# lyclyc52/Instance_NeRF

Hardware: AMD Instinct MI355X
Metric: Msamples/sec (train+infer) 3D-FRONT 800x800 at 1/2/4/8 MI355X; PSNR parity (higher is better)
Workload: dtype f32; 1 GPU; render 800x800 synthetic 3D-FRONT-like room, hash-grid NeRF L=16 F=2 T=6119864 sigma+rgb (BASELINE configs[1]), one view per step per GPU; parallelism=views sharded over 1 GPU(s), no data-path collective

## Files before the change

include/inr.h:

```cpp
#ifndef INR_H
#define INR_H

#include <stdint.h>

#ifdef __cplusplus
extern "C" {
#endif

#define INR_ABI_VERSION 12
#define INR_MAX_LEVELS 16

enum {
  INR_OK = 0,
  INR_EINVAL = -1,
  INR_ELAUNCH = -2,
  INR_ENODEV = -3
};

typedef void* inr_stream_t;

enum {
  INR_NUMERICS_TABLE_F16 = 1,
  INR_NUMERICS_MLP_F16 = 2
};

typedef struct inr_grid_desc {
  int32_t num_levels;
  int32_t level_dim;
  uint32_t offsets[INR_MAX_LEVELS + 1];
  float scales[INR_MAX_LEVELS];
  uint32_t resolutions[INR_MAX_LEVELS];
  uint32_t hashed[INR_MAX_LEVELS];
} inr_grid_desc;

int inr_abi_version(void);
const char* inr_last_error(void);
int inr_device_info(int32_t device, int64_t* props);
int inr_set_overlap_placement(int32_t on);
int inr_set_march_mode(int32_t mode);

int inr_get_rays(const float* poses, int64_t B, float fx, float fy, float cx, float cy, int32_t W,
                 const int64_t* inds , int64_t n, float* rays_o, float* rays_d, inr_stream_t s);

int inr_sample_training_batch(const float* pose , float fx, float fy, float cx, float cy, int32_t H, int32_t W,
                              const float* image , int32_t channels, const int32_t* mask ,
                              int32_t num_instances, int64_t seed, int64_t step, int64_t n, int64_t* inds ,
                              float* rays_o, float* rays_d, float* rgb , int64_t* labels ,
                              inr_stream_t s);

int inr_near_far_from_aabb(const float* rays_o, const float* rays_d, const float* aabb ,
                           int64_t N, float min_near, float* nears, float* fars, inr_stream_t s);
int inr_near_far_from_aabb_skip(const float* rays_o, const float* rays_d, const float* aabb , int64_t N,
                                float min_near, const int64_t* labels, int64_t ignore_index, float* nears, float* fars,
                                inr_stream_t s);

int inr_morton3D(const int32_t* coords , int64_t N, int32_t* indices, inr_stream_t s);
int inr_morton3D_invert(const int32_t* indices, int64_t N, int32_t* coords , inr_stream_t s);
int inr_packbits(const float* grid, int64_t n_bytes, float thresh, uint8_t* bitfield, inr_stream_t s);

int inr_mark_untrained_grid(const float* poses, int32_t B, float fx, float fy, float cx, float cy, int32_t H,
                            int32_t cascade, float bound, float* grid , inr_stream_t s);
int inr_occ_cell_positions(const int32_t* morton_idx, const float* noise, int64_t n, int32_t H, float cascade_bound,
                           float* xyz , inr_stream_t s);
int inr_occ_update(float* grid , const float* sigma , const int32_t* morton_idx ,
                   int64_t n_cells, int64_t m, float decay, float density_scale, float* tmp, double* mean_sum,
                   inr_stream_t s);
int inr_packbits_mean(const float* grid, int64_t n_cells , const double* mean_sum, float density_thresh,
                      uint8_t* bitfield, float* mean_out , const int32_t* counters ,
                      int32_t n_counters, int32_t counter_stride , double* stats_out ,
                      inr_stream_t s);
int64_t inr_occ_sample_workspace_bytes(int64_t n_cells);
int inr_occ_sample_cells(const float* grid , int64_t n_cells, const float* u ,
                         int64_t n, int32_t* morton_idx , void* workspace, inr_stream_t s);

int inr_march_write_fills_unowned_rows(int64_t N, int32_t sample_cap, int32_t max_steps);
int64_t inr_march_workspace_bytes(int64_t N, int32_t sample_cap);
int inr_march_rays_train_count(const float* rays_o, const float* rays_d, const uint8_t* bitfield,
                               float bound, float dt_gamma, int32_t max_steps, int64_t N,
                               int32_t cascade, int32_t H, const float* nears, const float* fars,
                               const float* noises , int32_t* rays ,
                               int32_t* counter , void* workspace, int32_t sample_cap, inr_stream_t s);
int inr_march_rays_train_write(const float* rays_o, const float* rays_d, const uint8_t* bitfield,
                               float bound, float dt_gamma, int32_t max_steps, int64_t N,
                               int32_t cascade, int32_t H, int64_t M, const float* nears,
                               const float* fars, const float* noises ,
                               const int32_t* rays , float* xyzs ,
                               float* dirs , float* deltas , const void* workspace,
                               int32_t sample_cap, inr_stream_t s);

int inr_march_rays_patch_write(const float* rays_o, const float* rays_d, const uint8_t* bitfield,
                               float bound, float dt_gamma, int32_t max_steps, int64_t N,
                               int32_t cascade, int32_t H, int64_t M, const float* nears,
                               const float* fars, const float* noises ,
                               const int32_t* rays ,
                               float* xyzs, float* dirs , float* deltas,
                               const void* workspace, int32_t sample_cap, int32_t* ray_ids ,
                               int32_t normalise , inr_stream_t s);
int inr_composite_rays_patch_forward(const float* sigmas, const float* rgbs, const float* deltas,
                                     const int32_t* rays, int64_t N, int64_t M, float T_thresh,
                                     const float* extra , int32_t K,
                                     float* weights_sum, float* depth, float* image,
                                     float* extra_out , float* weights ,
                                     uint64_t* skippable ,
                                     inr_stream_t s);
int inr_project_masks_patch(const float* xyzs, const float* weights, const int32_t* rays, int64_t N, int64_t M,
                            const uint32_t* mask_words, int32_t W, int32_t L, int32_t H, const float* bbox ,
                            int32_t k_total, int32_t k_base, int32_t k_count, float* out, inr_stream_t s);

int inr_march_rays(int64_t n_alive, int32_t n_step, const int32_t* rays_alive, const float* rays_t,
                   const float* rays_o, const float* rays_d, float bound, float dt_gamma,
                   int32_t max_steps, int32_t cascade, int32_t H, const uint8_t* bitfield,
                   const float* nears, const float* fars, float* xyzs, float* dirs, float* deltas,
                   inr_stream_t s);
int inr_composite_rays(int64_t n_alive, int32_t n_step, int32_t* rays_alive, float* rays_t,
                       const float* sigmas, const float* rgbs, const float* deltas,
                       float* weights_sum, float* depth, float* image, float T_thresh,
                       const float* extra , float* extra_acc ,
                       int32_t K, inr_stream_t s);
int inr_compact_alive(const int32_t* rays_alive, int64_t n_alive, int32_t* out, int32_t* n_out,
                      inr_stream_t s);

int inr_composite_rays_train_forward(const float* sigmas, const float* rgbs, const float* deltas,
                                     const int32_t* rays, int64_t N, int64_t M, float T_thresh,
                                     const float* extra , int32_t K,
                                     float* weights_sum, float* depth, float* image,
                                     float* extra_out , float* weights ,
                                     int32_t* sample_ray , inr_stream_t s);
int inr_composite_rays_extra_forward(const float* weights , const float* extra , const int32_t* rays,
                                     int64_t N, int64_t M, int32_t K, float* extra_out ,
                                     const int64_t* labels , int32_t n_classes, int64_t ignore_index,
                                     float* grad_pix, void* workspace, float* loss_out, inr_stream_t s);
int inr_composite_rays_train_backward(const float* grad_weights_sum, const float* grad_image,
                                      const float* grad_extra_out , const float* sigmas,
                                      const float* rgbs, const float* extra, const float* deltas,
                                      const int32_t* rays, const float* weights_sum,
                                      const float* image, const float* weights ,
                                      int64_t N, int64_t M, float T_thresh, int32_t K,
                                      float* grad_sigmas, float* grad_rgbs ,
                                      float* grad_extra , const int32_t* total_dev ,
                                      inr_stream_t s);

int inr_grid_encode_forward(const float* x , const float* embeddings ,
                            const inr_grid_desc* desc , int64_t M, float bound,
                            float* out , inr_stream_t s);
int inr_grid_encode_backward(const float* x, const float* grad_out ,
                             const inr_grid_desc* desc , int64_t M, float bound,
                             float* grad_embeddings , inr_stream_t s);

int inr_grid_encode_backward_ordered(const float* x, const float* grad_out, const int32_t* order,
                                     const inr_grid_desc* desc , int64_t M, float bound,
                                     float* grad_embeddings , inr_stream_t s);
int inr_grid_encode_backward_input(const float* x, const float* grad_out , const float* embeddings,
                                   const inr_grid_desc* desc , int64_t M, float bound, float* grad_x,
                                   inr_stream_t s);
int inr_grid_encode_backward_levels(const float* x, const float* grad_out, const int32_t* order,
                                    const inr_grid_desc* desc, int64_t M, float bound, float* grad_embeddings,
                                    int32_t level_lo, int32_t level_hi, inr_stream_t s);

#define INR_GRID_FX_STATE_FLOATS 4192
int inr_grid_encode_backward_levels_fx(const float* x, const float* grad_out, const int32_t* order,
                                       const inr_grid_desc* desc, int64_t M, float bound, float* grad_embeddings,
                                       int32_t level_lo, int32_t level_hi, float* fx_state ,
                                       inr_stream_t s);
int inr_grid_grad_finish_fx(float* grad_embeddings, const inr_grid_desc* desc , int32_t level_lo,
                            int32_t level_hi, float* fx_state, inr_stream_t s);
int inr_grid_fx_update(float* fx_state, int32_t num_levels, float headroom, int32_t sum_bits , inr_stream_t s);
int inr_grid_encode_backward_levels_fx64(const float* x, const float* grad_out, const int32_t* order,
                                         const inr_grid_desc* desc, int64_t M, float bound, float* grad_embeddings,
                                         int64_t* acc64 , int32_t level_lo, int32_t level_hi, float* fx_state,
                                         inr_stream_t s);
int inr_grid_grad_finish_fx64(int64_t* acc64, float* grad_embeddings, const inr_grid_desc* desc , int32_t level_lo,
                              int32_t level_hi, float* fx_state, inr_stream_t s);

int inr_sh_encode_forward(const float* d , int64_t M, int32_t degree, float* out, inr_stream_t s);
int inr_sh_encode_backward(const float* grad_out, const float* d, int64_t M, int32_t degree,
                           float* grad_d, inr_stream_t s);
int inr_sh_table_q(const float* d , int64_t N, float* out , inr_stream_t s);

int64_t inr_nerf_packed_floats(void);
int inr_nerf_pack_weights(const float* sigma_w0, const float* sigma_w1, const float* color_w0,
                          const float* color_w1, const float* color_w2, float* packed , int32_t numerics);
int64_t inr_instance_packed_floats(int32_t K);
int inr_instance_pack_weights(const float* w0, const float* w1, const float* w2, int32_t K,
                              float* packed , int32_t numerics);
int inr_nerf_forward(const float* x, const float* d, int64_t M, const int32_t* n_samples_dev,
                     float bound, const void* embeddings, const inr_grid_desc* desc ,
                     const float* packed , float density_scale, float* sigma, float* rgb,
                     float* geo_feat, int32_t numerics, inr_stream_t s);
int inr_nerf_forward_table(const float* x01, const int32_t* ray_ids, const float* sh_table_q, int64_t M,
                           float bound, const void* embeddings, const inr_grid_desc* desc ,
                           const float* packed , float density_scale, float* sigma, float* rgb,
                           int32_t numerics, inr_stream_t s);
int64_t inr_nerf_forward_table_sliced_workspace_bytes(int64_t M);
int inr_nerf_forward_table_sliced(const float* x01, const int32_t* ray_ids, const float* sh_table_q, int64_t M,
                                  float bound, const float* embeddings, const inr_grid_desc* desc ,
                                  const float* packed , float density_scale, float* sigma, float* rgb,
                                  float* fine_ws, inr_stream_t s);
int64_t inr_nerf_bwd_packed_floats(void);
int inr_nerf_pack_weights_device(const float* sigma_w0, const float* sigma_w1, const float* color_w0,
                                 const float* color_w1, const float* color_w2, float* packed_fwd,
                                 float* packed_bwd, inr_stream_t s);
int inr_nerf_forward_train(const float* x, const float* d, int64_t M, float bound, const float* embeddings,
                           const inr_grid_desc* desc , const float* packed_fwd, float* sigma, float* rgb,
                           float* enc, float* h1, float* so, float* cin, float* c1, float* c2, inr_stream_t s);
int inr_nerf_backward(const float* grad_sigma, const float* grad_rgb, const float* rgb, const float* so,
                      const float* h1, const float* c1, const float* c2, int64_t M, float density_scale,
                      const float* packed_bwd, float* grad_o, float* grad_zc2, float* grad_zc1, float* grad_so,
                      float* grad_zh1, float* grad_enc, inr_stream_t s);
int inr_nerf_forward_enc(const float* x, const float* d, int64_t M, float bound, const float* embeddings,
                         const inr_grid_desc* desc , const float* packed_fwd, float* sigma, float* rgb,
                         float* enc, inr_stream_t s);
int inr_nerf_head_backward(const float* enc, const float* d, const float* grad_sigma, const float* grad_rgb, int64_t M,
                           float density_scale, const float* packed_fwd, const float* packed_bwd, float* grad_enc,
                           void* workspace, float* grad_ws0, float* grad_ws1, float* grad_wc0, float* grad_wc1,
                           float* grad_wc2, float* zero_buf , int64_t zero_floats, inr_stream_t s);
int64_t inr_instance_bwd_packed_floats(void);
int inr_instance_pack_weights_device(const float* w0 , const float* w1 ,
                                     const float* w2 , int32_t K, float* packed_fwd, float* packed_bwd,
                                     inr_stream_t s);
int inr_instance_forward_train(const float* x, int64_t M, float bound, const float* embeddings,
                               const inr_grid_desc* desc , const float* packed_fwd, int32_t K,
                               float* logits, float* enc, float* h1, float* h2, inr_stream_t s);
int inr_instance_backward(const float* grad_logits, int32_t K, const float* h1, const float* h2, int64_t M,
                          const float* packed_bwd, float* grad_z2, float* grad_z1, float* grad_enc,
                          inr_stream_t s);
int inr_instance_forward_enc(const float* x, int64_t M, const int32_t* n_samples_dev, float bound,
                             const float* embeddings, const inr_grid_desc* desc , const float* packed_fwd,
                             int32_t K, float* logits, float* enc, inr_stream_t s);
int64_t inr_instance_head_workspace_bytes(void);
int inr_instance_head_backward(const float* enc, const float* weights, const int32_t* sample_ray,
                               const float* grad_pix, int32_t K, int64_t N, int64_t M, const int32_t* n_samples_dev,
                               const float* scale_a , const float* scale_b ,
                               const float* packed_fwd, const float* packed_bwd, float* grad_enc, void* workspace,
                               float* grad_w0, float* grad_w1, float* grad_w2, float* zero_buf ,
                               int64_t zero_floats, inr_stream_t s);
int inr_nerf_forward_dirs(const float* x, int64_t M, float bound, const float* embeddings, const inr_grid_desc* desc ,
                          const float* packed , const float* sh_dirs, int32_t n_dirs, float* out, inr_stream_t s);
int inr_nerf_forward_lattice(const float* ax_w, const float* ax_l, const float* ax_h, int32_t W, int32_t L, int32_t H,
                             float bound, const float* embeddings, const inr_grid_desc* desc ,
                             const float* packed , const float* sh_dirs, int32_t n_dirs, float logit_min,
                             float* out, inr_stream_t s);
int inr_instance_forward(const float* x, int64_t M, const int32_t* n_samples_dev, float bound,
                         const float* embeddings, const inr_grid_desc* desc ,
                         const float* packed , int32_t K, float* logits ,
                         inr_stream_t s);
int inr_instance_lattice(const float* ax_w, const float* ax_l, const float* ax_h, int32_t W, int32_t L, int32_t H,
                         float bound, const float* nerf_embeddings, const inr_grid_desc* nerf_desc ,
                         const float* nerf_packed , float density_scale, float sigma_thresh,
                         const float* inst_embeddings, const inr_grid_desc* inst_desc ,
                         const float* inst_packed , int32_t K, uint8_t* labels, float* confidence,
// ... 88 lines not shown
```

instance_nerf_amd/_lib.py:

```python
import ctypes
import os
from ctypes import POINTER, Structure, c_char_p, c_float, c_int32, c_int64, c_uint32, c_void_p

import torch

_HERE = os.path.dirname(os.path.abspath(__file__))
LIB_PATH = os.environ.get("INR_LIB_PATH") or os.path.join(_HERE, "csrc", "libinr_hip.so")
MAX_LEVELS = 16
GRID_FX_STATE_FLOATS = 4192
NUMERICS_TABLE_F16, NUMERICS_MLP_F16 = 1, 2


class GridDesc(Structure):
    _fields_ = [("num_levels", c_int32), ("level_dim", c_int32),
                ("offsets", c_uint32 * (MAX_LEVELS + 1)), ("scales", c_float * MAX_LEVELS),
                ("resolutions", c_uint32 * MAX_LEVELS), ("hashed", c_uint32 * MAX_LEVELS)]


P = c_void_p
_SIGS = {
    "inr_abi_version": (c_int32, []),
    "inr_last_error": (c_char_p, []),
    "inr_set_overlap_placement": (c_int32, [c_int32]),
    "inr_set_march_mode": (c_int32, [c_int32]),
    "inr_device_info": (c_int32, [c_int32, POINTER(c_int64)]),
    "inr_get_rays": (c_int32, [P, c_int64, c_float, c_float, c_float, c_float, c_int32, P, c_int64, P, P, P]),
    "inr_sample_training_batch": (c_int32, [P, c_float, c_float, c_float, c_float, c_int32, c_int32, P, c_int32, P, c_int32,
                                            c_int64, c_int64, c_int64, P, P, P, P, P, P]),
    "inr_near_far_from_aabb": (c_int32, [P, P, P, c_int64, c_float, P, P, P]),
    "inr_near_far_from_aabb_skip": (c_int32, [P, P, P, c_int64, c_float, P, c_int64, P, P, P]),
    "inr_morton3D": (c_int32, [P, c_int64, P, P]),
    "inr_morton3D_invert": (c_int32, [P, c_int64, P, P]),
    "inr_packbits": (c_int32, [P, c_int64, c_float, P, P]),
    "inr_mark_untrained_grid": (c_int32, [P, c_int32, c_float, c_float, c_float, c_float, c_int32, c_int32, c_float, P, P]),
    "inr_occ_cell_positions": (c_int32, [P, P, c_int64, c_int32, c_float, P, P]),
    "inr_occ_update": (c_int32, [P, P, P, c_int64, c_int64, c_float, c_float, P, P, P]),
    "inr_packbits_mean": (c_int32, [P, c_int64, P, c_float, P, P, P, c_int32, c_int32, P, P]),
    "inr_occ_sample_workspace_bytes": (c_int64, [c_int64]),
    "inr_occ_sample_cells": (c_int32, [P, c_int64, P, c_int64, P, P, P]),
    "inr_march_write_fills_unowned_rows": (c_int32, [c_int64, c_int32, c_int32]),
    "inr_march_workspace_bytes": (c_int64, [c_int64, c_int32]),
    "inr_march_rays_train_count": (c_int32, [P, P, P, c_float, c_float, c_int32, c_int64, c_int32, c_int32,
                                             P, P, P, P, P, P, c_int32, P]),
    "inr_march_rays_train_write": (c_int32, [P, P, P, c_float, c_float, c_int32, c_int64, c_int32, c_int32,
                                             c_int64, P, P, P, P, P, P, P, P, c_int32, P]),
    "inr_march_rays_patch_write": (c_int32, [P, P, P, c_float, c_float, c_int32, c_int64, c_int32, c_int32,
                                             c_int64, P, P, P, P, P, P, P, P, c_int32, P, c_int32, P]),
    "inr_nerf_bwd_packed_floats": (c_int64, []),
    "inr_nerf_pack_weights_device": (c_int32, [P, P, P, P, P, P, P, P]),
    "inr_nerf_forward_train": (c_int32, [P, P, c_int64, c_float, P, POINTER(GridDesc), P, P, P, P, P, P, P, P, P, P]),
    "inr_nerf_backward": (c_int32, [P, P, P, P, P, P, P, c_int64, c_float, P, P, P, P, P, P, P, P]),
    "inr_instance_bwd_packed_floats": (c_int64, []),
    "inr_instance_pack_weights_device": (c_int32, [P, P, P, c_int32, P, P, P]),
    "inr_instance_forward_train": (c_int32, [P, c_int64, c_float, P, POINTER(GridDesc), P, c_int32, P, P, P, P, P]),
    "inr_instance_backward": (c_int32, [P, c_int32, P, P, c_int64, P, P, P, P, P]),
    "inr_nerf_forward_enc": (c_int32, [P, P, c_int64, c_float, P, POINTER(GridDesc), P, P, P, P, P]),
    "inr_nerf_head_backward": (c_int32, [P, P, P, P, c_int64, c_float, P, P, P, P, P, P, P, P, P, P, c_int64, P]),
    "inr_instance_forward_enc": (c_int32, [P, c_int64, P, c_float, P, POINTER(GridDesc), P, c_int32, P, P, P]),
    "inr_instance_head_workspace_bytes": (c_int64, []),
    "inr_instance_head_backward": (c_int32, [P, P, P, P, c_int32, c_int64, c_int64, P, P, P, P, P, P, P, P, P, P, P, c_int64, P]),
    "inr_adam_step_multi": (c_int32, [c_int32, P, P, P, P, P, P, c_float, c_float, c_float, c_int32, c_float, P]),
    "inr_adam_ema_step_multi": (c_int32, [c_int32, P, P, P, P, P, P, c_float, c_float, c_float, c_int32, c_float, P,
                                          c_float, P]),
    "inr_adam_set_hyper": (c_int32, [P, c_int32, c_float, c_float, c_float, c_int32, P, P]),
    "inr_adam_step_multi_dev": (c_int32, [c_int32, P, P, P, P, P, P, c_float, c_float, c_float, P]),
    "inr_copy_multi": (c_int32, [c_int32, P, P, P, P]),
    "inr_adam_set_hyper_ema": (c_int32, [P, c_int32, c_float, c_float, c_float, c_int32, c_float, P, P]),
    "inr_adam_ema_step_multi_dev": (c_int32, [c_int32, P, P, P, P, P, P, c_float, c_float, c_float, P, P]),
    "inr_cross_entropy": (c_int32, [P, P, c_int64, c_int32, c_int64, P, P, P, P]),
    "inr_finish_rays": (c_int32, [P, P, P, P, P, P, c_float, c_float, c_float, c_int64, P, P, P]),
    "inr_finish_rays_mse": (c_int32, [P, P, P, P, P, c_float, c_float, c_float, P, P, c_int64, P, P, P, P, P]),
    "inr_sh_table_q": (c_int32, [P, c_int64, P, P]),
    "inr_nerf_forward_table": (c_int32, [P, P, P, c_int64, c_float, P, POINTER(GridDesc), P, c_float, P, P, c_int32, P]),
    "inr_nerf_forward_table_sliced_workspace_bytes": (c_int64, [c_int64]),
    "inr_nerf_forward_table_sliced": (c_int32, [P, P, P, c_int64, c_float, P, POINTER(GridDesc), P, c_float, P, P, P, P]),
    "inr_composite_rays_patch_forward": (c_int32, [P, P, P, P, c_int64, c_int64, c_float, P, c_int32, P, P, P, P, P, P, P]),
    "inr_project_masks_patch": (c_int32, [P, P, P, c_int64, c_int64, P, c_int32, c_int32, c_int32, P, c_int32, c_int32, c_int32,
                                          P, P]),
    "inr_march_rays": (c_int32, [c_int64, c_int32, P, P, P, P, c_float, c_float, c_int32, c_int32, c_int32,
                                 P, P, P, P, P, P, P]),
    "inr_composite_rays": (c_int32, [c_int64, c_int32, P, P, P, P, P, P, P, P, c_float, P, P, c_int32, P]),
    "inr_compact_alive": (c_int32, [P, c_int64, P, P, P]),
    "inr_composite_rays_extra_forward": (c_int32, [P, P, P, c_int64, c_int64, c_int32, P, P, c_int32, c_int64, P, P, P, P]),
    "inr_composite_rays_train_forward": (c_int32, [P, P, P, P, c_int64, c_int64, c_float, P, c_int32, P, P, P, P, P, P, P]),
    "inr_composite_rays_train_backward": (c_int32, [P, P, P, P, P, P, P, P, P, P, P, c_int64, c_int64, c_float, c_int32,
                                                    P, P, P, P, P]),
    "inr_grid_encode_forward": (c_int32, [P, P, POINTER(GridDesc), c_int64, c_float, P, P]),
    "inr_grid_encode_backward": (c_int32, [P, P, POINTER(GridDesc), c_int64, c_float, P, P]),
    "inr_grid_encode_backward_ordered": (c_int32, [P, P, P, POINTER(GridDesc), c_int64, c_float, P, P]),
    "inr_grid_encode_backward_input": (c_int32, [P, P, P, POINTER(GridDesc), c_int64, c_float, P, P]),
    "inr_grid_encode_backward_levels": (c_int32, [P, P, P, POINTER(GridDesc), c_int64, c_float, P, c_int32, c_int32, P]),
    "inr_grid_encode_backward_levels_fx": (c_int32, [P, P, P, POINTER(GridDesc), c_int64, c_float, P, c_int32, c_int32, P, P]),
    "inr_grid_grad_finish_fx": (c_int32, [P, POINTER(GridDesc), c_int32, c_int32, P, P]),
    "inr_grid_fx_update": (c_int32, [P, c_int32, c_float, c_int32, P]),
    "inr_grid_encode_backward_levels_fx64": (c_int32, [P, P, P, POINTER(GridDesc), c_int64, c_float, P, P, c_int32, c_int32, P, P]),
    "inr_grid_grad_finish_fx64": (c_int32, [P, P, POINTER(GridDesc), c_int32, c_int32, P, P]),
    "inr_sh_encode_forward": (c_int32, [P, c_int64, c_int32, P, P]),
    "inr_sh_encode_backward": (c_int32, [P, P, c_int64, c_int32, P, P]),
    "inr_nerf_packed_floats": (c_int64, []),
    "inr_nerf_pack_weights": (c_int32, [P, P, P, P, P, P, c_int32]),
    "inr_instance_packed_floats": (c_int64, [c_int32]),
    "inr_instance_pack_weights": (c_int32, [P, P, P, c_int32, P, c_int32]),
    "inr_nerf_forward": (c_int32, [P, P, c_int64, P, c_float, P, POINTER(GridDesc), P, c_float, P, P, P, c_int32, P]),
    "inr_nerf_forward_dirs": (c_int32, [P, c_int64, c_float, P, POINTER(GridDesc), P, P, c_int32, P, P]),
    "inr_nerf_forward_lattice": (c_int32, [P, P, P, c_int32, c_int32, c_int32, c_float, P, POINTER(GridDesc), P, P, c_int32,
                                           c_float, P, P]),
    "inr_instance_forward": (c_int32, [P, c_int64, P, c_float, P, POINTER(GridDesc), P, c_int32, P, P]),
    "inr_instance_lattice": (c_int32, [P, P, P, c_int32, c_int32, c_int32, c_float, P, POINTER(GridDesc), P, c_float,
                                       c_float, P, POINTER(GridDesc), P, c_int32, P, P, P, P]),
    "inr_instance_volume_stats": (c_int32, [P, P, c_int32, c_int32, c_int32, c_int32, P, c_int64, P, P, P, P]),
    "inr_mesh_workspace_bytes": (c_int64, [c_int32, c_int32, c_int32, c_int32]),
    "inr_mesh_count": (c_int32, [P, c_int32, c_float, c_float, P, c_int32, c_int32, c_int32, c_int32, c_int32, P, c_int64, P, P]),
    "inr_mesh_emit": (c_int32, [P, c_int32, c_float, c_float, P, c_int32, P, P, P, P, c_int32, c_int32, c_int32, c_float,
                                c_float, c_float, c_int32, P, c_int64, c_int32, c_int32, P, P, P, P, P]),
    "inr_roi_align_3d_set_mode": (c_int32, [c_int32]),
    "inr_roi_align_3d_forward": (c_int32, [P, P, P, c_int32, c_int32, c_int32, c_int32, c_int32, c_int64, c_int32,
                                           c_int32, c_int32, c_float, P, P]),
    "inr_roi_align_3d_backward": (c_int32, [P, P, P, c_int32, c_int32, c_int32, c_int32, c_int32, c_int64, c_int32,
                                            c_int32, c_int32, c_float, P, P]),
    "inr_roi_align_3d_backward_workspace_bytes": (c_int64, [c_int32, c_int32, c_int32, c_int32, c_int32, c_int64, c_int32,
                                                            c_int32, c_int32]),
    "inr_roi_align_3d_backward_prefers_workspace": (c_int32, [c_int32, c_int32, c_int32, c_int32, c_int32, c_int64, c_int32,
                                                              c_int32, c_int32, c_int64]),
    "inr_roi_align_3d_backward_ws": (c_int32, [P, P, P, c_int32, c_int32, c_int32, c_int32, c_int32, c_int64, c_int32,
                                               c_int32, c_int32, c_float, P, P, c_int64, P]),
    "inr_nerf_render": (c_int32, [P, P, P, P, c_int64, c_int64, c_float, P, POINTER(GridDesc), P, c_float, c_float,
                                  P, P, P, P, P, c_int32, c_int32, P]),
    "inr_instance_render": (c_int32, [P, P, P, c_int64, c_int64, c_float, P, POINTER(GridDesc), P, c_int32, P, c_int32, P,
                                      c_int32, P]),
    "inr_linear_wgrad_workspace_bytes": (c_int64, []),
    "inr_linear_wgrad": (c_int32, [P, P, c_int64, c_int32, c_int32, P, P, P]),
    "inr_adam_step": (c_int32, [P, P, P, P, c_int64, c_float, c_float, c_float, c_float, c_int32, c_float, P]),
}
EXPORTS = tuple(_SIGS)

ABI_VERSION = 12
INSTANCE_STATS_WORKSPACE_BYTES = 512 * 64 * 8 * 4
_lib = None


def load():
    global _lib
    if _lib is not None:
        return _lib
    if not os.path.exists(LIB_PATH):
        raise RuntimeError(
            f"{LIB_PATH} is missing: build it with `python -m instance_nerf_amd.build` "
            "(or __graft_entry__.build()).  There is no CPU fallback.")
    lib = ctypes.CDLL(LIB_PATH)
    version = getattr(lib, "inr_abi_version", None)
    if version is not None:
        version.restype, version.argtypes = c_int32, []
    found = version() if version is not None else None
    if found != ABI_VERSION:
        raise RuntimeError(f"{LIB_PATH} ABI version {found} != {ABI_VERSION} (include/inr.h "
                           "INR_ABI_VERSION): rebuild with `python -m instance_nerf_amd.build --force`")
    for name, (res, args) in _SIGS.items():
        fn = getattr(lib, name)
        fn.restype = res
        fn.argtypes = args
    _lib = lib
    return lib


def check(rc, what=""):
    if rc != 0:
        msg = load().inr_last_error()
        raise RuntimeError(f"libinr_hip {what} failed (code {rc}): {msg.decode() if msg else ''}")


_raw_stream = getattr(torch._C, "_cuda_getCurrentRawStream", None)
_cur_device = getattr(torch._C, "_cuda_getDevice", None)


def stream_ptr():
    if _raw_stream is not None and _cur_device is not None:
        return c_void_p(_raw_stream(_cur_device()))
    return c_void_p(torch.cuda.current_stream().cuda_stream)


def ptr(t, dtype=None, name="tensor", allow_none=False):
    if t is None:
        if allow_none:
            return None
        raise RuntimeError(f"{name} must not be None")
    if not t.is_cuda:
        raise RuntimeError(f"{name} must be a GPU tensor (the HIP path has no CPU fallback)")
    if not t.is_contiguous():
        raise RuntimeError(f"{name} must be contiguous")
    if dtype is not None and t.dtype != dtype:
        raise RuntimeError(f"{name} must be {dtype}, got {t.dtype}")
    return c_void_p(t.data_ptr())


def host_ptr(t, dtype, name="tensor"):
    if t.is_cuda or not t.is_contiguous() or t.dtype != dtype:
        raise RuntimeError(f"{name} must be a contiguous CPU {dtype} tensor")
    return c_void_p(t.data_ptr())


def make_grid_desc(table):
    d = GridDesc()
    L = int(table["num_levels"])
    d.num_levels = L
    d.level_dim = int(table["level_dim"])
    for i in range(L + 1):
        d.offsets[i] = int(table["offsets"][i])
    for i in range(L):
        d.scales[i] = float(table["scales"][i])
        d.resolutions[i] = int(table["resolutions"][i])
        d.hashed[i] = int(table["hashed"][i])
    return d
```

instance_nerf_amd/csrc/raymarch.hip:

```cpp
#include "common.h"

namespace inr {

static thread_local char g_err[512] = "";
int g_field_lds_min = 0;
int g_march_lds_pad = 0;
void set_error(const char* fmt, ...) {
  va_list ap;
  va_start(ap, fmt);
  vsnprintf(g_err, sizeof(g_err), fmt, ap);
  va_end(ap);
}

constexpr int kRayBlock = 256;
constexpr float kSqrt3x2 = 3.4641016151377544f;

__global__ void __launch_bounds__(kRayBlock) k_near_far(const float* __restrict__ rays_o,
                                                        const float* __restrict__ rays_d,
                                                        const float* __restrict__ aabb, int64_t N,
                                                        float min_near, float* __restrict__ nears,
                                                        float* __restrict__ fars,
                                                        const int64_t* __restrict__ labels, int64_t ignore) {
  const int64_t n = (int64_t)blockIdx.x * blockDim.x + threadIdx.x;
  if (n >= N) return;
  float near = -INFINITY, far = INFINITY;
  bool miss = labels != nullptr && labels[n] == ignore;
#pragma unroll
  for (int a = 0; a < 3; ++a) {
    const float o = rays_o[n * 3 + a];
    const float rd = 1.0f / rays_d[n * 3 + a];
    const float t0 = (aabb[a] - o) * rd;
    const float t1 = (aabb[a + 3] - o) * rd;
    const float lo = t0 > t1 ? t1 : t0;
    const float hi = t0 > t1 ? t0 : t1;
    if (a > 0) miss = miss || (near > hi) || (lo > far);
    near = lo > near ? lo : near;
    far = hi < far ? hi : far;
  }
  if (near < min_near) near = min_near;
  nears[n] = miss ? 3.402823466e+38f : near;
  fars[n] = miss ? 3.402823466e+38f : far;
}

__global__ void __launch_bounds__(kRayBlock) k_get_rays(const float* __restrict__ poses, int64_t B, float fx, float fy,
                                                        float cx, float cy, int W, const int64_t* __restrict__ inds,
                                                        int64_t n, float* __restrict__ rays_o,
                                                        float* __restrict__ rays_d) {
  const int64_t idx = (int64_t)blockIdx.x * blockDim.x + threadIdx.x;
  if (idx >= B * n) return;
  const int64_t b = idx / n, k = idx - b * n;
  const int64_t pix = inds ? inds[k] : k;
  const float i = (float)(pix % W) + 0.5f, j = (float)(pix / W) + 0.5f;
  const float xs = (i - cx) / fx, ys = (j - cy) / fy;
  const float nrm = sqrtf(xs * xs + ys * ys + 1.0f * 1.0f);
  const float dx = xs / nrm, dy = ys / nrm, dz = 1.0f / nrm;
  const float* P = poses + b * 16;
#pragma unroll
  for (int r = 0; r < 3; ++r) {
    rays_d[idx * 3 + r] = dx * P[r * 4 + 0] + dy * P[r * 4 + 1] + dz * P[r * 4 + 2];
    rays_o[idx * 3 + r] = P[r * 4 + 3];
  }
}

__device__ __forceinline__ uint64_t mix64(uint64_t z) {
  z = (z ^ (z >> 30)) * 0xBF58476D1CE4E5B9ull;
  z = (z ^ (z >> 27)) * 0x94D049BB133111EBull;
  return z ^ (z >> 31);
}
__global__ void __launch_bounds__(kRayBlock) k_sample_batch(const float* __restrict__ pose, float fx, float fy, float cx,
                                                            float cy, int H, int W, const float* __restrict__ image,
                                                            int C, const int32_t* __restrict__ mask, int num_instances,
                                                            uint64_t seed, uint64_t step, int64_t n,
                                                            int64_t* __restrict__ inds, float* __restrict__ rays_o,
                                                            float* __restrict__ rays_d, float* __restrict__ rgb,
                                                            int64_t* __restrict__ labels) {
  const int64_t k = (int64_t)blockIdx.x * blockDim.x + threadIdx.x;
  if (k >= n) return;
  const uint64_t h = mix64(seed + 0x9E3779B97F4A7C15ull * ((step << 32) + (uint64_t)k));
  const uint64_t pix = ((h >> 32) * (uint64_t)((int64_t)H * W)) >> 32;
  inds[k] = (int64_t)pix;
  const float i = (float)(pix % (uint64_t)W) + 0.5f, j = (float)(pix / (uint64_t)W) + 0.5f;
  const float xs = (i - cx) / fx, ys = (j - cy) / fy;
  const float nrm = sqrtf(xs * xs + ys * ys + 1.0f * 1.0f);
  const float dx = xs / nrm, dy = ys / nrm, dz = 1.0f / nrm;
#pragma unroll
  for (int r = 0; r < 3; ++r) {
    rays_d[k * 3 + r] = dx * pose[r * 4 + 0] + dy * pose[r * 4 + 1] + dz * pose[r * 4 + 2];
    rays_o[k * 3 + r] = pose[r * 4 + 3];
  }
  if (image) {
    for (int c = 0; c < C; ++c) rgb[k * C + c] = image[pix * C + c];
  }
  if (mask) {
    const int32_t l = mask[pix];
    labels[k] = l >= num_instances ? -1 : (int64_t)l;
  }
}

__global__ void k_morton3D(const int32_t* __restrict__ coords, int64_t N, int32_t* __restrict__ out) {
  const int64_t n = (int64_t)blockIdx.x * blockDim.x + threadIdx.x;
  if (n >= N) return;
  out[n] = (int32_t)morton3((uint32_t)coords[n * 3], (uint32_t)coords[n * 3 + 1], (uint32_t)coords[n * 3 + 2]);
}
__global__ void k_morton3D_invert(const int32_t* __restrict__ idx, int64_t N, int32_t* __restrict__ coords) {
  const int64_t n = (int64_t)blockIdx.x * blockDim.x + threadIdx.x;
  if (n >= N) return;
  const uint32_t m = (uint32_t)idx[n];
  coords[n * 3 + 0] = (int32_t)compact_bits10(m);
  coords[n * 3 + 1] = (int32_t)compact_bits10(m >> 1);
  coords[n * 3 + 2] = (int32_t)compact_bits10(m >> 2);
}
__global__ void k_packbits(const float* __restrict__ grid, int64_t n_bytes, float thresh,
                           uint8_t* __restrict__ bits) {
  const int64_t n = (int64_t)blockIdx.x * blockDim.x + threadIdx.x;
  if (n >= n_bytes) return;
  const float4 a = reinterpret_cast<const float4*>(grid)[n * 2];
  const float4 b = reinterpret_cast<const float4*>(grid)[n * 2 + 1];
  uint32_t v = (a.x > thresh) | ((a.y > thresh) << 1) | ((a.z > thresh) << 2) | ((a.w > thresh) << 3) |
               ((b.x > thresh) << 4) | ((b.y > thresh) << 5) | ((b.z > thresh) << 6) | ((b.w > thresh) << 7);
  bits[n] = (uint8_t)v;
}

__global__ void k_occ_positions(const int32_t* __restrict__ morton, const float* __restrict__ noise, int64_t n, float Hm1,
                                float ext, float half, float* __restrict__ xyz) {
  const int64_t i = (int64_t)blockIdx.x * blockDim.x + threadIdx.x;
  if (i >= n) return;
  const uint32_t m = morton ? (uint32_t)morton[i] : (uint32_t)i;
  const uint32_t c[3] = {compact_bits10(m), compact_bits10(m >> 1), compact_bits10(m >> 2)};
#pragma unroll
  for (int a = 0; a < 3; ++a) {
    float v = (2.0f * (float)c[a] / Hm1 - 1.0f) * ext;
    if (noise) v = v + (noise[i * 3 + a] * 2.0f - 1.0f) * half;
    xyz[i * 3 + a] = v;
  }
}
__global__ void __launch_bounds__(256) k_mark_untrained(const float* __restrict__ poses, int B, float kx, float ky, int H,
                                                        int C, float bound, float* __restrict__ grid) {
  const int64_t i = (int64_t)blockIdx.x * blockDim.x + threadIdx.x;
  const int64_t H3 = (int64_t)H * H * H;
  if (i >= (int64_t)C * H3) return;
  const int cas = (int)(i / H3);
  const uint32_t m = (uint32_t)(i - (int64_t)cas * H3);
  const float bnd = fminf(ldexpf(1.0f, cas), bound), half = bnd / (float)H, ext = bnd - half;
  const float wx = (2.0f * (float)compact_bits10(m) / (float)(H - 1) - 1.0f) * ext;
  const float wy = (2.0f * (float)compact_bits10(m >> 1) / (float)(H - 1) - 1.0f) * ext;
  const float wz = (2.0f * (float)compact_bits10(m >> 2) / (float)(H - 1) - 1.0f) * ext;
  bool seen = false;
  for (int b = 0; b < B && !seen; ++b) {
    const float* P = poses + (int64_t)b * 16;
    const float dx = wx - P[3], dy = wy - P[7], dz = wz - P[11];
    const float cx = dx * P[0] + dy * P[4] + dz * P[8];
    const float cy = dx * P[1] + dy * P[5] + dz * P[9];
    const float cz = dx * P[2] + dy * P[6] + dz * P[10];
    seen = cz > 0.0f && fabsf(cx) < kx * cz + half * 2.0f && fabsf(cy) < ky * cz + half * 2.0f;
  }
  if (!seen) grid[i] = -1.0f;
}

__global__ void k_occ_scatter(const float* __restrict__ sigma, const int32_t* __restrict__ morton, int64_t m,
                              float density_scale, float* __restrict__ tmp) {
  const int64_t i = (int64_t)blockIdx.x * blockDim.x + threadIdx.x;
  if (i < m) tmp[morton[i]] = sigma[i] * density_scale;
}
__global__ void __launch_bounds__(256) k_occ_update(float* __restrict__ grid, const float* __restrict__ tmp, int64_t n,
                                                    float decay, float scale, double* __restrict__ mean_sum) {
  __shared__ double red[4];
  double acc = 0.0;
  auto cell = [&](float g, float t, bool& changed) {
    t *= scale;
    if (g >= 0.0f && t >= 0.0f) { g = fmaxf(g * decay, t); changed = true; }
    acc += (double)fmaxf(g, 0.0f);
    return g;
  };
  const int64_t n4 = (((uintptr_t)grid | (uintptr_t)tmp) & 15) == 0 ? n / 4 : 0;
  for (int64_t i = (int64_t)blockIdx.x * blockDim.x + threadIdx.x; i < n4; i += (int64_t)gridDim.x * blockDim.x) {
    float4 g = reinterpret_cast<float4*>(grid)[i];
    const float4 t = reinterpret_cast<const float4*>(tmp)[i];
    bool changed = false;
    g.x = cell(g.x, t.x, changed); g.y = cell(g.y, t.y, changed); g.z = cell(g.z, t.z, changed); g.w = cell(g.w, t.w, changed);
    if (changed) reinterpret_cast<float4*>(grid)[i] = g;
  }
  for (int64_t i = n4 * 4 + (int64_t)blockIdx.x * blockDim.x + threadIdx.x; i < n; i += (int64_t)gridDim.x * blockDim.x) {
    bool changed = false;
    const float g = cell(grid[i], tmp[i], changed);
    if (changed) grid[i] = g;
  }
#pragma unroll
  for (int d = 32; d >= 1; d >>= 1) acc += __shfl_xor(acc, d, 64);
  if ((threadIdx.x & 63) == 0) red[threadIdx.x >> 6] = acc;
  __syncthreads();
  if (threadIdx.x == 0) atomicAdd(mean_sum, red[0] + red[1] + red[2] + red[3]);
}
__global__ void k_packbits_mean(const float* __restrict__ grid, int64_t n_bytes, const double* __restrict__ mean_sum,
                                double inv_cells, float density_thresh, uint8_t* __restrict__ bits,
                                float* __restrict__ mean_out, const int32_t* __restrict__ counters, int n_counters,
                                int counter_stride, double* __restrict__ stats_out) {
  const int64_t n = (int64_t)blockIdx.x * blockDim.x + threadIdx.x;
  const float mean = (float)(*mean_sum * inv_cells);
  if (n == 0 && mean_out) *mean_out = mean;
  if (n == 0 && stats_out) {
    int64_t total = 0;
    for (int k = 0; k < n_counters; ++k) total += counters[(int64_t)k * counter_stride];
    stats_out[0] = (double)mean;
    stats_out[1] = (double)total;
  }
  if (n >= n_bytes) return;
  const float thresh = fminf(mean, density_thresh);
  const float4 a = reinterpret_cast<const float4*>(grid)[n * 2];
  const float4 b = reinterpret_cast<const float4*>(grid)[n * 2 + 1];
  uint32_t v = (a.x > thresh) | ((a.y > thresh) << 1) | ((a.z > thresh) << 2) | ((a.w > thresh) << 3) |
               ((b.x > thresh) << 4) | ((b.y > thresh) << 5) | ((b.z > thresh) << 6) | ((b.w > thresh) << 7);
  bits[n] = (uint8_t)v;
}

struct MarchParams {
  const uint8_t* bits;
  float bound, dt_gamma, dt_min, dt_max, rH;
  int C, H, H3;
};

struct Ray {
  float ox, oy, oz, dx, dy, dz, rdx, rdy, rdz, sx, sy, sz;
};

__device__ __forceinline__ Ray load_ray(const float* __restrict__ o, const float* __restrict__ d, int64_t n) {
  Ray r;
  r.ox = o[n * 3]; r.oy = o[n * 3 + 1]; r.oz = o[n * 3 + 2];
  r.dx = d[n * 3]; r.dy = d[n * 3 + 1]; r.dz = d[n * 3 + 2];
  r.rdx = 1.0f / r.dx; r.rdy = 1.0f / r.dy; r.rdz = 1.0f / r.dz;
  r.sx = copysignf(1.0f, r.dx); r.sy = copysignf(1.0f, r.dy); r.sz = copysignf(1.0f, r.dz);
  return r;
}

__device__ __forceinline__ float step_dt(const MarchParams& P, float t) {
  return clampf(t * P.dt_gamma, P.dt_min, P.dt_max);
}
template <bool kConst>
struct StepRule {
  float c;
  __device__ __forceinline__ explicit StepRule(const MarchParams& P) : c(step_dt(P, 0.0f)) {}
  __device__ __forceinline__ float operator()(const MarchParams& P, float t) const {
    if constexpr (kConst) return c;
    else return step_dt(P, t);
  }
};

struct MortonCalc {
  __device__ __forceinline__ uint32_t operator()(uint32_t x, uint32_t y, uint32_t z) const { return morton3(x, y, z); }
};
struct MortonLut {
  const uint32_t* lut;
  __device__ __forceinline__ uint32_t operator()(uint32_t x, uint32_t y, uint32_t z) const {
    return lut[x] | (lut[y] << 1) | (lut[z] << 2);
  }
};

template <bool kSingle = false, bool kConstDt = false, class Emit, class Advance, class Morton = MortonCalc>
__device__ __forceinline__ int march_ray(const MarchParams& P, const Ray& r, float t, float far,
                                         int max_emit, Emit&& emit, Advance&& advance, Morton morton = Morton()) {
  int n = 0;
  float last_t = t;
  const StepRule<kConstDt> step(P);
  const float mb1 = fminf(ldexpf(1.0f, 0), P.bound), rmb1 = 1.0f / mb1;
  while (t < far && n < max_emit) {
    const float px = clampf(r.ox + t * r.dx, -P.bound, P.bound);
    const float py = clampf(r.oy + t * r.dy, -P.bound, P.bound);
    const float pz = clampf(r.oz + t * r.dz, -P.bound, P.bound);
    const float dt = step(P, t);
    int level = 0;
    float mb = mb1, rmb = rmb1;
    if constexpr (!kSingle) {
      int e0, e1;
      (void)frexpf(fmaxf(fabsf(px), fmaxf(fabsf(py), fabsf(pz))), &e0);
      (void)frexpf(dt * (float)P.H * 0.5f, &e1);
      level = max(clampi(e0, 0, P.C - 1), clampi(e1, 0, P.C - 1));
      mb = fminf(ldexpf(1.0f, level), P.bound);
      rmb = 1.0f / mb;
    }
    const int nx = clampi((int)(((px * rmb + 1.0f) * 0.5f) * (float)P.H), 0, P.H - 1);
    const int ny = clampi((int)(((py * rmb + 1.0f) * 0.5f) * (float)P.H), 0, P.H - 1);
    const int nz = clampi((int)(((pz * rmb + 1.0f) * 0.5f) * (float)P.H), 0, P.H - 1);
    const uint32_t idx = (uint32_t)level * (uint32_t)P.H3 + morton((uint32_t)nx, (uint32_t)ny, (uint32_t)nz);
    const bool occ = (P.bits[idx >> 3] >> (idx & 7)) & 1;
    if (occ) {
      const float tn = t + dt;
      emit(px, py, pz, dt, tn - last_t, t);
      t = tn;
      advance();
      last_t = tn;
      ++n;
    } else {
      const float ax = ((float)nx + 0.5f) + 0.5f * r.sx;
      const float ay = ((float)ny + 0.5f) + 0.5f * r.sy;
      const float az = ((float)nz + 0.5f) + 0.5f * r.sz;
      const float cx = (((ax * P.rH) * 2.0f - 1.0f) * mb - px) * r.rdx;
      const float cy = (((ay * P.rH) * 2.0f - 1.0f) * mb - py) * r.rdy;
      const float cz = (((az * P.rH) * 2.0f - 1.0f) * mb - pz) * r.rdz;
      const float tt = t + fmaxf(0.0f, fminf(cx, fminf(cy, cz)));
      do {
        t = t + step(P, t);
        advance();
      } while (t < tt);
    }
  }
  return n;
}
template <class Emit>
__device__ __forceinline__ int march_ray(const MarchParams& P, const Ray& r, float t, float far,
                                         int max_emit, Emit&& emit) {
  return P.dt_gamma == 0.0f ? march_ray<false, true>(P, r, t, far, max_emit, emit, [] {})
                            : march_ray<false, false>(P, r, t, far, max_emit, emit, [] {});
}
template <class Emit, class Advance, class Morton>
__device__ __forceinline__ int march_ray_any(const MarchParams& P, const Ray& r, float t, float far,
                                             int max_emit, Emit&& emit, Advance&& advance, Morton morton) {
  if (P.dt_gamma == 0.0f)
    return P.C == 1 ? march_ray<true, true>(P, r, t, far, max_emit, emit, advance, morton)
                    : march_ray<false, true>(P, r, t, far, max_emit, emit, advance, morton);
  return P.C == 1 ? march_ray<true, false>(P, r, t, far, max_emit, emit, advance, morton)
                  : march_ray<false, false>(P, r, t, far, max_emit, emit, advance, morton);
}

__device__ __forceinline__ float start_t(const MarchParams& P, float near, float noise) {
  return near + step_dt(P, near) * noise;
}

__global__ void __launch_bounds__(kRayBlock) k_march_count(MarchParams P, const float* __restrict__ rays_o,
                                                           const float* __restrict__ rays_d, int64_t N,
                                                           int max_steps, const float* __restrict__ nears,
                                                           const float* __restrict__ fars,
                                                           const float* __restrict__ noises,
                                                           int32_t* __restrict__ counts,
                                                           int32_t* __restrict__ block_sums,
                                                           uint32_t* __restrict__ mask, int cap_words) {
  __shared__ int32_t wsum[kRayBlock / 64];
  __shared__ uint32_t lut[1024];
  for (int i = threadIdx.x; i < P.H; i += kRayBlock) lut[i] = expand_bits10((uint32_t)i);
  __syncthreads();
  const MortonLut morton{lut};
  const int64_t n = (int64_t)blockIdx.x * blockDim.x + threadIdx.x;
  int cnt = 0;
  if (n < N) {
    const Ray r = load_ray(rays_o, rays_d, n);
    const float t0 = start_t(P, nears[n], noises ? noises[n] : 0.0f);
    if (cap_words > 0) {
      uint32_t word = 0;
      int widx = 0, cand = 0;
      bool ok = true;
      cnt = march_ray_any(P, r, t0, fars[n], max_steps,
                      [&](float, float, float, float, float, float) {
                        const int w = cand >> 5;
                        if (w < cap_words) {
                          while (widx < w) {
                            mask[(int64_t)widx * N + n] = word;
                            word = 0;
                            ++widx;
                          }
                          word |= 1u << (cand & 31);
                        } else {
                          ok = false;
                        }
                      },
                      [&] { ++cand; }, morton);
      if (widx < cap_words) mask[(int64_t)widx * N + n] = word;
      mask[(int64_t)cap_words * N + n] = ok ? 1u : 0u;
    } else {
      cnt = march_ray_any(P, r, t0, fars[n], max_steps, [](float, float, float, float, float, float) {}, [] {}, morton);
    }
    counts[n] = cnt;
  }
  const int incl = wave_inclusive_scan(cnt);
  if ((threadIdx.x & 63) == 63) wsum[threadIdx.x >> 6] = incl;
  __syncthreads();
  if (threadIdx.x == 0) {
    int s = 0;
#pragma unroll
    for (int w = 0; w < kRayBlock / 64; ++w) s += wsum[w];
    block_sums[blockIdx.x] = s;
  }
}

__global__ void __launch_bounds__(1024) k_scan_block_sums(int32_t* __restrict__ block_sums, int n_blocks,
                                                          int64_t N, int32_t* __restrict__ counter) {
  __shared__ int32_t wsum[16];
  __shared__ int32_t carry_s;
  if (threadIdx.x == 0) carry_s = 0;
  __syncthreads();
  for (int base = 0; base < n_blocks; base += 1024) {
    const int i = base + threadIdx.x;
    const int v = i < n_blocks ? block_sums[i] : 0;
    const int incl = wave_inclusive_scan(v);
    if ((threadIdx.x & 63) == 63) wsum[threadIdx.x >> 6] = incl;
    __syncthreads();
    int wave_off = 0;
    for (int w = 0; w < (int)(threadIdx.x >> 6); ++w) wave_off += wsum[w];
    const int carry = carry_s;
    if (i < n_blocks) block_sums[i] = carry + wave_off + incl - v;
    __syncthreads();
    if (threadIdx.x == 1023) carry_s = carry + wave_off + incl;
    __syncthreads();
  }
  if (threadIdx.x == 0) {
    counter[0] = carry_s;
    counter[1] = (int32_t)N;
  }
}

__global__ void __launch_bounds__(kRayBlock) k_finalize_offsets(const int32_t* __restrict__ counts,
                                                                const int32_t* __restrict__ block_prefix,
                                                                int64_t N, int32_t* __restrict__ rays) {
  __shared__ int32_t wsum[kRayBlock / 64];
  const int64_t n = (int64_t)blockIdx.x * blockDim.x + threadIdx.x;
  const int cnt = n < N ? counts[n] : 0;
  const int incl = wave_inclusive_scan(cnt);
  if ((threadIdx.x & 63) == 63) wsum[threadIdx.x >> 6] = incl;
  __syncthreads();
  int off = block_prefix[blockIdx.x] + incl - cnt;
  for (int w = 0; w < (int)(threadIdx.x >> 6); ++w) off += wsum[w];
  if (n < N) {
    rays[n * 3 + 0] = (int32_t)n;
    rays[n * 3 + 1] = off;
    rays[n * 3 + 2] = cnt;
  }
}

template <bool kConstDt, class Emit>
__device__ __forceinline__ void replay_ray_t(const MarchParams& P, const Ray& r, const uint32_t* __restrict__ mask, int64_t N,
                                             int64_t n, float t, int cnt, Emit&& emit) {
  const StepRule<kConstDt> step(P);
  float last_t = t;
  int emitted = 0;
  for (int w = 0; emitted < cnt; ++w) {
    const uint32_t bits = mask[(int64_t)w * N + n];
    for (int b0 = 0; b0 < 32; b0 += 8) {
      const uint32_t sub = (bits >> b0) & 0xFFu;
      if (__ballot(sub != 0u) == 0ull) {
#pragma unroll
        for (int j = 0; j < 8; ++j) t = t + step(P, t);
        continue;
      }
#pragma unroll
      for (int j = 0; j < 8; ++j) {
        const float dt = step(P, t);
        const float tn = t + dt;
        if (sub & (1u << j)) {
          const float px = clampf(r.ox + t * r.dx, -P.bound, P.bound);
          const float py = clampf(r.oy + t * r.dy, -P.bound, P.bound);
          const float pz = clampf(r.oz + t * r.dz, -P.bound, P.bound);
          emit(px, py, pz, dt, tn - last_t, t);
          last_t = tn;
          ++emitted;
        }
        t = tn;
      }
    }
  }
}
template <class Emit>
__device__ __forceinline__ void replay_ray(const MarchParams& P, const Ray& r, const uint32_t* __restrict__ mask, int64_t N,
                                           int64_t n, float t, int cnt, Emit&& emit) {
  if (P.dt_gamma == 0.0f) replay_ray_t<true>(P, r, mask, N, n, t, cnt, emit);
  else replay_ray_t<false>(P, r, mask, N, n, t, cnt, emit);
}

__global__ void __launch_bounds__(kRayBlock) k_march_write(MarchParams P, const float* __restrict__ rays_o,
                                                           const float* __restrict__ rays_d, int64_t N,
                                                           int64_t M, const float* __restrict__ nears,
                                                           const float* __restrict__ fars,
                                                           const float* __restrict__ noises,
                                                           const int32_t* __restrict__ rays,
                                                           float* __restrict__ xyzs, float* __restrict__ dirs,
                                                           float* __restrict__ deltas,
                                                           const uint32_t* __restrict__ mask, int cap_words) {
  const int64_t n = (int64_t)blockIdx.x * blockDim.x + threadIdx.x;
  if (n >= N) return;
  const int off = rays[n * 3 + 1];
  const int cnt = rays[n * 3 + 2];
  if (cnt == 0 || (int64_t)off + cnt > M) return;
  const Ray r = load_ray(rays_o, rays_d, n);
  int64_t i = off;
  auto emit = [&](float px, float py, float pz, float dt, float delta, float) {
    xyzs[i * 3 + 0] = px; xyzs[i * 3 + 1] = py; xyzs[i * 3 + 2] = pz;
    dirs[i * 3 + 0] = r.dx; dirs[i * 3 + 1] = r.dy; dirs[i * 3 + 2] = r.dz;
    deltas[i * 2 + 0] = dt; deltas[i * 2 + 1] = delta;
    ++i;
  };
  const float t0 = start_t(P, nears[n], noises ? noises[n] : 0.0f);
  if (cap_words > 0 && mask[(int64_t)cap_words * N + n]) {
    replay_ray(P, r, mask, N, n, t0, cnt, emit);
  } else {
    march_ray(P, r, t0, fars[n], cnt, emit);
  }
}

template <bool kSingle = false, class Emit>
__device__ __forceinline__ int march_ray_coop(const MarchParams& P, const Ray& r, float t, float far, int max_emit,
                                              Emit&& emit) {
  const float mb1 = fminf(ldexpf(1.0f, 0), P.bound), rmb1 = 1.0f / mb1;
  const int lane = threadIdx.x & 63;
  const uint64_t lt_mask = (1ull << lane) - 1ull;
  int n = 0;
  float last_t = t;
  while (t < far && n < max_emit) {
    float c = t;
    if (P.dt_gamma == 0.0f) {
      const float dt0 = step_dt(P, t);
      asm volatile(
          ".rept 63\n"
          "s_nop 1\n"
          "v_add_f32_dpp %0, %0, %1 wave_shr:1 row_mask:0xf bank_mask:0xf\n"
          ".endr\n"
          : "+v"(c)
          : "v"(dt0));
    } else {
      for (int j = 0; j < 63; ++j) c = j < lane ? c + step_dt(P, c) : c;
    }
    const bool in = c < far;
    const float px = clampf(r.ox + c * r.dx, -P.bound, P.bound);
    const float py = clampf(r.oy + c * r.dy, -P.bound, P.bound);
    const float pz = clampf(r.oz + c * r.dz, -P.bound, P.bound);
    const float dt = step_dt(P, c);
    const float tn = c + dt;
    int level = 0;
    float mb = mb1, rmb = rmb1;
    if constexpr (!kSingle) {
      int e0, e1;
      (void)frexpf(fmaxf(fabsf(px), fmaxf(fabsf(py), fabsf(pz))), &e0);
      (void)frexpf(dt * (float)P.H * 0.5f, &e1);
      level = max(clampi(e0, 0, P.C - 1), clampi(e1, 0, P.C - 1));
      mb = fminf(ldexpf(1.0f, level), P.bound);
      rmb = 1.0f / mb;
    }
    const int nx = clampi((int)(((px * rmb + 1.0f) * 0.5f) * (float)P.H), 0, P.H - 1);
    const int ny = clampi((int)(((py * rmb + 1.0f) * 0.5f) * (float)P.H), 0, P.H - 1);
    const int nz = clampi((int)(((pz * rmb + 1.0f) * 0.5f) * (float)P.H), 0, P.H - 1);
    const uint32_t idx = (uint32_t)level * (uint32_t)P.H3 + morton3((uint32_t)nx, (uint32_t)ny, (uint32_t)nz);
    const bool occ = (P.bits[idx >> 3] >> (idx & 7)) & 1;
    const float ax = ((float)nx + 0.5f) + 0.5f * r.sx;
    const float ay = ((float)ny + 0.5f) + 0.5f * r.sy;
    const float az = ((float)nz + 0.5f) + 0.5f * r.sz;
    const float cx = (((ax * P.rH) * 2.0f - 1.0f) * mb - px) * r.rdx;
    const float cy = (((ay * P.rH) * 2.0f - 1.0f) * mb - py) * r.rdy;
    const float cz = (((az * P.rH) * 2.0f - 1.0f) * mb - pz) * r.rdz;
    const float tt = c + fmaxf(0.0f, fminf(cx, fminf(cy, cz)));
    int lo = lane + 1, hi = 64;
    bool settled_all = false;
    if (P.dt_gamma == 0.0f) {
      const int i0 = lane + (int)fminf((tt - c) * (1.0f / dt), 64.0f);
      const float ca = __shfl(c, clampi(i0 - 1, 0, 63), 64);
      const float cb = __shfl(c, min(i0, 63), 64);
      const float cc = __shfl(c, min(i0 + 1, 63), 64);
      const bool lt_a = i0 - 1 <= lane || ca < tt;
      const bool ge_b = i0 >= 64 || !(cb < tt);
      const bool ge_c = i0 + 1 >= 64 || !(cc < tt);
      const bool take_b = i0 > lane && ge_b;
      const bool settled = take_b ? lt_a : ge_c;
      lo = take_b ? min(i0, 64) : i0 + 1;
      settled_all = __ballot(in && !occ && !settled) == 0;
    }
    if (!settled_all) {
      lo = lane + 1;
#pragma unroll
      for (int it = 0; it < 7; ++it) {
        const int mid = (lo + hi) >> 1;
        const float cm = __shfl(c, min(mid, 63), 64);
        const bool below = mid < 64 && cm < tt;
        if (lo < hi) {
          if (below) lo = mid + 1; else hi = mid;
        }
      }
    }
    const int next = lo;
    const uint64_t in_mask = __ballot(in);
    const uint64_t miss_mask = __ballot(in && !occ);
    const int n_in = __popcll(in_mask);
// ... 605 lines not shown
    const float e = live ? expf(x - m) : 0.f;
    float ssum = e;
#pragma unroll
    for (int d = 1; d < 64; d <<= 1) ssum += __shfl_xor(ssum, d, 64);
    const float xy = __shfl(x, keep ? (int)y : 0, 64);
    if (lane < K) ce.dpix[(int64_t)rid * K + lane] = (keep && live) ? e / ssum - (lane == (int)y ? 1.f : 0.f) : 0.f;
    if (lane == 0)
      ce.part[rid] = make_float4(keep ? (m + logf(ssum)) - xy : 0.f, keep ? 1.f : 0.f,
                                 (y != ce.ignore_index && !in_range) ? 1.f : 0.f, 0.f);
  }
}

__global__ void __launch_bounds__(1024) k_ce_finalize(const float4* __restrict__ part, int64_t N, float* __restrict__ loss_out) {
  __shared__ float red[3][16];
  float a = 0.f, b = 0.f, c = 0.f;
  for (int64_t i = threadIdx.x; i < N; i += 1024) {
    const float4 p = part[i];
    a += p.x; b += p.y; c += p.z;
  }
  a = wave_sum(a); b = wave_sum(b); c = wave_sum(c);
  if ((threadIdx.x & 63) == 0) { red[0][threadIdx.x >> 6] = a; red[1][threadIdx.x >> 6] = b; red[2][threadIdx.x >> 6] = c; }
  __syncthreads();
  if (threadIdx.x == 0) {
    float sa = 0.f, sb = 0.f, sc = 0.f;
    for (int w = 0; w < 16; ++w) { sa += red[0][w]; sb += red[1][w]; sc += red[2][w]; }
    loss_out[0] = sc > 0.f ? NAN : sa / sb;
    loss_out[1] = sb > 0.f ? 1.0f / sb : 0.f;
    loss_out[2] = sb;
    loss_out[3] = sc;
  }
}

__global__ void __launch_bounds__(kRayBlock) k_composite_train_bwd(
    const float* __restrict__ g_ws, const float* __restrict__ g_img, const float* __restrict__ sigmas,
    const float* __restrict__ rgbs, const float* __restrict__ deltas, const int32_t* __restrict__ rays,
    const float* __restrict__ weights_sum, const float* __restrict__ image, int64_t N, int64_t M, float T_thresh,
    float* __restrict__ grad_sigmas, float* __restrict__ grad_rgbs, const int32_t* __restrict__ total_dev) {
  const int64_t n = ((int64_t)blockIdx.x * blockDim.x + threadIdx.x) >> 6;
  const int lane = threadIdx.x & 63;
  if (n >= N) return;
  const int32_t rid = rays[n * 3], off = rays[n * 3 + 1];
  int32_t cnt = rays[n * 3 + 2];
  auto zero_rows = [&](int64_t lo, int64_t hi) {
    for (int64_t i = lo + lane; i < hi; i += 64) {
      grad_sigmas[i] = 0.f; grad_rgbs[i * 3] = 0.f; grad_rgbs[i * 3 + 1] = 0.f; grad_rgbs[i * 3 + 2] = 0.f;
    }
  };
  if (total_dev) {
    const int64_t total = total_dev[0];
    if (total < M) {
      const int64_t per = (M - total + N - 1) / N;
      zero_rows(total + n * per, min(M, total + (n + 1) * per));
    }
  }
  if ((int64_t)off + cnt > M) {
    if (total_dev && cnt > 0 && off < M) zero_rows(off, M);
    cnt = 0;
  }
  const float gr = g_img[rid * 3], gg = g_img[rid * 3 + 1], gb = g_img[rid * 3 + 2];
  const float gw = g_ws ? g_ws[rid] : 0.0f;
  const float rf = image[rid * 3], gf = image[rid * 3 + 1], bf = image[rid * 3 + 2];
  const float wsf = weights_sum[rid];
  float T_carry = 1.0f, cr_carry = 0.f, cg_carry = 0.f, cb_carry = 0.f;
  bool dead = false;
  for (int base = 0; base < cnt; base += 64) {
    const bool act = base + lane < cnt;
    const int64_t i = (int64_t)off + base + lane;
    if (dead) {
      if (act) { grad_sigmas[i] = 0.f; grad_rgbs[i * 3] = 0.f; grad_rgbs[i * 3 + 1] = 0.f; grad_rgbs[i * 3 + 2] = 0.f; }
      continue;
    }
    float alpha = 0.f, d0 = 0.f, cr = 0.f, cg = 0.f, cb = 0.f;
    if (act) {
      d0 = deltas[i * 2];
      alpha = 1.0f - expf(-sigmas[i] * d0);
      cr = rgbs[i * 3]; cg = rgbs[i * 3 + 1]; cb = rgbs[i * 3 + 2];
    }
    const float P = wave_incl_prod(1.0f - alpha, lane);
    float Pprev = __shfl_up(P, 1, 64);
    if (lane == 0) Pprev = 1.0f;
    const float T = T_carry * Pprev, Tn = T_carry * P;
    const bool used = act && (T >= T_thresh || (base + lane) == 0);
    const float w = used ? alpha * T : 0.0f;
    const float ar = cr_carry + wave_incl_sum(w * cr, lane);
    const float ag = cg_carry + wave_incl_sum(w * cg, lane);
    const float ab = cb_carry + wave_incl_sum(w * cb, lane);
    if (act) {
      grad_rgbs[i * 3] = gr * w; grad_rgbs[i * 3 + 1] = gg * w; grad_rgbs[i * 3 + 2] = gb * w;
      grad_sigmas[i] = used ? d0 * (gr * (Tn * cr - (rf - ar)) + gg * (Tn * cg - (gf - ag)) + gb * (Tn * cb - (bf - ab)) +
                                    gw * (1.0f - wsf))
                            : 0.0f;
    }
    T_carry *= __shfl(P, 63, 64);
    cr_carry = __shfl(ar, 63, 64); cg_carry = __shfl(ag, 63, 64); cb_carry = __shfl(ab, 63, 64);
    if (T_carry < T_thresh) dead = true;
  }
}

__global__ void __launch_bounds__(kRayBlock) k_composite_train_extra_bwd(
    const float* __restrict__ g_extra_out, const float* __restrict__ wbuf, const int32_t* __restrict__ rays, int64_t N,
    int64_t M, int K, float* __restrict__ grad_extra) {
  const int64_t n = ((int64_t)blockIdx.x * blockDim.x + threadIdx.x) >> 6;
  const int lane = threadIdx.x & 63;
  if (n >= N) return;
  const int32_t rid = rays[n * 3], off = rays[n * 3 + 1];
  int32_t cnt = rays[n * 3 + 2];
  if ((int64_t)off + cnt > M) cnt = 0;
  if (lane >= K) return;
  const float g = g_extra_out[(int64_t)rid * K + lane];
  for (int s = 0; s < cnt; ++s) grad_extra[((int64_t)off + s) * K + lane] = wbuf[(int64_t)off + s] * g;
}

constexpr int kGroup = 16;

struct GroupCursor {
  int c[kGroup];
  int S;
  int r;
  int k;
  __device__ __forceinline__ void init(int my_count, int my_offset) {
    const int lane = threadIdx.x & 63, g0 = lane & ~(kGroup - 1);
    r = lane & (kGroup - 1);
#pragma unroll
    for (int i = 0; i < kGroup; ++i) c[i] = __shfl(my_count, g0 + i, 64);
    S = __shfl(my_offset, g0, 64);
    k = 0;
  }
  __device__ __forceinline__ int total() const {
    int t = 0;
#pragma unroll
    for (int i = 0; i < kGroup; ++i) t += c[i];
    return t;
  }
  int nact_ = 0, rank_ = 0, k_change_ = 0;
  __device__ __forceinline__ int next() {
    if (k >= k_change_) {
      int nact = 0, rank = 0, nxt = 0x7FFFFFFF;
#pragma unroll
      for (int i = 0; i < kGroup; ++i) {
        const bool gt = c[i] > k;
        nact += gt ? 1 : 0;
        rank += (gt && i < r) ? 1 : 0;
        nxt = gt ? min(nxt, c[i]) : nxt;
      }
      nact_ = nact; rank_ = rank; k_change_ = nxt;
    }
    const int slot = S + rank_;
    S += nact_;
    ++k;
    return slot;
  }
};

__global__ void __launch_bounds__(kRayBlock) k_march_write_patch(MarchParams P, const float* __restrict__ rays_o,
                                                                 const float* __restrict__ rays_d, int64_t N, int64_t M,
                                                                 const float* __restrict__ nears,
                                                                 const float* __restrict__ fars,
                                                                 const float* __restrict__ noises,
                                                                 const int32_t* __restrict__ rays,
                                                                 float* __restrict__ xyzs, float* __restrict__ dirs,
                                                                 float* __restrict__ deltas,
                                                                 const uint32_t* __restrict__ mask, int cap_words,
                                                                 int32_t* __restrict__ ray_ids, int normalise) {
  const int64_t n = (int64_t)blockIdx.x * blockDim.x + threadIdx.x;
  const int off = n < N ? rays[n * 3 + 1] : 0;
  const int cnt = n < N ? rays[n * 3 + 2] : 0;
  GroupCursor cur;
  cur.init(cnt, off);
  if (cnt == 0 || (int64_t)cur.S + cur.total() > M) return;
  const Ray r = load_ray(rays_o, rays_d, n);
  const float rb = 2.0f * P.bound;
  auto emit = [&](float px, float py, float pz, float dt, float delta, float) {
    const int64_t i = cur.next();
    if (normalise) {
      px = (px + P.bound) / rb; py = (py + P.bound) / rb; pz = (pz + P.bound) / rb;
    }
    xyzs[i * 3 + 0] = px; xyzs[i * 3 + 1] = py; xyzs[i * 3 + 2] = pz;
    if (dirs) { dirs[i * 3 + 0] = r.dx; dirs[i * 3 + 1] = r.dy; dirs[i * 3 + 2] = r.dz; }
    if (ray_ids) ray_ids[i] = (int32_t)n;
    deltas[i * 2 + 0] = dt; deltas[i * 2 + 1] = delta;
  };
  const float t0 = start_t(P, nears[n], noises ? noises[n] : 0.0f);
  if (cap_words > 0 && mask[(int64_t)cap_words * N + n]) {
    replay_ray(P, r, mask, N, n, t0, cnt, emit);
  } else {
    march_ray(P, r, t0, fars[n], cnt, emit);
  }
}

__global__ void __launch_bounds__(kRayBlock) k_composite_patch_fwd(const float* __restrict__ sigmas,
                                                                   const float* __restrict__ rgbs,
                                                                   const float* __restrict__ deltas,
                                                                   const int32_t* __restrict__ rays, int64_t N, int64_t M,
                                                                   float T_thresh, float* __restrict__ wbuf,
                                                                   float* __restrict__ weights_sum,
                                                                   float* __restrict__ depth, float* __restrict__ image,
                                                                   unsigned long long* __restrict__ skippable) {
  const int64_t n = (int64_t)blockIdx.x * blockDim.x + threadIdx.x;
  const int lane = threadIdx.x & 63, g0 = lane & ~(kGroup - 1), rr = lane & (kGroup - 1);
  const int32_t rid = n < N ? rays[n * 3] : 0;
  const int off = n < N ? rays[n * 3 + 1] : 0;
  int cnt = n < N ? rays[n * 3 + 2] : 0;
  int S = __shfl(off, g0, 64);
  int gtot = cnt;
#pragma unroll
  for (int d = 1; d < kGroup; d <<= 1) gtot += __shfl_xor(gtot, d, 64);
  if ((int64_t)S + gtot > M) cnt = 0;
  int maxc = cnt;
#pragma unroll
  for (int d = 1; d < 64; d <<= 1) maxc = max(maxc, __shfl_xor(maxc, d, 64));
  float T = 1.0f, r = 0, g = 0, b = 0, ws = 0, t = 0, dsum = 0;
  bool done = false;
  unsigned n_skip = 0;
  constexpr int kAhead = 8;
  for (int k = 0; k < maxc; k += kAhead) {
    unsigned field[kAhead];
    int64_t slot[kAhead];
    bool active[kAhead];
    float2 dl[kAhead];
    float sg[kAhead], cr[kAhead], cg[kAhead], cb[kAhead];
#pragma unroll
    for (int j = 0; j < kAhead; ++j) {
      active[j] = k + j < cnt;
      field[j] = (unsigned)(__ballot(active[j]) >> g0) & 0xFFFFu;
      slot[j] = (int64_t)S + __popc(field[j] & ((1u << rr) - 1u));
      S += __popc(field[j]);
      const int64_t i = (active[j] && !done) ? slot[j] : 0;
      dl[j] = reinterpret_cast<const float2*>(deltas)[i];
      sg[j] = sigmas[i];
      cr[j] = rgbs[i * 3]; cg[j] = rgbs[i * 3 + 1]; cb[j] = rgbs[i * 3 + 2];
    }
#pragma unroll
    for (int j = 0; j < kAhead; ++j) {
      if (skippable) {
        const unsigned live = (unsigned)(__ballot(active[j] && !done) >> g0) & 0xFFFFu;
        if (rr == 0 && field[j] != 0 && live == 0) n_skip += __popc(field[j]);
      }
      if (active[j] && !done) {
        const float alpha = 1.0f - expf(-sg[j] * dl[j].x);
        const float w = alpha * T;
        r += w * cr[j]; g += w * cg[j]; b += w * cb[j];
        t += dl[j].y;
        dsum += w * t;
        ws += w;
        if (wbuf) wbuf[slot[j]] = w;
        T *= 1.0f - alpha;
        if (T < T_thresh) done = true;
      } else if (active[j] && wbuf) {
        wbuf[slot[j]] = 0.0f;
      }
    }
  }
  if (n < N) {
    weights_sum[rid] = ws; depth[rid] = dsum;
    image[rid * 3] = r; image[rid * 3 + 1] = g; image[rid * 3 + 2] = b;
  }
  if (skippable) {
#pragma unroll
    for (int d = 1; d < 64; d <<= 1) n_skip += __shfl_xor(n_skip, d, 64);
    if (lane == 0 && n_skip) atomicAdd(skippable, (unsigned long long)n_skip);
  }
}

__global__ void __launch_bounds__(kRayBlock) k_composite_patch_extra(const float* __restrict__ wbuf,
                                                                     const float* __restrict__ extra,
                                                                     const int32_t* __restrict__ rays, int64_t N,
                                                                     int64_t M, int K, float* __restrict__ extra_out) {
  const int64_t n = ((int64_t)blockIdx.x * blockDim.x + threadIdx.x) >> 6;
  const int lane = threadIdx.x & 63;
  if (n >= N) return;
  const int64_t g0 = n & ~(int64_t)(kGroup - 1);
  const int r = (int)(n - g0);
  int c[kGroup];
  int total = 0;
#pragma unroll
  for (int i = 0; i < kGroup; ++i) {
    c[i] = (g0 + i < N) ? rays[(g0 + i) * 3 + 2] : 0;
    total += c[i];
  }
  const int32_t rid = rays[n * 3];
  int64_t S = rays[g0 * 3 + 1];
  const int cnt = (S + total <= M) ? c[r] : 0;
  float acc = 0.0f;
  for (int k = 0; k < cnt; ++k) {
    int nact = 0, rank = 0;
#pragma unroll
    for (int i = 0; i < kGroup; ++i) {
      const int gt = c[i] > k ? 1 : 0;
      nact += gt;
      rank += (i < r) ? gt : 0;
    }
    const int64_t slot = S + rank;
    S += nact;
    const float w = wbuf[slot];
    if (lane < K && w != 0.0f) acc += w * extra[slot * K + lane];
  }
  if (lane < K) extra_out[(int64_t)rid * K + lane] = acc;
}

struct MaskVolume {
  float lo[3], hi[3], res[3];
  int W, L, H;
};
__global__ void __launch_bounds__(kRayBlock) k_project_masks_patch(const float* __restrict__ xyzs,
                                                                   const float* __restrict__ wbuf,
                                                                   const int32_t* __restrict__ rays, int64_t N, int64_t M,
                                                                   const uint32_t* __restrict__ words, MaskVolume V,
                                                                   int k_total, int k_base, int k_count,
                                                                   float* __restrict__ out) {
  const int64_t n = (int64_t)blockIdx.x * blockDim.x + threadIdx.x;
  const int lane = threadIdx.x & 63, g0 = lane & ~(kGroup - 1), rr = lane & (kGroup - 1);
  const int32_t rid = n < N ? rays[n * 3] : 0;
  const int off = n < N ? rays[n * 3 + 1] : 0;
  int cnt = n < N ? rays[n * 3 + 2] : 0;
  int S = __shfl(off, g0, 64);
  int gtot = cnt;
#pragma unroll
  for (int d = 1; d < kGroup; d <<= 1) gtot += __shfl_xor(gtot, d, 64);
  if ((int64_t)S + gtot > M) cnt = 0;
  int maxc = cnt;
#pragma unroll
  for (int d = 1; d < 64; d <<= 1) maxc = max(maxc, __shfl_xor(maxc, d, 64));
  float acc[32];
#pragma unroll
  for (int i = 0; i < 32; ++i) acc[i] = 0.0f;
  for (int k = 0; k < maxc; ++k) {
    const bool active = k < cnt;
    const unsigned field = (unsigned)(__ballot(active) >> g0) & 0xFFFFu;
    const int64_t slot = (int64_t)S + __popc(field & ((1u << rr) - 1u));
    S += __popc(field);
    const float w = active ? wbuf[slot] : 0.0f;
    if (w != 0.0f) {
      const float x = xyzs[slot * 3], y = xyzs[slot * 3 + 1], z = xyzs[slot * 3 + 2];
      const float fx = floorf(((x - V.lo[0]) / (V.hi[0] - V.lo[0])) * V.res[0]);
      const float fy = floorf(((y - V.lo[1]) / (V.hi[1] - V.lo[1])) * V.res[1]);
      const float fz = floorf(((z - V.lo[2]) / (V.hi[2] - V.lo[2])) * V.res[2]);
      const bool inside = fx >= 0.0f && fx < V.res[0] && fy >= 0.0f && fy < V.res[1] && fz >= 0.0f && fz < V.res[2];
      if (inside) {
        const uint32_t word = words[((int64_t)(int)fx * V.L + (int)fy) * V.H + (int)fz];
// ... 123 lines not shown
  INR_REQUIRE(grid && bitfield, "null pointer");
  INR_REQUIRE(((uintptr_t)grid & 15) == 0, "grid must be 16-byte aligned");
  k_packbits<<<blocks_for(n_bytes, 256), 256, 0, as_stream(s)>>>(grid, n_bytes, thresh, bitfield);
  return check_launch("packbits");
}

int inr_mark_untrained_grid(const float* poses, int32_t B, float fx, float fy, float cx, float cy, int32_t H, int32_t cascade,
                            float bound, float* grid, inr_stream_t s) {
  INR_REQUIRE(B >= 0 && H >= 2 && H <= 1024 && cascade >= 1 && grid, "bad argument");
  INR_REQUIRE(B == 0 || poses, "null poses");
  INR_REQUIRE(fx != 0.0f && fy != 0.0f, "zero focal length");
  const int64_t n = (int64_t)cascade * H * H * H;
  k_mark_untrained<<<blocks_for(n, 256), 256, 0, as_stream(s)>>>(poses, B, cx / fx, cy / fy, H, cascade, bound, grid);
  return check_launch("mark_untrained_grid");
}

int inr_occ_cell_positions(const int32_t* morton_idx, const float* noise, int64_t n, int32_t H, float cascade_bound,
                           float* xyz, inr_stream_t s) {
  INR_REQUIRE(n >= 0 && H >= 2 && H <= 1024, "bad argument");
  if (n == 0) return INR_OK;
  INR_REQUIRE(xyz, "null pointer");
  const float half = cascade_bound / (float)H;
  k_occ_positions<<<blocks_for(n, 256), 256, 0, as_stream(s)>>>(morton_idx, noise, n, (float)(H - 1), cascade_bound - half,
                                                                half, xyz);
  return check_launch("occ_cell_positions");
}

int inr_occ_update(float* grid, const float* sigma, const int32_t* morton_idx, int64_t n_cells, int64_t m, float decay,
                   float density_scale, float* tmp, double* mean_sum, inr_stream_t s) {
  INR_REQUIRE(n_cells > 0 && m >= 0 && grid && mean_sum, "bad argument");
  INR_REQUIRE(m == 0 || sigma, "null sigma");
  hipStream_t st = as_stream(s);
  const unsigned nb = (unsigned)std::min<int64_t>((n_cells + 1023) / 1024, (int64_t)cu_count() * 2);
  if (morton_idx) {
    INR_REQUIRE(tmp, "a listed update needs the scratch grid");
    if (hipMemsetAsync(tmp, 0xBF, (size_t)n_cells * sizeof(float), st) != hipSuccess) {
      set_error("occ_update: memset failed");
      return INR_ELAUNCH;
    }
    if (m) k_occ_scatter<<<blocks_for(m, 256), 256, 0, st>>>(sigma, morton_idx, m, density_scale, tmp);
    k_occ_update<<<nb, 256, 0, st>>>(grid, tmp, n_cells, decay, 1.0f, mean_sum);
  } else {
    INR_REQUIRE(m == n_cells, "a full sweep needs one sigma per cell (Morton order)");
    k_occ_update<<<nb, 256, 0, st>>>(grid, sigma, n_cells, decay, density_scale, mean_sum);
  }
  return check_launch("occ_update");
}

int inr_packbits_mean(const float* grid, int64_t n_cells, const double* mean_sum, float density_thresh, uint8_t* bitfield,
                      float* mean_out, const int32_t* counters, int32_t n_counters, int32_t counter_stride,
                      double* stats_out, inr_stream_t s) {
  INR_REQUIRE(n_cells > 0 && n_cells % 8 == 0 && grid && mean_sum && bitfield, "bad argument");
  INR_REQUIRE(((uintptr_t)grid & 15) == 0, "grid must be 16-byte aligned");
  INR_REQUIRE(n_counters >= 0 && (n_counters == 0 || (counters && stats_out && counter_stride > 0)), "bad counters");
  k_packbits_mean<<<blocks_for(n_cells / 8, 256), 256, 0, as_stream(s)>>>(grid, n_cells / 8, mean_sum, 1.0 / (double)n_cells,
                                                                           density_thresh, bitfield, mean_out, counters,
                                                                           n_counters, counter_stride, stats_out);
  return check_launch("packbits_mean");
}

int64_t inr_occ_sample_workspace_bytes(int64_t n_cells) {
  if (n_cells <= 0) return -1;
  const int64_t n_blocks = (n_cells + kOccBlockCells - 1) / kOccBlockCells;
  return n_blocks * (kOccBlockCells / 64) * (int64_t)sizeof(uint64_t) + (n_blocks + 2 * kOccBuckets) * (int64_t)sizeof(int32_t);
}

int inr_occ_sample_cells(const float* grid, int64_t n_cells, const float* u, int64_t n, int32_t* morton_idx,
                         void* workspace, inr_stream_t s) {
  INR_REQUIRE(grid && u && morton_idx && workspace && n > 0 && n_cells > 0, "bad argument");
  INR_REQUIRE(2 * n < (int64_t)1 << 31 && n_cells < (int64_t)1 << 31, "sizes must fit int32");
  INR_REQUIRE(((uintptr_t)workspace & 7) == 0, "workspace must be 8-byte aligned");
  const int64_t n_blocks = (n_cells + kOccBlockCells - 1) / kOccBlockCells;
  INR_REQUIRE(n_blocks <= kOccMaxBlocks, "grid too large for the block table (H <= 256)");
  hipStream_t st = as_stream(s);
  uint64_t* masks = reinterpret_cast<uint64_t*>(workspace);
  int32_t* block_counts = reinterpret_cast<int32_t*>(masks + n_blocks * (kOccBlockCells / 64));
  int32_t* hist = block_counts + n_blocks;
  k_occ_count<<<(int)n_blocks, kOccBlockCells, 0, st>>>(grid, n_cells, masks, block_counts, hist);
  k_occ_hist<<<(int)std::min<int64_t>(64, blocks_for(2 * n, 1024)), 1024, 0, st>>>(u, n, hist);
  const size_t lds = (size_t)(2 * (kOccBuckets + 1) + n_blocks + 1) * sizeof(int32_t);
  static size_t lds_allowed = 64 * 1024;
  if (lds > lds_allowed) {
    if (hipFuncSetAttribute((const void*)k_occ_pick, hipFuncAttributeMaxDynamicSharedMemorySize, (int)lds) != hipSuccess) {
      set_error("occ_sample_cells: %zu bytes of LDS refused", lds);
      return INR_ELAUNCH;
    }
    lds_allowed = lds;
  }
  k_occ_pick<<<(int)std::min<int64_t>(256, blocks_for(2 * n, 1024)), 1024, lds, st>>>(u + 2 * n, n, hist, masks, block_counts,
                                                                                       (int)n_blocks, n_cells, morton_idx);
  return check_launch("occ_sample_cells");
}

static int g_march_mode = -1;
static bool use_coop(int64_t N, int32_t sample_cap) {
  if (sample_cap > 0) return false;
  if (g_march_mode >= 0) return g_march_mode != 0;
  return N <= 32768;
}
int inr_set_march_mode(int32_t mode) {
  INR_REQUIRE(mode >= -1 && mode <= 1, "mode must be -1 (automatic), 0 (lane per ray) or 1 (wave per ray)");
  g_march_mode = mode;
  return INR_OK;
}

static int64_t ws_ints(int64_t N) {
  const int64_t nb = (N + kRayBlock - 1) / kRayBlock;
  return ((N + nb + 64 + 1) / 2) * 2;
}
static int cap_words_of(int32_t sample_cap) { return sample_cap > 0 ? (sample_cap + 31) / 32 : 0; }
constexpr int kStagePitch = 1024;
constexpr int64_t kStageMaxRays = 8192;
static bool use_stage(int64_t N, int32_t sample_cap, int max_steps) {
  return use_coop(N, sample_cap) && N <= kStageMaxRays && max_steps <= kStagePitch;
}
static int64_t stage_offset_bytes(int64_t N, int32_t sample_cap) {
  const int w = cap_words_of(sample_cap);
  const int64_t b = ws_ints(N) * (int64_t)sizeof(int32_t) + (w ? N * (int64_t)(w + 1) * (int64_t)sizeof(uint32_t) : 0);
  return (b + 15) / 16 * 16;
}
int inr_march_write_fills_unowned_rows(int64_t N, int32_t sample_cap, int32_t max_steps) {
  return use_stage(N, sample_cap, max_steps) ? 1 : 0;
}
int64_t inr_march_workspace_bytes(int64_t N, int32_t sample_cap) {
  const int64_t base = stage_offset_bytes(N, sample_cap);
  return base + (N <= kStageMaxRays && sample_cap == 0 ? N * (int64_t)kStagePitch * 5 * (int64_t)sizeof(float) : 0);
}

static size_t march_lds_pad() { return (size_t)inr::g_march_lds_pad; }

int inr_march_rays_train_count(const float* rays_o, const float* rays_d, const uint8_t* bitfield, float bound,
                               float dt_gamma, int32_t max_steps, int64_t N, int32_t cascade, int32_t H,
                               const float* nears, const float* fars, const float* noises, int32_t* rays,
                               int32_t* counter, void* workspace, int32_t sample_cap, inr_stream_t s) {
  INR_REQUIRE(rays_o && rays_d && bitfield && nears && fars && rays && counter && workspace, "null pointer");
  INR_REQUIRE(N > 0 && N < (1ll << 31), "N out of range");
  INR_REQUIRE(max_steps > 0 && cascade >= 1 && H >= 8 && H <= 1024, "bad grid parameters");
  const MarchParams P = make_params(bitfield, bound, dt_gamma, max_steps, cascade, H);
  const unsigned nb = blocks_for(N, kRayBlock);
  INR_REQUIRE(sample_cap >= 0 && ((uintptr_t)workspace & 7) == 0, "workspace must be 8-byte aligned");
  int32_t* counts = reinterpret_cast<int32_t*>(workspace);
  int32_t* block_sums = counts + N;
  uint32_t* mask = reinterpret_cast<uint32_t*>(counts + ws_ints(N));
  hipStream_t st = as_stream(s);
  if (use_coop(N, sample_cap)) {
    float* stage = use_stage(N, sample_cap, max_steps)
                       ? reinterpret_cast<float*>(reinterpret_cast<char*>(workspace) + stage_offset_bytes(N, sample_cap)) : nullptr;
    k_march_count_coop<<<blocks_for(N, kCoopRaysPerBlock), kCoopRaysPerBlock * 64, 0, st>>>(P, rays_o, rays_d, N, max_steps,
                                                                                          nears, fars, noises, counts, stage,
                                                                                          kStagePitch);
    k_scan_counts<<<1, 1024, 0, st>>>(counts, N, rays, counter);
    return check_launch("march_rays_train_count");
  }
  k_march_count<<<nb, kRayBlock, march_lds_pad(), st>>>(P, rays_o, rays_d, N, max_steps, nears, fars, noises, counts, block_sums,
                                          mask, cap_words_of(sample_cap));
  k_scan_block_sums<<<1, 1024, 0, st>>>(block_sums, (int)nb, N, counter);
  k_finalize_offsets<<<nb, kRayBlock, 0, st>>>(counts, block_sums, N, rays);
  return check_launch("march_rays_train_count");
}

int inr_march_rays_train_write(const float* rays_o, const float* rays_d, const uint8_t* bitfield, float bound,
                               float dt_gamma, int32_t max_steps, int64_t N, int32_t cascade, int32_t H, int64_t M,
                               const float* nears, const float* fars, const float* noises, const int32_t* rays,
                               float* xyzs, float* dirs, float* deltas, const void* workspace, int32_t sample_cap,
                               inr_stream_t s) {
  INR_REQUIRE(rays_o && rays_d && bitfield && nears && fars && rays, "null pointer");
  INR_REQUIRE(N > 0 && M >= 0, "bad sizes");
  if (M == 0) return INR_OK;
  INR_REQUIRE(M == 0 || (xyzs && dirs && deltas), "null output");
  const MarchParams P = make_params(bitfield, bound, dt_gamma, max_steps, cascade, H);
  INR_REQUIRE(sample_cap == 0 || workspace, "sample_cap > 0 needs the workspace of the count pass");
  const uint32_t* mask = sample_cap > 0 ? reinterpret_cast<const uint32_t*>(reinterpret_cast<const int32_t*>(workspace) + ws_ints(N)) : nullptr;
  if (use_stage(N, sample_cap, max_steps)) {
    INR_REQUIRE(workspace, "the staged marcher needs the workspace of the count pass");
    const float* stage = reinterpret_cast<const float*>(reinterpret_cast<const char*>(workspace) + stage_offset_bytes(N, sample_cap));
    k_march_write_staged<<<blocks_for(N, kCoopRaysPerBlock), kCoopRaysPerBlock * 64, 0, as_stream(s)>>>(
        rays_d, N, M, rays, stage, kStagePitch, xyzs, dirs, deltas);
    return check_launch("march_rays_train_write");
  }
  if (use_coop(N, sample_cap)) {
    k_march_write_coop<<<blocks_for(N, kCoopRaysPerBlock), kCoopRaysPerBlock * 64, 0, as_stream(s)>>>(
        P, rays_o, rays_d, N, M, nears, fars, noises, rays, xyzs, dirs, deltas);
    return check_launch("march_rays_train_write");
  }
  k_march_write<<<blocks_for(N, kRayBlock), kRayBlock, 0, as_stream(s)>>>(P, rays_o, rays_d, N, M, nears, fars, noises,
                                                                          rays, xyzs, dirs, deltas, mask, cap_words_of(sample_cap));
  return check_launch("march_rays_train_write");
}

int inr_march_rays_patch_write(const float* rays_o, const float* rays_d, const uint8_t* bitfield, float bound,
                               float dt_gamma, int32_t max_steps, int64_t N, int32_t cascade, int32_t H, int64_t M,
                               const float* nears, const float* fars, const float* noises, const int32_t* rays,
                               float* xyzs, float* dirs, float* deltas, const void* workspace, int32_t sample_cap,
                               int32_t* ray_ids, int32_t normalise, inr_stream_t s) {
  INR_REQUIRE(rays_o && rays_d && bitfield && nears && fars && rays, "null pointer");
  INR_REQUIRE(N > 0 && M >= 0, "bad sizes");
  if (M == 0) return INR_OK;
  INR_REQUIRE(M == 0 || (xyzs && deltas && (dirs || ray_ids)), "null output");
  const MarchParams P = make_params(bitfield, bound, dt_gamma, max_steps, cascade, H);
  INR_REQUIRE(sample_cap == 0 || workspace, "sample_cap > 0 needs the workspace of the count pass");
  const uint32_t* mask = sample_cap > 0 ? reinterpret_cast<const uint32_t*>(reinterpret_cast<const int32_t*>(workspace) + ws_ints(N)) : nullptr;
  k_march_write_patch<<<blocks_for(N, kRayBlock), kRayBlock, march_lds_pad(), as_stream(s)>>>(P, rays_o, rays_d, N, M, nears, fars,
                                                                                noises, rays, xyzs, dirs, deltas, mask,
                                                                                cap_words_of(sample_cap), ray_ids, normalise);
  return check_launch("march_rays_patch_write");
}

int inr_composite_rays_patch_forward(const float* sigmas, const float* rgbs, const float* deltas, const int32_t* rays,
                                     int64_t N, int64_t M, float T_thresh, const float* extra, int32_t K,
                                     float* weights_sum, float* depth, float* image, float* extra_out,
                                     float* weights, uint64_t* skippable, inr_stream_t s) {
  INR_REQUIRE(N >= 0 && M >= 0, "bad sizes");
  if (N == 0) return INR_OK;
  INR_REQUIRE(rays && weights_sum && depth && image, "null pointer");
  INR_REQUIRE(M == 0 || (sigmas && rgbs && deltas), "null sample arrays");
  INR_REQUIRE(!extra || (extra_out && weights && K > 0 && K <= 64), "extra needs extra_out, weights and 0 < K <= 64");
  INR_REQUIRE(((uintptr_t)deltas & 7) == 0, "deltas must be 8-byte aligned");
  hipStream_t st = as_stream(s);
  k_composite_patch_fwd<<<blocks_for(N, kRayBlock), kRayBlock, 0, st>>>(sigmas, rgbs, deltas, rays, N, M, T_thresh,
                                                                        weights, weights_sum, depth, image,
                                                                        reinterpret_cast<unsigned long long*>(skippable));
  if (extra_out && K > 0)
    k_composite_patch_extra<<<blocks_for(N * 64, kRayBlock), kRayBlock, 0, st>>>(weights, extra, rays, N, M, K,
                                                                                 extra_out);
  return check_launch("composite_rays_patch_forward");
}

int inr_project_masks_patch(const float* xyzs, const float* weights, const int32_t* rays, int64_t N, int64_t M,
                            const uint32_t* mask_words, int32_t W, int32_t L, int32_t H, const float* bbox ,
                            int32_t k_total, int32_t k_base, int32_t k_count, float* out, inr_stream_t s) {
  INR_REQUIRE(N >= 0 && M >= 0 && W > 0 && L > 0 && H > 0, "bad sizes");
  INR_REQUIRE(k_total > 0 && k_base >= 0 && k_count > 0 && k_count <= 32 && k_base + k_count <= k_total, "bad mask range");
  if (N == 0) return INR_OK;
  INR_REQUIRE(rays && mask_words && bbox && out, "null pointer");
  INR_REQUIRE(M == 0 || (xyzs && weights), "null sample arrays");
  MaskVolume V;
  for (int a = 0; a < 3; ++a) { V.lo[a] = bbox[a]; V.hi[a] = bbox[3 + a]; }
  V.res[0] = (float)W; V.res[1] = (float)L; V.res[2] = (float)H;
  V.W = W; V.L = L; V.H = H;
  k_project_masks_patch<<<blocks_for(N, kRayBlock), kRayBlock, 0, as_stream(s)>>>(xyzs, weights, rays, N, M, mask_words, V,
                                                                                 k_total, k_base, k_count, out);
  return check_launch("project_masks_patch");
}

int inr_march_rays(int64_t n_alive, int32_t n_step, const int32_t* rays_alive, const float* rays_t,
                   const float* rays_o, const float* rays_d, float bound, float dt_gamma, int32_t max_steps,
                   int32_t cascade, int32_t H, const uint8_t* bitfield, const float* nears, const float* fars,
                   float* xyzs, float* dirs, float* deltas, inr_stream_t s) {
  (void)nears;
  INR_REQUIRE(rays_alive && rays_t && rays_o && rays_d && bitfield && fars && xyzs && dirs && deltas, "null pointer");
  INR_REQUIRE(n_alive >= 0 && n_step > 0, "bad sizes");
  if (n_alive == 0) return INR_OK;
  const MarchParams P = make_params(bitfield, bound, dt_gamma, max_steps, cascade, H);
  k_march_rays<<<blocks_for(n_alive, kRayBlock), kRayBlock, 0, as_stream(s)>>>(P, n_alive, n_step, rays_alive, rays_t,
                                                                               rays_o, rays_d, fars, xyzs, dirs, deltas);
  return check_launch("march_rays");
}

int inr_composite_rays(int64_t n_alive, int32_t n_step, int32_t* rays_alive, float* rays_t, const float* sigmas,
                       const float* rgbs, const float* deltas, float* weights_sum, float* depth, float* image,
                       float T_thresh, const float* extra, float* extra_acc, int32_t K, inr_stream_t s) {
  INR_REQUIRE(rays_alive && rays_t && sigmas && rgbs && deltas && weights_sum && depth && image, "null pointer");
  INR_REQUIRE(!extra || (extra_acc && K > 0), "extra given without extra_acc/K");
  if (n_alive == 0) return INR_OK;
  k_composite_rays<<<blocks_for(n_alive, kRayBlock), kRayBlock, 0, as_stream(s)>>>(
      n_alive, n_step, rays_alive, rays_t, sigmas, rgbs, deltas, weights_sum, depth, image, T_thresh, extra, extra_acc, K);
  return check_launch("composite_rays");
}

int inr_compact_alive(const int32_t* rays_alive, int64_t n_alive, int32_t* out, int32_t* n_out, inr_stream_t s) {
  INR_REQUIRE(rays_alive && out && n_out && n_alive >= 0, "bad argument");
  if (n_alive == 0) {
    (void)hipMemsetAsync(n_out, 0, 2 * sizeof(int32_t), as_stream(s));
    return check_launch("compact_alive");
  }
  const unsigned nb = blocks_for(n_alive, kRayBlock);
  int32_t* counts = out + n_alive;
  int32_t* block_sums = counts + n_alive;
  hipStream_t st = as_stream(s);
  k_alive_flags<<<nb, kRayBlock, 0, st>>>(rays_alive, n_alive, counts, block_sums);
  k_scan_block_sums<<<1, 1024, 0, st>>>(block_sums, (int)nb, n_alive, n_out);
  k_alive_scatter<<<nb, kRayBlock, 0, st>>>(rays_alive, n_alive, block_sums, out);
  return check_launch("compact_alive");
}

int inr_cross_entropy(const float* logits, const int64_t* labels, int64_t N, int32_t K, int64_t ignore_index,
                      float* grad_logits, float* acc, float* loss, inr_stream_t s) {
  INR_REQUIRE(N >= 0 && K > 0 && K <= 64, "K must be in 1..64");
  INR_REQUIRE(acc && loss && ((uintptr_t)acc & 7) == 0, "null or misaligned pointer");
  hipStream_t st = as_stream(s);
  int nb = 0;
  if (N > 0) {
    INR_REQUIRE(logits && labels && grad_logits, "null pointer");
    nb = (int)std::min<int64_t>((N + 3) / 4, kCeBlocks);
    k_ce_rows<<<nb, 256, 0, st>>>(logits, labels, N, K, ignore_index, grad_logits, reinterpret_cast<float2*>(acc));
  }
  const unsigned nb2 = (unsigned)std::max<int64_t>(1, std::min<int64_t>((N * K + 255) / 256, (int64_t)cu_count() * 4));
  k_ce_scale<<<nb2, 256, 0, st>>>(grad_logits, N * K, reinterpret_cast<const float2*>(acc), nb, loss);
  return check_launch("cross_entropy");
}

int inr_finish_rays(const float* image, const float* depth, const float* weights_sum, const float* nears,
                    const float* fars, const float* t0, float bg_r, float bg_g, float bg_b, int64_t N, float* image_out,
                    float* depth_out, inr_stream_t s) {
  INR_REQUIRE(N >= 0, "negative N");
  if (N == 0) return INR_OK;
  INR_REQUIRE(image && depth && weights_sum && nears && fars && image_out && depth_out, "null pointer");
  k_finish_rays<<<blocks_for(N, 256), 256, 0, as_stream(s)>>>(image, depth, weights_sum, nears, fars, t0, bg_r, bg_g, bg_b,
                                                              N, image_out, depth_out);
  return check_launch("finish_rays");
}

int inr_finish_rays_mse(const float* image, const float* depth, const float* weights_sum, const float* nears,
                        const float* fars, float bg_r, float bg_g, float bg_b, const float* bg_rays, const float* target,
                        int64_t N, float* image_out, float* depth_out, float* grad, float* loss, inr_stream_t s) {
  INR_REQUIRE(N > 0 && N <= INR_FINISH_MSE_MAX_RAYS, "N out of range (one workgroup: 0 < N <= INR_FINISH_MSE_MAX_RAYS)");
  INR_REQUIRE(image && depth && weights_sum && nears && fars && target && image_out && depth_out && grad && loss,
              "null pointer");
  k_finish_rays_mse<<<1, kFinishMseThreads, 0, as_stream(s)>>>(image, depth, weights_sum, nears, fars, bg_r, bg_g, bg_b,
                                                               bg_rays, target, N, image_out, depth_out, grad, loss);
  return check_launch("finish_rays_mse");
}

int inr_composite_rays_train_forward(const float* sigmas, const float* rgbs, const float* deltas, const int32_t* rays,
                                     int64_t N, int64_t M, float T_thresh, const float* extra, int32_t K,
                                     float* weights_sum, float* depth, float* image, float* extra_out, float* weights,
                                     int32_t* sample_ray, inr_stream_t s) {
  INR_REQUIRE(rays && weights_sum && depth && image && N >= 0 && M >= 0, "bad argument");
  INR_REQUIRE(!sample_ray || weights, "sample_ray needs weights");
  INR_REQUIRE(!extra || (extra_out && weights && K > 0 && K <= 64), "extra needs extra_out, weights and 0 < K <= 64");
  INR_REQUIRE(!extra_out || M == 0 || (extra && weights), "extra_out needs extra and weights");
  if (N == 0) return INR_OK;
  INR_REQUIRE(M == 0 || (sigmas && rgbs && deltas), "null sample arrays");
  INR_REQUIRE(((uintptr_t)deltas & 7) == 0, "deltas must be 8-byte aligned");
  hipStream_t st = as_stream(s);
  k_composite_train_fwd<<<blocks_for(N * 64, kRayBlock), kRayBlock, 0, st>>>(sigmas, rgbs, deltas, rays, N, M, T_thresh,
                                                                             weights_sum, depth, image, weights, sample_ray);
  if (extra_out && K > 0)
    k_composite_train_extra_fwd<<<blocks_for(N * 64, kRayBlock), kRayBlock, 0, st>>>(weights, extra, rays, N, M, K,
                                                                                     extra_out, CeArgs{});
  return check_launch("composite_rays_train_forward");
}

int inr_composite_rays_extra_forward(const float* weights, const float* extra, const int32_t* rays, int64_t N, int64_t M,
                                     int32_t K, float* extra_out, const int64_t* labels, int32_t n_classes,
                                     int64_t ignore_index, float* grad_pix, void* workspace, float* loss_out,
                                     inr_stream_t s) {
  INR_REQUIRE(rays && extra_out && N >= 0 && M >= 0 && K > 0 && K <= 64, "bad argument");
  INR_REQUIRE(!labels || (grad_pix && workspace && loss_out && n_classes > 0 && n_classes <= K),
              "labels need grad_pix, workspace, loss_out and 0 < n_classes <= K");
  INR_REQUIRE(((uintptr_t)workspace & 15) == 0, "workspace must be 16-byte aligned");
  if (N == 0) return INR_OK;
  INR_REQUIRE(M == 0 || (weights && extra), "null sample arrays");
  hipStream_t st = as_stream(s);
  CeArgs ce{};
  if (labels) ce = CeArgs{labels, n_classes, ignore_index, grad_pix, reinterpret_cast<float4*>(workspace)};
  k_composite_train_extra_fwd<<<blocks_for(N * 64, kRayBlock), kRayBlock, 0, st>>>(weights, extra, rays, N, M, K, extra_out, ce);
  if (labels) k_ce_finalize<<<1, 1024, 0, st>>>(reinterpret_cast<const float4*>(workspace), N, loss_out);
// ... 29 lines not shown
```

instance_nerf_amd/nerf/renderer.py:

```python
import math
import os

import torch
import torch.nn as nn

from .. import _lib, raymarching
from .._lib import check, ptr, stream_ptr


def sample_pdf(bins, weights, n_samples, det=False):
    weights = weights + 1e-5
    pdf = weights / torch.sum(weights, -1, keepdim=True)
    cdf = torch.cat([torch.zeros_like(pdf[..., :1]), torch.cumsum(pdf, -1)], -1)
    if det:
        u = torch.linspace(0.5 / n_samples, 1 - 0.5 / n_samples, steps=n_samples, device=weights.device)
        u = u.expand(list(cdf.shape[:-1]) + [n_samples])
    else:
        u = torch.rand(list(cdf.shape[:-1]) + [n_samples], device=weights.device)
    u = u.contiguous()
    inds = torch.searchsorted(cdf, u, right=True)
    below = torch.max(torch.zeros_like(inds - 1), inds - 1)
    above = torch.min((cdf.shape[-1] - 1) * torch.ones_like(inds), inds)
    cdf_g = torch.stack([torch.gather(cdf, 1, below), torch.gather(cdf, 1, above)], -1)
    bins_g = torch.stack([torch.gather(bins, 1, below), torch.gather(bins, 1, above)], -1)
    denom = cdf_g[..., 1] - cdf_g[..., 0]
    denom = torch.where(denom < 1e-5, torch.ones_like(denom), denom)
    t = (u - cdf_g[..., 0]) / denom
    return bins_g[..., 0] + t * (bins_g[..., 1] - bins_g[..., 0])


class NeRFRenderer(nn.Module):
    min_staged_batch = 1 << 20

    def __init__(self, bound=1, cuda_ray=False, density_scale=1, min_near=0.2, density_thresh=0.01,
                 bg_radius=-1, grid_size=128):
        super().__init__()
        self.bound = bound
        self.cascade = 1 + math.ceil(math.log2(bound))
        self.grid_size = grid_size
        self.density_scale = density_scale
        self.min_near = min_near
        self.density_thresh = density_thresh
        self.bg_radius = bg_radius
        if bg_radius > 0:
            raise NotImplementedError("background sphere model is outside the hot path (SURVEY.md section 2)")
        aabb = torch.tensor([-bound, -bound, -bound, bound, bound, bound], dtype=torch.float32)
        self.register_buffer("aabb_train", aabb)
        self.register_buffer("aabb_infer", aabb.clone())
        self.cuda_ray = cuda_ray
        if cuda_ray:
            self.register_buffer("density_grid", torch.zeros(self.cascade, grid_size ** 3))
            self.register_buffer("density_bitfield", torch.zeros(self.cascade * grid_size ** 3 // 8, dtype=torch.uint8))
            self.mean_density = 0
            self.iter_density = 0
            self.register_buffer("step_counter", torch.zeros(16, 2, dtype=torch.int32))
            self.mean_count = 0
            self.local_step = 0
            self.last_counter = None

    @property
    def mean_density(self):
        pending = self.__dict__.get("_mean_density_dev")
        if pending is not None:
            self.__dict__["_mean_density"] = float(pending[0].item())
            self.__dict__["_mean_density_dev"] = None
        return self.__dict__.get("_mean_density", 0)

    @mean_density.setter
    def mean_density(self, value):
        self.__dict__["_mean_density_dev"] = None
        self.__dict__["_mean_density"] = value

    def forward(self, x, d):
        raise NotImplementedError()

    def density(self, x):
        raise NotImplementedError()

    def color(self, x, d, mask=None, **kwargs):
        raise NotImplementedError()

    def density_sigma(self, x):
        return self.density(x)["sigma"]

    def instance(self, x):
        return None

    def reset_extra_state(self):
        if not self.cuda_ray:
            return
        self.density_grid.zero_()
        self.mean_density = 0
        self.iter_density = 0
        self.step_counter.zero_()
        self.mean_count = 0
        self.local_step = 0

    def run(self, rays_o, rays_d, num_steps=128, upsample_steps=128, bg_color=None, perturb=False, **kwargs):
        prefix = rays_o.shape[:-1]
        rays_o = rays_o.contiguous().view(-1, 3).float()
        rays_d = rays_d.contiguous().view(-1, 3).float()
        N, device = rays_o.shape[0], rays_o.device
        aabb = self.aabb_train if self.training else self.aabb_infer
        nears, fars = raymarching.near_far_from_aabb(rays_o, rays_d, aabb, self.min_near)
        hit = (fars > nears) & (fars < 3.0e38)
        nears = torch.where(hit, nears, torch.zeros_like(nears)).unsqueeze(-1)
        fars = torch.where(hit, fars, torch.ones_like(fars)).unsqueeze(-1)

        z_vals = torch.linspace(0.0, 1.0, num_steps, device=device).unsqueeze(0)
        z_vals = nears + (fars - nears) * z_vals
        sample_dist = (fars - nears) / num_steps
        if perturb:
            z_vals = z_vals + (torch.rand(z_vals.shape, device=device) - 0.5) * sample_dist

        def positions(z):
            x = rays_o.unsqueeze(-2) + rays_d.unsqueeze(-2) * z.unsqueeze(-1)
            return torch.min(torch.max(x, aabb[:3]), aabb[3:])

        def weights_of(z, sigma):
            deltas = torch.cat([z[..., 1:] - z[..., :-1], sample_dist * torch.ones_like(z[..., :1])], dim=-1)
            alphas = 1 - torch.exp(-deltas * self.density_scale * sigma)
            shifted = torch.cat([torch.ones_like(alphas[..., :1]), 1 - alphas + 1e-15], dim=-1)
            return alphas * torch.cumprod(shifted, dim=-1)[..., :-1], deltas

        xyzs = positions(z_vals)
        den = {k: v.view(N, num_steps, -1) for k, v in self.density(xyzs.reshape(-1, 3)).items()}
        if upsample_steps > 0:
            with torch.no_grad():
                weights, deltas = weights_of(z_vals, den["sigma"].squeeze(-1))
                z_mid = z_vals[..., :-1] + 0.5 * deltas[..., :-1]
                new_z = sample_pdf(z_mid, weights[:, 1:-1], upsample_steps, det=not self.training).detach()
                new_xyzs = positions(new_z)
            new_den = {k: v.view(N, upsample_steps, -1) for k, v in self.density(new_xyzs.reshape(-1, 3)).items()}
            z_vals, order = torch.sort(torch.cat([z_vals, new_z], dim=1), dim=1)
            xyzs = torch.gather(torch.cat([xyzs, new_xyzs], dim=1), 1, order.unsqueeze(-1).expand(-1, -1, 3))
            den = {k: torch.gather(torch.cat([den[k], new_den[k]], dim=1), 1,
                                   order.unsqueeze(-1).expand(-1, -1, den[k].shape[-1])) for k in den}
        weights, _ = weights_of(z_vals, den["sigma"].squeeze(-1))
        weights = weights * hit.unsqueeze(-1)
        T = z_vals.shape[1]
        dirs = rays_d.unsqueeze(-2).expand(-1, T, -1)
        mask = (weights > 1e-4).reshape(-1)
        rgbs = self.color(xyzs.reshape(-1, 3), dirs.reshape(-1, 3), mask=mask,
                          geo_feat=den["geo_feat"].reshape(-1, den["geo_feat"].shape[-1])).view(N, T, 3)
        weights_sum = weights.sum(dim=-1)
        depth = torch.sum(weights * ((z_vals - nears) / (fars - nears)).clamp(0, 1), dim=-1)
        image = torch.sum(weights.unsqueeze(-1) * rgbs, dim=-2)
        if bg_color is None:
            bg_color = 1
        image = image + (1 - weights_sum).unsqueeze(-1) * bg_color
        results = {"image": image.view(*prefix, 3), "depth": depth.view(*prefix), "weights_sum": weights_sum.view(*prefix)}
        if getattr(self, "num_instances", 0) > 0:
            logits = self.instance(xyzs.reshape(-1, 3)).view(N, T, -1)
            results["instance"] = torch.sum(weights.detach().unsqueeze(-1) * logits, dim=-2).view(*prefix, -1)
        return results

    def _instance_for_compositing(self, x):
        return self.instance(x)

    def run_cuda(self, rays_o, rays_d, dt_gamma=0, bg_color=None, perturb=False, force_all_rays=False,
                 max_steps=1024, T_thresh=1e-4, infer_mode="auto", noises=None, field_gate=None, ce_labels=None,
                 ce_ignore_index=-1, mse_target=None, marched=None, ce_prune=False, **kwargs):
        prefix = rays_o.shape[:-1]
        rays_o = rays_o.contiguous().view(-1, 3).float()
        rays_d = rays_d.contiguous().view(-1, 3).float()
        N = rays_o.shape[0]
        device = rays_o.device
        aabb = self.aabb_train if self.training else self.aabb_infer
        if marched is not None and not (self.training and marched["n_rays"] == N
                                        and marched.get("grid_state", self.iter_density) == self.iter_density):
            self.drop_ahead(marched)
            marched = None
        if marched is not None:
            marched["consume"]()
            nears, fars = marched["nears"], marched["fars"]
        elif self.training and ce_prune and ce_labels is not None:
            nears, fars = raymarching.near_far_from_aabb(rays_o, rays_d, aabb, self.min_near, skip_labels=ce_labels,
                                                         ignore_index=ce_ignore_index)
        else:
            nears, fars = raymarching.near_far_from_aabb(rays_o, rays_d, aabb, self.min_near)
        if bg_color is None:
            bg_color = 1
        results = {}
        skipped_frac = None
        with_instance = getattr(self, "num_instances", 0) > 0
        if not self.training and infer_mode == "auto":
            infer_mode = "fused_terminate" if self._recent_skippable() > self.terminate_above else "fused"

        fused_inst = with_instance and getattr(self, "_fusable_inst", False) and hasattr(self, "instance_render")
        if (not self.training and infer_mode == "fused_terminate" and getattr(self, "_fusable", False)
                and (fused_inst or not with_instance)):
            counter = torch.zeros(2, dtype=torch.int32, device=device)
            xyzs, _, deltas, rays = raymarching.march_rays_patch(
                rays_o, rays_d, self.bound, self.density_bitfield, self.cascade, self.grid_size, nears, fars,
                dt_gamma, max_steps, noises=noises if perturb else None, counter=counter, table=True)
            if field_gate is not None:
                field_gate.acquire()
            weights_sum, depth, image, wbuf, evaluated = self.nerf_render(xyzs, deltas, rays, rays_d, T_thresh,
                                                                          want_weights=with_instance, normalised=True)
            if field_gate is not None:
                field_gate.release()
            if with_instance:
                if field_gate is not None:
                    field_gate.acquire()
                results["instance"] = self.instance_render(xyzs, rays, wbuf, normalised=True).view(*prefix, -1)
                if field_gate is not None:
                    field_gate.release()
            results["num_samples"] = counter
            results["num_evaluated"] = evaluated
            skipped_frac = (evaluated, int(xyzs.shape[0]), True)
        elif not self.training and infer_mode in ("fused", "fused_terminate"):
            counter = torch.zeros(2, dtype=torch.int32, device=device)
            table = (fused_inst or not with_instance) and getattr(self, "_fusable", False) and hasattr(self, "forward_table")
            early = {}

            def while_waiting():
                early["skippable"] = torch.zeros(1, dtype=torch.int64, device=device)
                if table and hasattr(self, "sh_table"):
                    early["shq"] = self.sh_table(rays_d)
            xyzs, dirs, deltas, rays = raymarching.march_rays_patch(
                rays_o, rays_d, self.bound, self.density_bitfield, self.cascade, self.grid_size, nears, fars,
                dt_gamma, max_steps, noises=noises if perturb else None, counter=counter, table=table,
                while_waiting=while_waiting)
            if field_gate is not None:
                field_gate.acquire()
            sigmas, rgbs = self.forward_table(xyzs, dirs, rays_d, shq=early.get("shq")) if table else self(xyzs, dirs)
            if field_gate is not None:
                field_gate.release()
            if self.density_scale != 1:
                sigmas = self.density_scale * sigmas
            skippable = early["skippable"]
            if fused_inst:
                weights_sum, depth, image, wbuf = raymarching.composite_rays_patch(sigmas, rgbs, deltas, rays, T_thresh,
                                                                                  return_weights=True, skippable=skippable)
                if field_gate is not None:
                    field_gate.acquire()
                results["instance"] = self.instance_render(xyzs, rays, wbuf, normalised=table).view(*prefix, -1)
                if field_gate is not None:
                    field_gate.release()
            else:
                extra = self._instance_for_compositing(xyzs) if with_instance else None
                out = raymarching.composite_rays_patch(sigmas, rgbs, deltas, rays, T_thresh, extra=extra,
                                                       skippable=skippable)
                weights_sum, depth, image = out[0], out[1], out[2]
                if with_instance:
                    results["instance"] = out[3][:, :self.num_instances].reshape(*prefix, -1)
            results["num_samples"] = counter
            if table:
                results["frame_path"] = getattr(self, "last_frame_path", "fused")
            skipped_frac = (skippable, int(xyzs.shape[0]), False)
        elif self.training or infer_mode == "fused_raymajor":
            if marched is not None:
                counter = marched["counter"]
                xyzs, dirs, deltas, rays = marched["xyzs"], marched["dirs"], marched["deltas"], marched["rays"]
            else:
                if self.training:
                    counter = self.step_counter[self.local_step % 16]
                    self.local_step += 1
                    mean_count = self.mean_count
                else:
                    counter = torch.zeros(2, dtype=torch.int32, device=device)
                    mean_count = -1
                    force_all_rays = True
                xyzs, dirs, deltas, rays = raymarching.march_rays_train(
                    rays_o, rays_d, self.bound, self.density_bitfield, self.cascade, self.grid_size, nears, fars,
                    counter, mean_count, perturb, 128, force_all_rays, dt_gamma, max_steps, noises=noises)
            if self.training:
                self.last_counter = counter
            head = with_instance and getattr(self, "instance_head_available", lambda x: False)(xyzs)
            shaded = None
            if (marched is not None and marched.get("shaded") is not None and head and self.shade_ahead_applies()
                    and marched["T_thresh"] == float(T_thresh) and marched["density_scale"] == float(self.density_scale)):
                shaded = marched["shaded"]
            else:
                sigmas, rgbs = self(xyzs, dirs)
                if self.density_scale != 1:
                    sigmas = self.density_scale * sigmas
            if head:
                weights_sum, depth, image, wbuf, sample_ray = shaded if shaded is not None else raymarching.composite_rays_train(
                    sigmas, rgbs, deltas, rays, T_thresh, return_weights=True, total_dev=counter)
                if ce_labels is not None:
                    inst, results["instance_ce"] = self.instance_head_train(
                        xyzs, wbuf, sample_ray, rays, n_dev=counter, ce_labels=ce_labels.reshape(-1),
                        ce_ignore_index=ce_ignore_index)
                else:
                    inst = self.instance_head_train(xyzs, wbuf, sample_ray, rays, n_dev=counter)
                results["instance"] = inst[:, :self.num_instances].reshape(*prefix, -1)
            else:
                extra = self._instance_for_compositing(xyzs) if with_instance else None
                out = raymarching.composite_rays_train(sigmas, rgbs, deltas, rays, T_thresh, extra=extra,
                                                       total_dev=counter)
                weights_sum, depth, image = out[0], out[1], out[2]
                if with_instance:
                    results["instance"] = out[3][:, :self.num_instances].reshape(*prefix, -1)
            results["num_samples"] = counter
        elif infer_mode == "wavefront":
            dtype = torch.float32
            weights_sum = torch.zeros(N, dtype=dtype, device=device)
            depth = torch.zeros(N, dtype=dtype, device=device)
            image = torch.zeros(N, 3, dtype=dtype, device=device)
            K = getattr(self, "num_instances", 0)
            inst = torch.zeros(N, K, dtype=dtype, device=device) if with_instance else None
            n_alive = N
            rays_alive = torch.arange(n_alive, dtype=torch.int32, device=device)
            rays_t = nears.clone()
            step = 0
            evaluated = 0
            while step < max_steps and n_alive > 0:
                n_step = max(min(N // n_alive, 8), 1)
                xyzs, dirs, deltas = raymarching.march_rays(n_alive, n_step, rays_alive, rays_t, rays_o, rays_d,
                                                            self.bound, self.density_bitfield, self.cascade,
                                                            self.grid_size, nears, fars, 128, perturb, dt_gamma,
                                                            max_steps)
                sigmas, rgbs = self(xyzs, dirs)
                sigmas = self.density_scale * sigmas
                extra = self.instance(xyzs) if with_instance else None
                raymarching.composite_rays(n_alive, n_step, rays_alive, rays_t, sigmas, rgbs, deltas, weights_sum,
                                           depth, image, T_thresh, extra=extra, extra_acc=inst)
                evaluated += n_alive * n_step
                rays_alive, n_alive = raymarching.compact_alive(rays_alive, n_alive)
                step += n_step
            if with_instance:
                results["instance"] = inst.view(*prefix, -1)
        else:
            raise ValueError(f"unknown infer_mode {infer_mode!r}")

        if not self.training and skipped_frac is not None:
            self._note_skippable(*skipped_frac)
        t_start = None
        if not self.training and infer_mode in ("fused", "fused_terminate", "fused_raymajor"):
            t_start = nears
            if perturb and noises is not None:
                dt_min = 2 * math.sqrt(3) / max_steps
                dt_max = 2 * math.sqrt(3) * 2 ** (self.cascade - 1) / self.grid_size
                t_start = nears + torch.clamp(nears * dt_gamma, dt_min, dt_max) * noises.to(nears)
        bg3 = self._bg_triplet(bg_color)
        flows = torch.is_grad_enabled() and (image.requires_grad or weights_sum.requires_grad)
        bg_per_ray = torch.is_tensor(bg_color) and bg_color.is_cuda and bg_color.numel() == 3 * N
        if (self.training and mse_target is not None and flows and t_start is None and image.is_cuda
                and 0 < N <= raymarching.FINISH_MSE_MAX_RAYS and (bg3 is not None or bg_per_ray)):
            image, depth, results["image_mse"] = raymarching.finish_rays_mse(
                image, weights_sum, depth, nears, fars, bg3 if bg3 is not None else bg_color, mse_target)
        elif bg3 is not None and not (torch.is_grad_enabled() and (image.requires_grad or weights_sum.requires_grad)):
            lib = _lib.load()
            src_i, src_d = image.detach().contiguous(), depth.detach().contiguous()
            image = torch.empty_like(src_i) if self.training else src_i
            depth = torch.empty_like(src_d) if self.training else src_d
            check(lib.inr_finish_rays(ptr(src_i, torch.float32, "image"), ptr(src_d, torch.float32, "depth"),
                                      ptr(weights_sum.detach().contiguous(), torch.float32, "weights_sum"),
                                      ptr(nears, torch.float32, "nears"), ptr(fars, torch.float32, "fars"),
                                      ptr(t_start, torch.float32, "t0", allow_none=True),
                                      bg3[0], bg3[1], bg3[2], N, ptr(image), ptr(depth), stream_ptr()), "finish_rays")
        else:
            if isinstance(bg_color, (list, tuple)):
                bg_color = image.new_tensor(bg_color)
            image = image + (1 - weights_sum).unsqueeze(-1) * bg_color
            if t_start is not None:
                depth = depth + t_start * weights_sum.detach()
            depth = torch.clamp(depth - nears, min=0) / (fars - nears)
        results["image"] = image.view(*prefix, 3)
        results["depth"] = depth.view(*prefix)
        results["weights_sum"] = weights_sum.view(*prefix)
        return results

    terminate_above = 0.50

    def _note_skippable(self, counter, total, counts_evaluated):
        if not counter.is_cuda:
            v = float(counter.reshape(-1)[0]) / max(total, 1)
            self._skippable_value = 1.0 - v if counts_evaluated else v
            return
        d = self.__dict__
        if "_skippable_free" not in d:
            d["_skippable_free"] = [torch.empty(1, dtype=torch.int64, pin_memory=True) for _ in range(4)]
            d["_skippable_pending"] = []
        self._recent_skippable()
        if not d["_skippable_free"]:
            return
        host = d["_skippable_free"].pop()
        host.copy_(counter.reshape(-1)[:1].view(torch.int64), non_blocking=True)
        ev = torch.cuda.Event()
        ev.record()
        d["_skippable_pending"].append((ev, host, total, counts_evaluated))

# ... 21 lines not shown
            return
        if not torch.is_tensor(poses):
            poses = torch.as_tensor(poses)
        dev = self.density_grid.device
        poses = poses.to(dev).float().contiguous().view(-1, 16)
        fx, fy, cx, cy = [float(v) for v in intrinsic]
        check(_lib.load().inr_mark_untrained_grid(ptr(poses, torch.float32, "poses", allow_none=poses.shape[0] == 0),
                                                  poses.shape[0], fx, fy, cx, cy, self.grid_size, self.cascade,
                                                  float(self.bound), ptr(self.density_grid, torch.float32, "density_grid"),
                                                  stream_ptr()), "mark_untrained_grid")

    def shade_ahead_applies(self):
        if not (getattr(self, "num_instances", 0) > 0 and getattr(self, "_fusable", False)
                and hasattr(self, "_nerf_params") and hasattr(self, "instance_head_train")):
            return False
        if any(p.requires_grad for p in self._nerf_params()):
            return False
        inst = [self.instance_encoder.embeddings] + [l.weight for l in self.instance_net]
        return bool(self._fusable_inst and self.fused_instance_train and self.fused_instance_head
                    and all(p.requires_grad for p in inst))

    @torch.no_grad()
    def march_ahead(self, rays_o, rays_d, dt_gamma=0, perturb=False, max_steps=1024, stream=None, shade=False,
                    T_thresh=1e-4, bufs=None, counter=None, skip_labels=None, ignore_index=-1):
        if not (self.cuda_ray and self.training and self.mean_count > 0 and rays_o.is_cuda):
            return None
        rays_o_in, rays_d_in = rays_o, rays_d
        rays_o = rays_o.contiguous().view(-1, 3).float()
        rays_d = rays_d.contiguous().view(-1, 3).float()
        N = rays_o.shape[0]
        if not _lib.load().inr_march_write_fills_unowned_rows(N, raymarching.SAMPLE_CAP_TRAIN, int(max_steps)):
            return None
        shade = bool(shade) and self.shade_ahead_applies()
        main = torch.cuda.current_stream()
        side = stream if stream is not None else main
        if side is not main:
            side.wait_stream(main)
        M_al = (int(self.mean_count) + 127) // 128 * 128
        if bufs is not None:
            b = bufs
            if b["n_rays"] != N or b["n_samples"] < M_al or (shade and "sigmas" not in b):
                raise RuntimeError("march_ahead(bufs=): buffer set of another batch size")
        else:
            own = getattr(self, "_ahead_bufs", None)
            if (own is None or own[0]["n_rays"] != N or own[0]["n_samples"] != M_al or own[0]["nears"].device != rays_o.device
                    or (shade and "sigmas" not in own[0])):
                own = self._ahead_bufs = [raymarching.march_train_buffers(N, M_al, rays_o.device, shade=shade) for _ in range(2)]
                self._ahead_turn = 0
            b = own[self._ahead_turn]
            self._ahead_turn ^= 1
        slot_taken = counter is None
        slot_index = -1
        if counter is None:
            slot_index = self.local_step % 16
            counter = self.step_counter[slot_index]
            self.local_step += 1
        with torch.cuda.stream(side):
            nears, fars = raymarching.near_far_from_aabb(rays_o, rays_d, self.aabb_train, self.min_near,
                                                         out=(b["nears"], b["fars"]), skip_labels=skip_labels,
                                                         ignore_index=ignore_index)
            xyzs, dirs, deltas, rays = raymarching.march_rays_train(
                rays_o, rays_d, self.bound, self.density_bitfield, self.cascade, self.grid_size, nears, fars,
                counter, self.mean_count, perturb, 128, False, dt_gamma, max_steps, out=b)
            shaded = None
            if shade:
                M = xyzs.shape[0]
                sigmas, rgbs = b["sigmas"][:M], b["rgbs"][:M]
                self._fused_nerf(xyzs, dirs, True, False, out=(sigmas, rgbs))
                if self.density_scale != 1:
                    sigmas.mul_(self.density_scale)
                shaded = raymarching.composite_rays_train_into(sigmas, rgbs, deltas, rays, T_thresh, b)
            done = None
            if side is not main:
                done = torch.cuda.Event()
                done.record(side)
        out = {"n_rays": N, "key": (rays_o.data_ptr(), rays_d.data_ptr(), N), "rays_o": rays_o_in, "rays_d": rays_d_in,
               "nears": nears, "fars": fars, "xyzs": xyzs, "dirs": dirs, "deltas": deltas, "rays": rays, "counter": counter,
               "shaded": shaded, "T_thresh": float(T_thresh), "density_scale": float(self.density_scale),
               "slot_taken": slot_taken, "slot_index": slot_index, "grid_state": self.iter_density,
               "skip_labels": skip_labels}

        def consume():
            cur = torch.cuda.current_stream()
            if done is not None and side is not cur:
                cur.wait_event(done)
        out["consume"] = consume
        return out

    def drop_ahead(self, marched):
        if marched is not None and marched.get("slot_taken") and self.local_step > 0:
            if marched.get("slot_index", -1) == (self.local_step - 1) % 16:
                self.local_step -= 1
            marched["slot_taken"] = False

    @torch.no_grad()
    def update_extra_state(self, decay=0.95, S=128):
        if not self.cuda_ray:
            return
        lib = _lib.load()
        dev = self.density_bitfield.device
        H, C = self.grid_size, self.cascade
        n_cells = H ** 3
        st = stream_ptr()
        total_step = min(16, self.local_step)
        counted = None
        if total_step > 0:
            host = self.__dict__.get("_count_host")
            if host is None:
                host = self.__dict__["_count_host"] = torch.empty(1, dtype=torch.int64).pin_memory()
            host.copy_(self.step_counter[:total_step, 0].sum(0, keepdim=True, dtype=torch.int64), non_blocking=True)
            counted = torch.cuda.Event()
            counted.record()
        mean_sum = torch.zeros(1, dtype=torch.float64, device=dev)
        grid = self.density_grid
        full = self.iter_density < 16
        for cas in range(C):
            bnd = float(min(2 ** cas, self.bound))
            if full:
                idx, m = None, n_cells
            else:
                n = n_cells // 4
                u = torch.rand(4 * n, dtype=torch.float32, device=dev)
                idx = torch.empty(2 * n, dtype=torch.int32, device=dev)
                work = torch.empty(lib.inr_occ_sample_workspace_bytes(n_cells) // 8 + 1, dtype=torch.int64, device=dev)
                check(lib.inr_occ_sample_cells(ptr(grid[cas], torch.float32, "density_grid"), n_cells, ptr(u), n, ptr(idx),
                                               ptr(work), st), "occ_sample_cells")
                m = 2 * n
            xyz = torch.empty(m, 3, dtype=torch.float32, device=dev)
            noise = torch.rand_like(xyz)
            check(lib.inr_occ_cell_positions(ptr(idx, torch.int32, "morton_idx", allow_none=True),
                                             ptr(noise, torch.float32, "noise"), m, H, bnd, ptr(xyz), st),
                  "occ_cell_positions")
            sigma = self.density_sigma(xyz).reshape(-1).detach().float().contiguous()
            tmp = None if full else torch.empty(n_cells, dtype=torch.float32, device=dev)
            check(lib.inr_occ_update(ptr(grid[cas], torch.float32, "density_grid"), ptr(sigma, torch.float32, "sigma"),
                                     ptr(idx, torch.int32, "morton_idx", allow_none=True), n_cells, m, float(decay),
                                     float(self.density_scale), ptr(tmp, allow_none=True), ptr(mean_sum), st),
                  "occ_update")
        stats = torch.empty(2, dtype=torch.float64, device=dev)
        check(lib.inr_packbits_mean(ptr(grid, torch.float32, "density_grid"), C * n_cells, ptr(mean_sum),
                                    float(self.density_thresh), ptr(self.density_bitfield, torch.uint8, "density_bitfield"),
                                    None, ptr(self.step_counter, torch.int32, "step_counter"), max(total_step, 1),
                                    self.step_counter.stride(0), ptr(stats), st), "packbits_mean")
        self.iter_density += 1
        self.__dict__["_mean_density_dev"] = stats
        if counted is not None:
            counted.synchronize()
            self.mean_count = int(float(host[0]) / total_step)
        self.local_step = 0

    def render(self, rays_o, rays_d, staged=False, max_ray_batch=4096, **kwargs):
        _run = self.run_cuda if self.cuda_ray else self.run
        B, N = rays_o.shape[:2]
        if self.cuda_ray:
            max_ray_batch = max(int(max_ray_batch), int(self.min_staged_batch))
        if staged and N > max_ray_batch:
            if not self.training and kwargs.get("infer_mode", "auto") == "auto":
                kwargs = dict(kwargs, infer_mode="fused_terminate" if self._recent_skippable() > self.terminate_above else "fused")
            chunks = {}
            for b in range(B):
                head = 0
                while head < N:
                    tail = min(head + max_ray_batch, N)
                    r = _run(rays_o[b:b + 1, head:tail], rays_d[b:b + 1, head:tail], **kwargs)
                    for k, v in r.items():
                        if torch.is_tensor(v) and v.dim() >= 2 and v.shape[:2] == (1, tail - head):
                            chunks.setdefault((k, b), []).append(v)
                    head += max_ray_batch
            keys = sorted({k for k, _ in chunks})
            n_chunks = (N + max_ray_batch - 1) // max_ray_batch
            keys = [k for k in keys if all(len(chunks.get((k, b), ())) == n_chunks for b in range(B))]
            return {k: torch.cat([torch.cat(chunks[(k, b)], 1) for b in range(B)], 0) for k in keys}
        return _run(rays_o, rays_d, **kwargs)


class FramePipeline:

    def __init__(self, net, device=None):
        self.net = net
        self.streams = [torch.cuda.Stream(device=device), torch.cuda.Stream(device=device)]
        self._turn = 0
        self._field_done = None
        self.open()

    def open(self):
        raymarching.set_overlap_placement(os.environ.get("INR_PIPELINE_PLACEMENT", "1") != "0")

    def acquire(self):
        if self._field_done is not None:
            torch.cuda.current_stream().wait_event(self._field_done)

    def release(self):
        self._field_done = torch.cuda.Event()
        self._field_done.record(torch.cuda.current_stream())

    def next_stream(self):
        st = self.streams[self._turn]
        self._turn ^= 1
        return st

    def render(self, rays_o, rays_d, stream=None, **kwargs):
        if kwargs.pop("staged", False):
            raise RuntimeError("FramePipeline renders a whole view per call (staged=False)")
        if stream is None:
            stream = self.next_stream()
            stream.wait_stream(torch.cuda.current_stream())
            rays_o.record_stream(stream)
            rays_d.record_stream(stream)
        with torch.cuda.stream(stream):
            out = self.net.render(rays_o, rays_d, staged=False, field_gate=self, **kwargs)
        out["stream"] = stream
        return out

    def synchronize(self):
        for st in self.streams:
            st.synchronize()

    def close(self):
        self.synchronize()
        raymarching.set_overlap_placement(False)

    def __enter__(self):
        return self

    def __exit__(self, *exc):
        self.close()
        return False
```

instance_nerf_amd/nerf/utils.py:

```python
import math
import os
import time

import numpy as np
import torch
import torch.distributed as dist

from .. import _lib


_PATCH_INDS = {}


SUPER_TILE = int(os.environ.get("INR_SUPER_TILE", "0"))


def patch_order(H, W, patch, device, super_tile=None):
    st = SUPER_TILE if super_tile is None else super_tile
    key = (H, W, patch, st, str(device))
    if key not in _PATCH_INDS:
        jj, ii = torch.meshgrid(torch.arange(H), torch.arange(W), indexing="ij")
        ii, jj = ii.reshape(-1), jj.reshape(-1)
        npx = (W + patch - 1) // patch
        k = ((jj // patch) * npx + (ii // patch))
        if st:
            nsx = (W + st - 1) // st
            pps = st // patch
            k = ((jj // st) * nsx + (ii // st)) * (pps * pps) + ((jj % st) // patch) * pps + ((ii % st) // patch)
        k = k * (patch * patch) + (jj % patch) * patch + (ii % patch)
        _PATCH_INDS[key] = torch.argsort(k).to(device)
    return _PATCH_INDS[key]


@torch.no_grad()
def get_rays(poses, intrinsics, H, W, N=-1, error_map=None, inds=None, patch=0):
    device = poses.device
    B = poses.shape[0]
    fx, fy, cx, cy = intrinsics
    if inds is None and N > 0 and error_map is not None:
        inds_coarse = torch.multinomial(error_map.to(device), N, replacement=False)
        cx_, cy_ = torch.div(inds_coarse, 128, rounding_mode="floor"), inds_coarse % 128
        sx, sy = H / 128, W / 128
        px = (cx_ * sx + torch.rand(B, N, device=device) * sx).long().clamp(max=H - 1)
        py = (cy_ * sy + torch.rand(B, N, device=device) * sy).long().clamp(max=W - 1)
        per_batch = px * W + py
        parts = [get_rays(poses[b:b + 1], intrinsics, H, W, inds=per_batch[b]) for b in range(B)]
        return {"rays_o": torch.cat([p["rays_o"] for p in parts]), "rays_d": torch.cat([p["rays_d"] for p in parts]),
                "inds": per_batch, "inds_coarse": inds_coarse}
    if inds is None:
        if N > 0:
            inds = torch.randint(0, H * W, size=[N], device=device)
        elif patch:
            inds = patch_order(H, W, patch, device)
        else:
            inds = torch.arange(H * W, device=device)
    inds = inds.contiguous().long()
    n = inds.shape[0]
    if poses.is_cuda:
        lib = _lib.load()
        poses = poses.contiguous().float()
        rays_o = torch.empty(B, n, 3, dtype=torch.float32, device=device)
        rays_d = torch.empty(B, n, 3, dtype=torch.float32, device=device)
        _lib.check(lib.inr_get_rays(_lib.ptr(poses, torch.float32, "poses"), B, float(fx), float(fy), float(cx), float(cy),
                                    int(W), _lib.ptr(inds, torch.int64, "inds", allow_none=n == 0), n,
                                    _lib.ptr(rays_o, allow_none=B * n == 0), _lib.ptr(rays_d, allow_none=B * n == 0),
                                    _lib.stream_ptr()), "get_rays")
        return {"rays_o": rays_o, "rays_d": rays_d, "inds": inds[None].expand(B, -1)}
    i = (inds % W).float() + 0.5
    j = torch.div(inds, W, rounding_mode="floor").float() + 0.5
    xs = (i - cx) / fx
    ys = (j - cy) / fy
    zs = torch.ones_like(xs)
    d = torch.stack([xs, ys, zs], -1)
    d = d / torch.sqrt(d[:, 0] * d[:, 0] + d[:, 1] * d[:, 1] + d[:, 2] * d[:, 2]).unsqueeze(-1)
    R = poses[:, :3, :3].float()
    rays_d = (d[None, :, None, 0] * R[:, None, :, 0] + d[None, :, None, 1] * R[:, None, :, 1]
              + d[None, :, None, 2] * R[:, None, :, 2])
    rays_o = poses[:, None, :3, 3].float().expand_as(rays_d).contiguous()
    return {"rays_o": rays_o, "rays_d": rays_d.contiguous(), "inds": inds[None].expand(B, -1)}


def seed_everything(seed):
    import random
    random.seed(seed)
    os.environ["PYTHONHASHSEED"] = str(seed)
    np.random.seed(seed)
    torch.manual_seed(seed)
    if torch.cuda.is_available():
        torch.cuda.manual_seed(seed)


def linear_to_srgb(x):
    return torch.where(x < 0.0031308, 12.92 * x, 1.055 * x.clamp(min=0.0031308) ** 0.41666 - 0.055)


def srgb_to_linear(x):
    return torch.where(x < 0.04045, x / 12.92, ((x.clamp(min=0.04045) + 0.055) / 1.055) ** 2.4)


class PSNRMeter:
    def __init__(self):
        self.V, self.N = 0.0, 0

    def clear(self):
        self.V, self.N = 0.0, 0

    def update(self, preds, truths):
        mse = torch.mean((preds.detach().float() - truths.detach().float()) ** 2).item()
        self.V += -10 * math.log10(max(mse, 1e-12))
        self.N += 1

    def measure(self):
        return self.V / max(self.N, 1)

    def report(self):
        return f"PSNR = {self.measure():.6f}"


class MIoUMeter:

    def __init__(self, num_classes):
        self.K = num_classes
        self.clear()

    def clear(self):
        self.inter = torch.zeros(self.K, dtype=torch.float64)
        self.union = torch.zeros(self.K, dtype=torch.float64)
        self.truth = torch.zeros(self.K, dtype=torch.float64)

    def update(self, pred_ids, true_ids):
        p, t = pred_ids.reshape(-1).cpu(), true_ids.reshape(-1).cpu()
        keep = t >= 0
        p, t = p[keep], t[keep]
        for k in range(self.K):
            pk, tk = p == k, t == k
            self.inter[k] += (pk & tk).sum()
            self.union[k] += (pk | tk).sum()
            self.truth[k] += tk.sum()

    def measure(self, all_predicted=False):
        present = self.union > 0 if all_predicted else self.truth > 0
        return float((self.inter[present] / self.union[present]).mean()) if present.any() else 0.0

    def measure_both(self):
        return {"miou_gt_ids": self.measure(False), "miou_all_ids": self.measure(True)}

    def report(self):
        b = self.measure_both()
        return f"mIoU = {b['miou_gt_ids']:.6f} (over ground-truth ids; {b['miou_all_ids']:.6f} counting ids only predicted)"


class FusedAdam(torch.optim.Optimizer):

    def __init__(self, params, lr=1e-2, betas=(0.9, 0.99), eps=1e-15):
        super().__init__(params, dict(lr=lr, betas=tuple(betas), eps=eps))
        self.step_count = 0
        self._ema = None

    @property
    def betas(self):
        return tuple(self.param_groups[0]["betas"])

    @property
    def eps(self):
        return self.param_groups[0]["eps"]

    def _moments(self, p):
        st = self.state[p]
        if "exp_avg" not in st:
            st["step"] = torch.tensor(float(self.step_count))
            st["exp_avg"] = torch.zeros_like(p.data)
            st["exp_avg_sq"] = torch.zeros_like(p.data)
        return st

    def state_dict(self):
        for st in self.state.values():
            if "exp_avg" in st:
                st["step"] = torch.tensor(float(self.step_count))
        return super().state_dict()

    def load_state_dict(self, sd):
        if "param_groups" not in sd:
            flat = [p for g in self.param_groups for p in g["params"]]
            for g, lr in zip(self.param_groups, sd["lrs"]):
                g["lr"] = lr
            for i, (m, v) in sd["state"].items():
                p = flat[int(i)]
                self.state[p] = {"step": torch.tensor(float(sd["step"])), "exp_avg": m.to(p.device), "exp_avg_sq": v.to(p.device)}
            self.step_count = int(sd["step"])
            return
        super().load_state_dict(sd)
        steps = [int(float(st["step"])) for st in self.state.values() if "step" in st]
        self.step_count = max(steps) if steps else 0
        for p, st in self.state.items():
            for k in ("exp_avg", "exp_avg_sq"):
                if k in st:
                    st[k] = st[k].to(p.device, torch.float32).contiguous()

    def _jobs(self):
        jobs = []
        for g in self.param_groups:
            for p in g["params"]:
                if not p.requires_grad:
                    continue
                pieces = getattr(p, "_inr_grad_shards", None)
                if pieces:
                    st = self._moments(p)
                    flat = lambda t: t.view(-1)
                    for piece in pieces:
                        a, n = piece["own"], piece["grad"].numel()
                        if n == 0:
                            continue
                        jobs.append((flat(p.data)[a:a + n], piece["grad"], flat(st["exp_avg"])[a:a + n],
                                     flat(st["exp_avg_sq"])[a:a + n], g, p, (a, n)))
                    continue
                if p.grad is None:
                    continue
# ... 415 lines not shown
                                      _lib.stream_ptr()), "copy_multi")


class Trainer:

    def __init__(self, name, opt, model, criterion=None, optimizer=None, ema_decay=None, lr_scheduler=None, metrics=None,
                 local_rank=0, world_size=1, device=None, mute=False, fp16=False, eval_interval=1, max_keep_ckpt=2,
                 workspace="workspace", best_mode="min", use_loss_as_metric=True, report_metric_at_train=False,
                 use_checkpoint="latest", use_tensorboardX=True, scheduler_update_every_step=False, *,
                 lr=1e-2, iters=30000, fused_adam=True, stage="nerf", update_extra_interval=None, use_graph=False,
                 look_ahead=False, shade_ahead=None, prune_ignored=True, fixed_point_grad=None):
        self.name, self.opt, self.model = name, opt, model
        self.world_size, self.local_rank = world_size, local_rank
        grad_sync.world_size = world_size
        self.device = device or (torch.device("cuda", local_rank) if torch.cuda.is_available() else torch.device("cpu"))
        self.stage = stage
        self.workspace = workspace
        self.mute, self.fp16 = mute, bool(fp16)
        if self.fp16 and hasattr(model, "half_table"):
            model.half_table = True
            model.mlp_fp16 = True
        self.metrics = list(metrics) if metrics else []
        self.eval_interval, self.max_keep_ckpt = eval_interval, max_keep_ckpt
        self.best_mode, self.use_loss_as_metric = best_mode, use_loss_as_metric
        self.report_metric_at_train = report_metric_at_train
        self.scheduler_update_every_step = scheduler_update_every_step
        if update_extra_interval is None:
            update_extra_interval = getattr(opt, "update_extra_interval", 16) if opt is not None else 16
        self.update_extra_interval = update_extra_interval
        self._default_criterion = criterion is None
        self.criterion = criterion or (torch.nn.MSELoss(reduction="none") if stage == "nerf" else None)
        model.to(self.device)
        if stage == "instance":
            model.freeze_nerf()
        if optimizer is not None:
            self.optimizer = optimizer(self.model)
        else:
            groups = [{"params": [p for p in g["params"] if p.requires_grad], "lr": g["lr"]} for g in model.get_params(lr)]
            groups = [g for g in groups if g["params"]]
            if fused_adam and self.device.type == "cuda":
                self.optimizer = FusedAdam(groups, lr=lr, betas=(0.9, 0.99), eps=1e-15)
            else:
                self.optimizer = torch.optim.Adam(groups, lr=lr, betas=(0.9, 0.99), eps=1e-15)
        grad_sync.sharded_ok = isinstance(self.optimizer, FusedAdam) and world_size > 1 and not use_graph
        self._ahead, self._side_stream = None, None
        self.look_ahead = bool(look_ahead)
        self.shade_ahead = bool(use_graph and look_ahead) if shade_ahead is None else bool(shade_ahead)
        self.pipe_fork = os.environ.get("INR_PIPE_FORK", "scatter")
        self.prune_ignored = bool(prune_ignored)
        if fixed_point_grad is not None:
            from . import network as _network
            _network.FX_GRAD = 64 if fixed_point_grad == 64 else (32 if fixed_point_grad else 0)
        self.iters = iters
        self.lr_scheduler = lr_scheduler(self.optimizer) if lr_scheduler is not None else None
        trained = [p for g in self.optimizer.param_groups for p in g["params"] if p.requires_grad]
        self.ema = ParamEMA(trained, ema_decay) if ema_decay is not None else None
        self.base_lrs = [g["lr"] for g in self.optimizer.param_groups]
        self.use_graph = (bool(use_graph) and world_size == 1 and isinstance(self.optimizer, FusedAdam)
                          and self.lr_scheduler is None)
        if self.ema is not None and isinstance(self.optimizer, FusedAdam):
            self.optimizer.attach_ema(self.ema)
        self._graph = None
        self._pipe = None
        self.global_step = 0
        self.local_step = 0
        self.epoch = 0
        self.stats = {"loss": [], "valid_loss": [], "results": [], "checkpoints": [], "best_result": None}
        self.bg_color = 1
        self.log_ptr = None
        self.ckpt_path = self.best_path = None
        if self.workspace is not None:
            self.ckpt_path = os.path.join(self.workspace, "checkpoints")
            self.best_path = os.path.join(self.ckpt_path, f"{self.name}.pth")
        if self.workspace is not None and use_checkpoint != "scratch":
            if use_checkpoint in ("latest", "latest_model"):
                self.load_checkpoint(model_only=use_checkpoint == "latest_model")
            elif use_checkpoint == "best":
                if self.best_path and os.path.exists(self.best_path):
                    self.load_checkpoint(self.best_path)
                else:
                    self.load_checkpoint()
            else:
                self.load_checkpoint(use_checkpoint)

    def log(self, *args, **kwargs):
        if self.local_rank == 0 and not self.mute:
            print(*args, **kwargs)

    def _lr_step(self):
        if self.lr_scheduler is not None:
            return
        f = 0.1 ** min(self.global_step / self.iters, 1)
        for g, b in zip(self.optimizer.param_groups, self.base_lrs):
            g["lr"] = b * f

    def _render_kwargs(self):
        return vars(self.opt) if self.opt is not None else {}

    def train_step(self, data):
        bg_color = self.bg_color
        gt = None
        if self.stage == "nerf":
            images = data["images"]
            gt = images
            if images.shape[-1] == 4:
                bg_color = torch.rand_like(images[..., :3])
                gt = images[..., :3] * images[..., 3:] + bg_color * (1 - images[..., 3:])
        extra = {}
        if self.stage == "instance" and getattr(self.model, "cuda_ray", False) and data["rays_o"].is_cuda:
            extra["ce_labels"] = data["masks"]
            extra["ce_prune"] = self.prune_ignored
        if (self.stage == "nerf" and self._default_criterion and getattr(self.model, "cuda_ray", False)
                and data["rays_o"].is_cuda):
            extra["mse_target"] = gt
        ahead = self._ahead
        if ahead is not None:
            self._ahead = None
            if (ahead["rays_o"] is data["rays_o"] and ahead["rays_d"] is data["rays_d"]
                    and ahead.get("skip_labels") is self._skip_labels(data)):
                extra["marched"] = ahead
            elif hasattr(self.model, "drop_ahead"):
                self.model.drop_ahead(ahead)
        outputs = self.model.render(data["rays_o"], data["rays_d"], staged=False, bg_color=bg_color, perturb=True,
                                    force_all_rays=False, **extra, **self._render_kwargs())
        if self.stage == "nerf":
            pred = outputs["image"]
            loss = outputs["image_mse"] if "image_mse" in outputs else self.criterion(pred, gt).mean()
            return pred, gt, loss
        logits = outputs["instance"]
        K = logits.shape[-1]
        if "instance_ce" in outputs:
            loss = outputs["instance_ce"]
        elif logits.is_cuda and K <= 64 and logits.dtype == torch.float32:
            from .. import raymarching
            loss = raymarching.cross_entropy(logits.reshape(-1, K), data["masks"].reshape(-1), ignore_index=-1)
        else:
            loss = torch.nn.functional.cross_entropy(logits.reshape(-1, K), data["masks"].reshape(-1).long(), ignore_index=-1)
        return logits, data["masks"], loss

    @staticmethod
    def _as_image(t, data, channels=None):
        if "H" in data and "W" in data and t.dim() >= 2 and t.shape[1] == int(data["H"]) * int(data["W"]):
            tail = t.shape[2:]
            return t.reshape(t.shape[0], int(data["H"]), int(data["W"]), *tail)
        return t

    def _render_view(self, data, **kwargs):
        rays_o, rays_d = data["rays_o"], data["rays_d"]
        H, W = int(data.get("H", 0) or 0), int(data.get("W", 0) or 0)
        if not (getattr(self.model, "cuda_ray", False) and rays_o.is_cuda and rays_o.dim() == 3 and H * W == rays_o.shape[1]
                and H % 4 == 0 and W % 4 == 0):
            return self.model.render(rays_o, rays_d, **kwargs)
        inds = patch_order(H, W, 4, rays_o.device)
        out = self.model.render(rays_o[:, inds].contiguous(), rays_d[:, inds].contiguous(), **kwargs)
        for k, v in list(out.items()):
            if torch.is_tensor(v) and v.dim() >= 2 and v.shape[1] == H * W:
                back = torch.empty_like(v)
                back[:, inds] = v
                out[k] = back
        return out

    @torch.no_grad()
    def eval_step(self, data):
        outputs = self._render_view(data, staged=True, bg_color=self.bg_color, perturb=False, **self._render_kwargs())
        return self._eval_outputs(data, outputs)

    def _eval_outputs(self, data, outputs):
        if self.stage == "nerf":
            images = data["images"]
            flat = images.reshape(images.shape[0], -1, images.shape[-1])
            gt = flat[..., :3] * flat[..., 3:] + self.bg_color * (1 - flat[..., 3:]) if flat.shape[-1] == 4 else flat
            loss = self.criterion(outputs["image"], gt).mean()
            return (self._as_image(outputs["image"], data), self._as_image(outputs["depth"], data),
                    self._as_image(gt, data), loss)
        logits = outputs["instance"]
        K = logits.shape[-1]
        masks = data["masks"].reshape(logits.shape[0], -1)
        loss = torch.nn.functional.cross_entropy(logits.reshape(-1, K), masks.reshape(-1).long(), ignore_index=-1)
        return (self._as_image(logits.argmax(-1), data), self._as_image(outputs["depth"], data),
                self._as_image(masks, data), loss)

    @torch.no_grad()
    def test_step(self, data, bg_color=None, perturb=False):
        outputs = self._render_view(data, staged=True, bg_color=self.bg_color if bg_color is None else bg_color,
                                    perturb=perturb, **self._render_kwargs())
        return self._test_outputs(data, outputs)

    def _test_outputs(self, data, outputs):
        inst = outputs.get("instance")
        return (self._as_image(outputs["image"], data), self._as_image(outputs["depth"], data),
                None if inst is None else self._as_image(inst, data))

    pipeline_views = True

    @torch.no_grad()
    def render_sequence(self, loader, pipeline=None, **kwargs):
        kw = dict(staged=True, bg_color=self.bg_color, perturb=False)
        kw.update(self._render_kwargs())
        kw.update(kwargs)
        use = self.pipeline_views if pipeline is None else bool(pipeline)
        use = use and getattr(self.model, "cuda_ray", False) and self.device.type == "cuda"
        if not use:
            for data in loader:
                yield data, self._render_view(data, **kw)
            return
        from .renderer import FramePipeline
        pipe = self.__dict__.get("_frame_pipe")
        if pipe is None or pipe.net is not self.model:
            pipe = self.__dict__["_frame_pipe"] = FramePipeline(self.model, self.device)
        pipe.open()
        try:
            pending = None
            for data in loader:
                cur = torch.cuda.current_stream()
                st = pipe.next_stream()
                st.wait_stream(cur)
                for k in ("rays_o", "rays_d"):
                    if torch.is_tensor(data.get(k)) and data[k].is_cuda:
                        data[k].record_stream(st)
                with torch.cuda.stream(st):
                    out = self._render_view(data, field_gate=pipe, **kw)
                    done = torch.cuda.Event()
                    done.record(st)
                if pending is not None:
                    yield self._finish_view(*pending)
                pending = (data, out, done)
            if pending is not None:
                yield self._finish_view(*pending)
        finally:
            pipe.close()

    @staticmethod
    def _finish_view(data, out, done):
        done.synchronize()
        cur = torch.cuda.current_stream()
        for v in out.values():
            if torch.is_tensor(v) and v.is_cuda:
                v.record_stream(cur)
        return data, out

    GRAPH_ALIGN = 16384

    def _graph_capacity(self, mean_count):
        a = self.GRAPH_ALIGN
        need = (mean_count + a - 1) // a * a
        held = getattr(self, "_held_capacity", 0)
        if need <= held <= need + max(2 * a, need // 8):
            need = held
        self._held_capacity = need
        return need

    def _graph_key(self, data):
        return (self.model.mean_count, self.stage) + tuple((k, tuple(v.shape)) for k, v in sorted(data.items())
                                                            if torch.is_tensor(v))

    def _capture(self, data):
        m = self.model
        static = {k: (v.clone() if torch.is_tensor(v) else v) for k, v in data.items()}
        slot = m.local_step % 16
        opt = self.optimizer
        for g in opt.param_groups:
            for p in g["params"]:
                if p.requires_grad:
                    opt._moments(p)
                    if getattr(p, "_is_hash_table", False):
                        from . import network as _network
                        _network.fx_state(p)
                        if _network.fx_bits() == 64:
                            _network.fx_acc64(p)
        opt.hyper_tensor(self.device)
        self.optimizer.zero_grad()
        torch.cuda.synchronize()
        g = torch.cuda.CUDAGraph()
        with torch.cuda.graph(g):
            _, _, loss = self.train_step(static)
            loss.backward()
            self.optimizer.step_captured()
        m.local_step -= 1
        self._graph = {"graph": g, "static": static, "loss": loss, "slot": slot, "key": self._graph_key(data)}

    def _replay(self, data):
        G, m = self._graph, self.model
        copy_tensors([(G["static"][k], v) for k, v in data.items() if torch.is_tensor(v)])
        self._lr_step()
        self.optimizer.refresh_hyper()
        G["graph"].replay()
        cur = m.local_step % 16
        if cur != G["slot"]:
            m.step_counter[cur].copy_(m.step_counter[G["slot"]])
        m.local_step += 1
        self.optimizer.bump_versions()
        if self.ema is not None:
            self.ema.update()
        return G["loss"].detach()

    def _pipe_applies(self, data):
        m = self.model
        if not (self.use_graph and self.look_ahead and m.cuda_ray and m.mean_count > 0 and data["rays_o"].is_cuda
                and hasattr(m, "march_ahead")):
            return False
        from .. import raymarching
        kw = self._render_kwargs()
        return bool(_lib.load().inr_march_write_fills_unowned_rows(data["rays_o"].numel() // 3, raymarching.SAMPLE_CAP_TRAIN,
                                                                    int(kw.get("max_steps", 1024))))

    def _pipe_args(self):
        kw = self._render_kwargs()
        return dict(dt_gamma=kw.get("dt_gamma", 0), perturb=True, max_steps=kw.get("max_steps", 1024),
                    shade=self.stage == "instance" and self.shade_ahead, T_thresh=kw.get("T_thresh", 1e-4))

    def _skip_labels(self, data):
        return data["masks"] if (self.stage == "instance" and self.prune_ignored and "masks" in data) else None

# ... 447 lines not shown
```

instance_nerf_amd/raymarching.py:

```python
import math

import torch

from . import _lib
from ._lib import check, ptr, stream_ptr

F32, I32, U8 = torch.float32, torch.int32, torch.uint8

SAMPLE_CAP = int(__import__("os").environ.get("INR_SAMPLE_CAP", "1024"))
SAMPLE_CAP_TRAIN = int(__import__("os").environ.get("INR_SAMPLE_CAP_TRAIN", "0"))


def _f(t):
    return t.contiguous().float() if (t.dtype != F32 or not t.is_contiguous()) else t


def set_overlap_placement(on):
    check(_lib.load().inr_set_overlap_placement(1 if on else 0), "set_overlap_placement")


def set_march_mode(mode):
    code = {None: -1, "auto": -1, "lane_per_ray": 0, "wave_per_ray": 1}[mode]
    check(_lib.load().inr_set_march_mode(code), "set_march_mode")

# ... 41 lines not shown
    check(lib.inr_morton3D(ptr(coords, I32, "coords"), N, ptr(out), stream_ptr()), "morton3D")
    return out


def morton3D_invert(indices):
    lib = _lib.load()
    indices = indices.int().contiguous()
    N = indices.shape[0]
    out = torch.empty(N, 3, dtype=I32, device=indices.device)
    check(lib.inr_morton3D_invert(ptr(indices, I32, "indices"), N, ptr(out), stream_ptr()), "morton3D_invert")
    return out


def packbits(grid, thresh, bitfield=None):
    lib = _lib.load()
    grid = _f(grid)
    n = grid.numel()
    if n % 8:
        raise RuntimeError("packbits: number of cells must be a multiple of 8")
    if bitfield is None:
        bitfield = torch.empty(n // 8, dtype=U8, device=grid.device)
    check(lib.inr_packbits(ptr(grid, F32, "grid"), n // 8, float(thresh), ptr(bitfield, U8, "bitfield"),
                           stream_ptr()), "packbits")
    return bitfield


def march_train_buffers(n_rays, n_samples, device, shade=False):
    lib = _lib.load()
    b = {"n_rays": n_rays, "n_samples": n_samples,
         "nears": torch.empty(n_rays, dtype=F32, device=device), "fars": torch.empty(n_rays, dtype=F32, device=device),
         "noises": torch.empty(n_rays, dtype=F32, device=device), "rays": torch.empty(n_rays, 3, dtype=I32, device=device),
         "ws": torch.empty(lib.inr_march_workspace_bytes(n_rays, SAMPLE_CAP_TRAIN) // 8 + 1, dtype=torch.int64, device=device),
         "buf": torch.empty(n_samples * 8, dtype=F32, device=device)}
    if shade:
        b.update({"sigmas": torch.empty(n_samples, dtype=F32, device=device),
                  "rgbs": torch.empty(n_samples, 3, dtype=F32, device=device),
                  "weights_sum": torch.empty(n_rays, dtype=F32, device=device),
                  "depth": torch.empty(n_rays, dtype=F32, device=device),
                  "image": torch.empty(n_rays, 3, dtype=F32, device=device),
                  "weights": torch.empty(n_samples, dtype=F32, device=device),
                  "sample_ray": torch.empty(n_samples, dtype=I32, device=device)})
    return b


def march_rays_train(rays_o, rays_d, bound, density_bitfield, C, H, nears, fars, step_counter=None,
                     mean_count=-1, perturb=False, align=-1, force_all_rays=False, dt_gamma=0, max_steps=1024,
                     noises=None, separate_buffers=False, out=None):
    lib = _lib.load()
    rays_o, rays_d = _f(rays_o).view(-1, 3), _f(rays_d).view(-1, 3)
    dev = rays_o.device
    N = rays_o.shape[0]
    nears, fars = _f(nears), _f(fars)
    if noises is None:
        if not perturb:
            noises = None
        elif out is not None:
            noises = torch.rand(N, dtype=F32, device=dev, out=out["noises"])
        else:
            noises = torch.rand(N, dtype=F32, device=dev)
    else:
        noises = _f(noises)
    if step_counter is None:
        step_counter = torch.zeros(2, dtype=I32, device=dev)
    cap = SAMPLE_CAP_TRAIN
    if out is not None:
        if force_all_rays or mean_count <= 0 or out["n_rays"] != N or out["n_samples"] < int(mean_count):
            raise RuntimeError("march_rays_train(out=) needs the steady state and buffers of the batch's size")
        rays, ws = out["rays"], out["ws"]
    else:
        rays = torch.empty(N, 3, dtype=I32, device=dev)
        ws = torch.empty(lib.inr_march_workspace_bytes(N, cap) // 8 + 1, dtype=torch.int64, device=dev)
    args = (ptr(rays_o, F32, "rays_o"), ptr(rays_d, F32, "rays_d"), ptr(density_bitfield, U8, "density_bitfield"),
            float(bound), float(dt_gamma), int(max_steps), N, int(C), int(H))
    check(lib.inr_march_rays_train_count(*args, ptr(nears, F32, "nears"), ptr(fars, F32, "fars"),
                                         ptr(noises, F32, "noises", allow_none=True), ptr(rays),
                                         ptr(step_counter, I32, "step_counter"), ptr(ws), cap, stream_ptr()),
          "march_rays_train_count")
    if force_all_rays or mean_count <= 0:
        M = int(step_counter[0].item())
    else:
        M = int(mean_count)
    if align > 0:
        M += align - M % align if M % align else 0
    alloc = torch.empty if lib.inr_march_write_fills_unowned_rows(N, cap, int(max_steps)) else torch.zeros
    if out is not None:
        if alloc is not torch.empty or M > out["n_samples"]:
            raise RuntimeError("march_rays_train(out=) needs the staged marcher (it clears unowned rows itself)")
        buf = out["buf"]
        xyzs, dirs, deltas = buf[:M * 3].view(M, 3), buf[M * 3:M * 6].view(M, 3), buf[M * 6:M * 8].view(M, 2)
    elif separate_buffers:
        xyzs, dirs, deltas = (alloc(M, 3, dtype=F32, device=dev), alloc(M, 3, dtype=F32, device=dev),
                              alloc(M, 2, dtype=F32, device=dev))
    else:
        buf = alloc(M * 8, dtype=F32, device=dev)
        xyzs, dirs, deltas = buf[:M * 3].view(M, 3), buf[M * 3:M * 6].view(M, 3), buf[M * 6:].view(M, 2)
    check(lib.inr_march_rays_train_write(*args, M, ptr(nears), ptr(fars), ptr(noises, F32, "noises", allow_none=True),
                                         ptr(rays), ptr(xyzs), ptr(dirs), ptr(deltas), ptr(ws), cap, stream_ptr()),
          "march_rays_train_write")
    return xyzs, dirs, deltas, rays


GROUP = 16


_PINNED_COUNT = {}


def _read_count(counter, while_waiting=None):
    key = counter.device.index
    host = _PINNED_COUNT.get(key)
    if host is None:
        host = _PINNED_COUNT[key] = torch.empty(2, dtype=I32, pin_memory=True)
    host.copy_(counter[:2], non_blocking=True)
    ev = torch.cuda.Event()
    ev.record()
    if while_waiting is not None:
        while_waiting()
    ev.synchronize()
    return int(host[0])


def march_rays_patch(rays_o, rays_d, bound, density_bitfield, C, H, nears, fars, dt_gamma=0, max_steps=1024,
                     noises=None, counter=None, table=False, while_waiting=None):
    lib = _lib.load()
    rays_o, rays_d = _f(rays_o).view(-1, 3), _f(rays_d).view(-1, 3)
    dev = rays_o.device
    N = rays_o.shape[0]
    nears, fars = _f(nears), _f(fars)
    noises = _f(noises) if noises is not None else None
    if counter is None:
        counter = torch.zeros(2, dtype=I32, device=dev)
    rays = torch.empty(N, 3, dtype=I32, device=dev)
    cap = SAMPLE_CAP
    ws = torch.empty(lib.inr_march_workspace_bytes(N, cap) // 8 + 1, dtype=torch.int64, device=dev)
    args = (ptr(rays_o, F32, "rays_o"), ptr(rays_d, F32, "rays_d"), ptr(density_bitfield, U8, "density_bitfield"),
            float(bound), float(dt_gamma), int(max_steps), N, int(C), int(H))
    check(lib.inr_march_rays_train_count(*args, ptr(nears, F32, "nears"), ptr(fars, F32, "fars"),
                                         ptr(noises, F32, "noises", allow_none=True), ptr(rays),
                                         ptr(counter, I32, "counter"), ptr(ws), cap, stream_ptr()),
          "march_rays_train_count")
    M = _read_count(counter, while_waiting)
    xyzs = torch.empty(M, 3, dtype=F32, device=dev)
    dirs = None if table else torch.empty(M, 3, dtype=F32, device=dev)
    ray_ids = torch.empty(M, dtype=I32, device=dev) if table else None
    deltas = torch.empty(M, 2, dtype=F32, device=dev)
    check(lib.inr_march_rays_patch_write(*args, M, ptr(nears), ptr(fars), ptr(noises, F32, "noises", allow_none=True),
                                         ptr(rays), ptr(xyzs, allow_none=M == 0), ptr(dirs, allow_none=True),
                                         ptr(deltas, allow_none=M == 0), ptr(ws), cap,
                                         ptr(ray_ids, allow_none=True), 1 if table else 0, stream_ptr()),
          "march_rays_patch_write")
    return xyzs, (ray_ids if table else dirs), deltas, rays


def composite_rays_patch(sigmas, rgbs, deltas, rays, T_thresh=1e-4, extra=None, return_weights=False, skippable=None):
    lib = _lib.load()
    sigmas, rgbs, deltas = _f(sigmas), _f(rgbs), _f(deltas)
    dev = rays.device
    N, M = rays.shape[0], sigmas.shape[0]
    K = 0 if extra is None else extra.shape[1]
    ws = torch.empty(N, dtype=F32, device=dev)
    depth = torch.empty(N, dtype=F32, device=dev)
    image = torch.empty(N, 3, dtype=F32, device=dev)
    extra_out = torch.empty(N, K, dtype=F32, device=dev) if K else None
    wbuf = torch.empty(max(M, 1), dtype=F32, device=dev) if (K or return_weights) else None
    none_ok = M == 0
    check(lib.inr_composite_rays_patch_forward(
        ptr(sigmas, F32, "sigmas", allow_none=none_ok), ptr(rgbs, F32, "rgbs", allow_none=none_ok),
        ptr(deltas, F32, "deltas", allow_none=none_ok), ptr(rays, I32, "rays"), N, M, float(T_thresh),
        ptr(_f(extra) if extra is not None else None, allow_none=True), K, ptr(ws), ptr(depth), ptr(image),
        ptr(extra_out, allow_none=True), ptr(wbuf, allow_none=True), ptr(skippable, torch.int64, "skippable", allow_none=True),
        stream_ptr()), "composite_rays_patch_forward")
    out = (ws, depth, image) + ((extra_out,) if K else ())
    return out + ((wbuf,) if return_weights else ())


def patch_slots(rays):
    r = rays.cpu().long()
    N = r.shape[0]
    cnt, off = r[:, 2], r[:, 1]
    pad = (-N) % GROUP
    c = torch.cat([cnt, torch.zeros(pad, dtype=torch.long)]).view(-1, GROUP)
    base = torch.cat([off, torch.zeros(pad, dtype=torch.long)]).view(-1, GROUP)[:, 0]
    out = []
    for g in range(c.shape[0]):
        cg = c[g]
        kmax = int(cg.max())
        if kmax == 0:
            continue
        k = torch.arange(kmax)[:, None]
        act = cg[None, :] > k
        nact = act.sum(1)
        S = base[g] + torch.cat([torch.zeros(1, dtype=torch.long), nact.cumsum(0)[:-1]])
        rank = act.long().cumsum(1) - act.long()
        slot = S[:, None] + rank
        for i in range(GROUP):
            out.append(slot[: int(cg[i]), i])
    return torch.cat(out) if out else torch.zeros(0, dtype=torch.long)


class _CompositeRaysTrain(torch.autograd.Function):
    @staticmethod
    def forward(ctx, sigmas, rgbs, extra, deltas, rays, T_thresh, want_weights=False, total_dev=None):
        lib = _lib.load()
        sigmas, rgbs, deltas = _f(sigmas), _f(rgbs), _f(deltas)
        dev = sigmas.device
        N = rays.shape[0]
        K = 0 if extra is None else extra.shape[1]
        if extra is not None:
            extra = _f(extra)
        ws = torch.empty(N, dtype=F32, device=dev)
        depth = torch.empty(N, dtype=F32, device=dev)
        image = torch.empty(N, 3, dtype=F32, device=dev)
        extra_out = torch.empty(N, K, dtype=F32, device=dev) if K else None
        wbuf = torch.empty(sigmas.shape[0], dtype=F32, device=dev) if (K or want_weights) else None
        sample_ray = torch.empty(sigmas.shape[0], dtype=I32, device=dev) if want_weights else None
        check(lib.inr_composite_rays_train_forward(
            ptr(sigmas, F32, "sigmas"), ptr(rgbs, F32, "rgbs"), ptr(deltas, F32, "deltas"), ptr(rays, I32, "rays"),
            N, sigmas.shape[0], float(T_thresh), ptr(extra, F32, "extra", allow_none=True), K, ptr(ws), ptr(depth),
            ptr(image),
            ptr(extra_out, allow_none=True), ptr(wbuf, allow_none=True), ptr(sample_ray, allow_none=True), stream_ptr()),
            "composite_rays_train_forward")
        ctx.save_for_backward(sigmas, rgbs, extra, deltas, rays, ws, image, wbuf, total_dev)
        ctx.T_thresh = T_thresh
        ctx.K = K
        ctx.set_materialize_grads(False)
        if ctx.needs_input_grad[0] or ctx.needs_input_grad[1]:
            ctx.mark_non_differentiable(depth)
        else:
            ctx.mark_non_differentiable(depth, ws, image)
        out = (ws, depth, image) + ((extra_out,) if K else ())
        if want_weights:
            ctx.mark_non_differentiable(wbuf, sample_ray)
            out = out + (wbuf, sample_ray)
        ctx.n_out = len(out)
        return out

    @staticmethod
    def backward(ctx, g_ws, g_depth, g_image, *rest):
        g_extra = rest[0] if ctx.K else None
        lib = _lib.load()
        sigmas, rgbs, extra, deltas, rays, ws, image, wbuf, total_dev = ctx.saved_tensors
        N = rays.shape[0]
        K = ctx.K
        dev = sigmas.device
        need_field = ctx.needs_input_grad[0] or ctx.needs_input_grad[1]
        gs = gc = None
        if need_field:
            g_ws = _f(g_ws) if g_ws is not None else None
            g_image = _f(g_image) if g_image is not None else torch.zeros(N, 3, dtype=F32, device=dev)
            alloc = torch.empty_like if total_dev is not None else torch.zeros_like
            gs = alloc(sigmas)
            gc = alloc(rgbs)
        ge = None
        if K and g_extra is not None and ctx.needs_input_grad[2]:
            g_extra = _f(g_extra)
            ge = torch.zeros_like(extra)
        else:
            g_extra = None
        if need_field or ge is not None:
            check(lib.inr_composite_rays_train_backward(
                ptr(g_ws, allow_none=True) if need_field else None, ptr(g_image) if need_field else None,
                ptr(g_extra, allow_none=True), ptr(sigmas), ptr(rgbs),
                ptr(extra, allow_none=True), ptr(deltas), ptr(rays), ptr(ws), ptr(image), ptr(wbuf, allow_none=True), N,
                sigmas.shape[0], float(ctx.T_thresh), K, ptr(gs, allow_none=True), ptr(gc, allow_none=True),
                ptr(ge, allow_none=True), ptr(total_dev, I32, "total_dev", allow_none=True), stream_ptr()),
                "composite_rays_train_backward")
        return gs, gc, ge, None, None, None, None, None


@torch.no_grad()
def composite_rays_train_into(sigmas, rgbs, deltas, rays, T_thresh, out):
    lib = _lib.load()
    N, M = rays.shape[0], sigmas.shape[0]
    ws, depth, image = out["weights_sum"], out["depth"], out["image"]
    wbuf, sample_ray = out["weights"][:M], out["sample_ray"][:M]
    check(lib.inr_composite_rays_train_forward(
        ptr(sigmas, F32, "sigmas"), ptr(rgbs, F32, "rgbs"), ptr(deltas, F32, "deltas"), ptr(rays, I32, "rays"),
        N, M, float(T_thresh), None, 0, ptr(ws), ptr(depth), ptr(image), None, ptr(wbuf), ptr(sample_ray), stream_ptr()),
        "composite_rays_train_forward")
    return ws, depth, image, wbuf, sample_ray


def composite_rays_train(sigmas, rgbs, deltas, rays, T_thresh=1e-4, extra=None, return_weights=False, total_dev=None):
    return _CompositeRaysTrain.apply(sigmas, rgbs, extra, deltas, rays, T_thresh, bool(return_weights), total_dev)


def march_rays(n_alive, n_step, rays_alive, rays_t, rays_o, rays_d, bound, density_bitfield, C, H, near, far,
               align=-1, perturb=False, dt_gamma=0, max_steps=1024):
    lib = _lib.load()
    rays_o, rays_d = _f(rays_o).view(-1, 3), _f(rays_d).view(-1, 3)
    dev = rays_o.device
    M = n_alive * n_step
    if align > 0 and M % align:
        M += align - M % align
    xyzs = torch.zeros(M, 3, dtype=F32, device=dev)
    dirs = torch.zeros(M, 3, dtype=F32, device=dev)
    deltas = torch.zeros(M, 2, dtype=F32, device=dev)
    check(lib.inr_march_rays(n_alive, n_step, ptr(rays_alive, I32, "rays_alive"), ptr(rays_t, F32, "rays_t"),
                             ptr(rays_o, F32, "rays_o"), ptr(rays_d, F32, "rays_d"), float(bound), float(dt_gamma),
                             int(max_steps), int(C), int(H), ptr(density_bitfield, U8, "density_bitfield"),
                             ptr(_f(near)), ptr(_f(far)), ptr(xyzs), ptr(dirs), ptr(deltas), stream_ptr()),
          "march_rays")
    return xyzs, dirs, deltas


def composite_rays(n_alive, n_step, rays_alive, rays_t, sigmas, rgbs, deltas, weights_sum, depth, image,
# ... 125 lines not shown
```

Measured before the change: 6516 Msamples/s.

## Fuse near/far slab test and ray reordering into frame march count/write kernels

Adds frame-level march entry points that compute near/far AABB intersections inside the march count and write kernels, and accept a ray permutation (order), so results scatter back natively instead of through gather/scatter copies in Python. The count path merges the block-sum scan and offset finalize into one decoupled kernel. Identity ray indices are cached and passed as null to get_rays. This removes several small launches and full-frame permutation copies during eval rendering, but adds redundant per-block prefix summation and more complex indexing.

```diff
diff --git a/include/inr.h b/include/inr.h
--- a/include/inr.h
+++ b/include/inr.h
@@ -7,7 +7,7 @@
 extern "C" {
 #endif
 
-#define INR_ABI_VERSION 12
+#define INR_ABI_VERSION 13
 #define INR_MAX_LEVELS 16
 
 enum {
@@ -96,6 +96,18 @@
                                float* xyzs, float* dirs , float* deltas,
                                const void* workspace, int32_t sample_cap, int32_t* ray_ids ,
                                int32_t normalise , inr_stream_t s);
+int inr_frame_march_count(const float* rays_o, const float* rays_d, const uint8_t* bitfield, float bound, float dt_gamma,
+                          int32_t max_steps, int64_t N, int32_t cascade, int32_t H, const float* aabb ,
+                          float min_near, float* nears, float* fars, const float* noises ,
+                          const int32_t* order , int32_t rays_marched, int32_t* rays ,
+                          int32_t* counter , void* workspace, int32_t sample_cap, inr_stream_t s);
+int inr_frame_march_write(const float* rays_o, const float* rays_d, const uint8_t* bitfield, float bound, float dt_gamma,
+                          int32_t max_steps, int64_t N, int32_t cascade, int32_t H, int64_t M,
+                          const float* aabb , float min_near, const float* nears ,
+                          const float* fars , const float* noises ,
+                          const int32_t* rays , float* xyzs,
+                          float* dirs , float* deltas, const void* workspace, int32_t sample_cap,
+                          int32_t* ray_ids , int32_t normalise, int32_t rays_marched, inr_stream_t s);
 int inr_composite_rays_patch_forward(const float* sigmas, const float* rgbs, const float* deltas,
                                      const int32_t* rays, int64_t N, int64_t M, float T_thresh,
                                      const float* extra , int32_t K,
diff --git a/instance_nerf_amd/_lib.py b/instance_nerf_amd/_lib.py
--- a/instance_nerf_amd/_lib.py
+++ b/instance_nerf_amd/_lib.py
@@ -46,6 +46,10 @@
                                              c_int64, P, P, P, P, P, P, P, P, c_int32, P]),
     "inr_march_rays_patch_write": (c_int32, [P, P, P, c_float, c_float, c_int32, c_int64, c_int32, c_int32,
                                              c_int64, P, P, P, P, P, P, P, P, c_int32, P, c_int32, P]),
+    "inr_frame_march_count": (c_int32, [P, P, P, c_float, c_float, c_int32, c_int64, c_int32, c_int32, P, c_float,
+                                        P, P, P, P, c_int32, P, P, P, c_int32, P]),
+    "inr_frame_march_write": (c_int32, [P, P, P, c_float, c_float, c_int32, c_int64, c_int32, c_int32,
+                                        c_int64, P, c_float, P, P, P, P, P, P, P, P, c_int32, P, c_int32, c_int32, P]),
     "inr_nerf_bwd_packed_floats": (c_int64, []),
     "inr_nerf_pack_weights_device": (c_int32, [P, P, P, P, P, P, P, P]),
     "inr_nerf_forward_train": (c_int32, [P, P, c_int64, c_float, P, POINTER(GridDesc), P, P, P, P, P, P, P, P, P, P]),
@@ -134,7 +138,7 @@
 }
 EXPORTS = tuple(_SIGS)
 
-ABI_VERSION = 12
+ABI_VERSION = 13
 INSTANCE_STATS_WORKSPACE_BYTES = 512 * 64 * 8 * 4
 _lib = None
 
diff --git a/instance_nerf_amd/csrc/raymarch.hip b/instance_nerf_amd/csrc/raymarch.hip
--- a/instance_nerf_amd/csrc/raymarch.hip
+++ b/instance_nerf_amd/csrc/raymarch.hip
@@ -15,6 +15,24 @@
 constexpr int kRayBlock = 256;
 constexpr float kSqrt3x2 = 3.4641016151377544f;
 
+__device__ __forceinline__ void slab_near_far(const float (&o)[3], const float (&rd)[3], const float* __restrict__ aabb,
+                                              float min_near, bool miss, float& near_out, float& far_out) {
+  float near = -INFINITY, far = INFINITY;
+#pragma unroll
+  for (int a = 0; a < 3; ++a) {
+    const float t0 = (aabb[a] - o[a]) * rd[a];
+    const float t1 = (aabb[a + 3] - o[a]) * rd[a];
+    const float lo = t0 > t1 ? t1 : t0;
+    const float hi = t0 > t1 ? t0 : t1;
+    if (a > 0) miss = miss || (near > hi) || (lo > far);
+    near = lo > near ? lo : near;
+    far = hi < far ? hi : far;
+  }
+  if (near < min_near) near = min_near;
+  near_out = miss ? 3.402823466e+38f : near;
+  far_out = miss ? 3.402823466e+38f : far;
+}
+
 __global__ void __launch_bounds__(kRayBlock) k_near_far(const float* __restrict__ rays_o,
                                                         const float* __restrict__ rays_d,
                                                         const float* __restrict__ aabb, int64_t N,
@@ -23,23 +41,10 @@
                                                         const int64_t* __restrict__ labels, int64_t ignore) {
   const int64_t n = (int64_t)blockIdx.x * blockDim.x + threadIdx.x;
   if (n >= N) return;
-  float near = -INFINITY, far = INFINITY;
-  bool miss = labels != nullptr && labels[n] == ignore;
-#pragma unroll
-  for (int a = 0; a < 3; ++a) {
-    const float o = rays_o[n * 3 + a];
-    const float rd = 1.0f / rays_d[n * 3 + a];
-    const float t0 = (aabb[a] - o) * rd;
-    const float t1 = (aabb[a + 3] - o) * rd;
-    const float lo = t0 > t1 ? t1 : t0;
-    const float hi = t0 > t1 ? t0 : t1;
-    if (a > 0) miss = miss || (near > hi) || (lo > far);
-    near = lo > near ? lo : near;
-    far = hi < far ? hi : far;
-  }
-  if (near < min_near) near = min_near;
-  nears[n] = miss ? 3.402823466e+38f : near;
-  fars[n] = miss ? 3.402823466e+38f : far;
+  const bool miss = labels != nullptr && labels[n] == ignore;
+  const float o[3] = {rays_o[n * 3], rays_o[n * 3 + 1], rays_o[n * 3 + 2]};
+  const float rd[3] = {1.0f / rays_d[n * 3], 1.0f / rays_d[n * 3 + 1], 1.0f / rays_d[n * 3 + 2]};
+  slab_near_far(o, rd, aabb, min_near, miss, nears[n], fars[n]);
 }
 
 __global__ void __launch_bounds__(kRayBlock) k_get_rays(const float* __restrict__ poses, int64_t B, float fx, float fy,
@@ -325,6 +330,21 @@
   return near + step_dt(P, near) * noise;
 }
 
+struct FrameArgs {
+  const int32_t* order;
+  const float* aabb;
+  float min_near;
+  float* nears_out;
+  float* fars_out;
+  int rays_marched;
+};
+__device__ __forceinline__ int64_t ordered_ray(const int32_t* __restrict__ order, int64_t n, int64_t N) {
+  if (!order) return n;
+  const int64_t r = order[n];
+  return r < 0 ? 0 : (r >= N ? N - 1 : r);
+}
+
+template <bool kFrame>
 __global__ void __launch_bounds__(kRayBlock) k_march_count(MarchParams P, const float* __restrict__ rays_o,
                                                            const float* __restrict__ rays_d, int64_t N,
                                                            int max_steps, const float* __restrict__ nears,
@@ -332,7 +352,7 @@
                                                            const float* __restrict__ noises,
                                                            int32_t* __restrict__ counts,
                                                            int32_t* __restrict__ block_sums,
-                                                           uint32_t* __restrict__ mask, int cap_words) {
+                                                           uint32_t* __restrict__ mask, int cap_words, FrameArgs F) {
   __shared__ int32_t wsum[kRayBlock / 64];
   __shared__ uint32_t lut[1024];
   for (int i = threadIdx.x; i < P.H; i += kRayBlock) lut[i] = expand_bits10((uint32_t)i);
@@ -341,13 +361,25 @@
   const int64_t n = (int64_t)blockIdx.x * blockDim.x + threadIdx.x;
   int cnt = 0;
   if (n < N) {
-    const Ray r = load_ray(rays_o, rays_d, n);
-    const float t0 = start_t(P, nears[n], noises ? noises[n] : 0.0f);
+    const int64_t rid = kFrame ? ordered_ray(F.order, n, N) : n;
+    const Ray r = load_ray(rays_o, rays_d, (kFrame && F.rays_marched) ? n : rid);
+    float near, far;
+    if (kFrame && F.aabb) {
+      const float o[3] = {r.ox, r.oy, r.oz};
+      const float rd[3] = {r.rdx, r.rdy, r.rdz};
+      slab_near_far(o, rd, F.aabb, F.min_near, false, near, far);
+      F.nears_out[rid] = near;
+      F.fars_out[rid] = far;
+    } else {
+      near = nears[rid];
+      far = fars[rid];
+    }
+    const float t0 = start_t(P, near, noises ? noises[rid] : 0.0f);
     if (cap_words > 0) {
       uint32_t word = 0;
       int widx = 0, cand = 0;
       bool ok = true;
-      cnt = march_ray_any(P, r, t0, fars[n], max_steps,
+      cnt = march_ray_any(P, r, t0, far, max_steps,
                       [&](float, float, float, float, float, float) {
                         const int w = cand >> 5;
                         if (w < cap_words) {
@@ -365,7 +397,7 @@
       if (widx < cap_words) mask[(int64_t)widx * N + n] = word;
       mask[(int64_t)cap_words * N + n] = ok ? 1u : 0u;
     } else {
-      cnt = march_ray_any(P, r, t0, fars[n], max_steps, [](float, float, float, float, float, float) {}, [] {}, morton);
+      cnt = march_ray_any(P, r, t0, far, max_steps, [](float, float, float, float, float, float) {}, [] {}, morton);
     }
     counts[n] = cnt;
   }
@@ -421,6 +453,39 @@
     rays[n * 3 + 0] = (int32_t)n;
     rays[n * 3 + 1] = off;
     rays[n * 3 + 2] = cnt;
+  }
+}
+
+__global__ void __launch_bounds__(kRayBlock) k_scan_finalize(const int32_t* __restrict__ counts,
+                                                             const int32_t* __restrict__ block_sums, int64_t N,
+                                                             const int32_t* __restrict__ order,
+                                                             int32_t* __restrict__ rays, int32_t* __restrict__ counter) {
+  __shared__ int32_t wsum[kRayBlock / 64];
+  __shared__ int32_t psum[kRayBlock / 64];
+  int part = 0;
+  for (int i = threadIdx.x; i < (int)blockIdx.x; i += kRayBlock) part += block_sums[i];
+#pragma unroll
+  for (int d = 1; d < 64; d <<= 1) part += __shfl_xor(part, d, 64);
+  const int64_t n = (int64_t)blockIdx.x * blockDim.x + threadIdx.x;
+  const int cnt = n < N ? counts[n] : 0;
+  const int incl = wave_inclusive_scan(cnt);
+  if ((threadIdx.x & 63) == 63) wsum[threadIdx.x >> 6] = incl;
+  if ((threadIdx.x & 63) == 0) psum[threadIdx.x >> 6] = part;
+  __syncthreads();
+  int off = incl - cnt;
+#pragma unroll
+  for (int w = 0; w < kRayBlock / 64; ++w) off += psum[w];
+  for (int w = 0; w < (int)(threadIdx.x >> 6); ++w) off += wsum[w];
+  if (n < N) {
+    rays[n * 3 + 0] = (int32_t)ordered_ray(order, n, N);
+    rays[n * 3 + 1] = off;
+    rays[n * 3 + 2] = cnt;
+  }
+  if (blockIdx.x == gridDim.x - 1 && threadIdx.x == kRayBlock - 1) {
+    counter[0] = off + cnt;
+    counter[1] = (int32_t)N;
+    counter[2] = 0;
+    counter[3] = 0;
   }
 }
 
@@ -1332,6 +1397,7 @@
   }
 };
 
+template <bool kFrame>
 __global__ void __launch_bounds__(kRayBlock) k_march_write_patch(MarchParams P, const float* __restrict__ rays_o,
                                                                  const float* __restrict__ rays_d, int64_t N, int64_t M,
                                                                  const float* __restrict__ nears,
@@ -1341,14 +1407,18 @@
                                                                  float* __restrict__ xyzs, float* __restrict__ dirs,
                                                                  float* __restrict__ deltas,
                                                                  const uint32_t* __restrict__ mask, int cap_words,
-                                                                 int32_t* __restrict__ ray_ids, int normalise) {
+                                                                 int32_t* __restrict__ ray_ids, int normalise,
+                                                                 int rays_marched, const float* __restrict__ aabb,
+                                                                 float min_near) {
   const int64_t n = (int64_t)blockIdx.x * blockDim.x + threadIdx.x;
   const int off = n < N ? rays[n * 3 + 1] : 0;
   const int cnt = n < N ? rays[n * 3 + 2] : 0;
   GroupCursor cur;
   cur.init(cnt, off);
   if (cnt == 0 || (int64_t)cur.S + cur.total() > M) return;
-  const Ray r = load_ray(rays_o, rays_d, n);
+  const int64_t rid = kFrame ? (int64_t)rays[n * 3] : n;
+  const int64_t row = (kFrame && rays_marched) ? n : rid;
+  const Ray r = load_ray(rays_o, rays_d, row);
   const float rb = 2.0f * P.bound;
   auto emit = [&](float px, float py, float pz, float dt, float delta, float) {
     const int64_t i = cur.next();
@@ -1357,14 +1427,23 @@
     }
     xyzs[i * 3 + 0] = px; xyzs[i * 3 + 1] = py; xyzs[i * 3 + 2] = pz;
     if (dirs) { dirs[i * 3 + 0] = r.dx; dirs[i * 3 + 1] = r.dy; dirs[i * 3 + 2] = r.dz; }
-    if (ray_ids) ray_ids[i] = (int32_t)n;
+    if (ray_ids) ray_ids[i] = (int32_t)row;
     deltas[i * 2 + 0] = dt; deltas[i * 2 + 1] = delta;
   };
-  const float t0 = start_t(P, nears[n], noises ? noises[n] : 0.0f);
+  float near, far;
+  if (kFrame && aabb) {
+    const float o[3] = {r.ox, r.oy, r.oz};
+    const float rd[3] = {r.rdx, r.rdy, r.rdz};
+    slab_near_far(o, rd, aabb, min_near, false, near, far);
+  } else {
+    near = nears[rid];
+    far = fars[rid];
+  }
+  const float t0 = start_t(P, near, noises ? noises[rid] : 0.0f);
   if (cap_words > 0 && mask[(int64_t)cap_words * N + n]) {
     replay_ray(P, r, mask, N, n, t0, cnt, emit);
   } else {
-    march_ray(P, r, t0, fars[n], cnt, emit);
+    march_ray(P, r, t0, far, cnt, emit);
   }
 }
 
@@ -1794,8 +1873,8 @@
     k_scan_counts<<<1, 1024, 0, st>>>(counts, N, rays, counter);
     return check_launch("march_rays_train_count");
   }
-  k_march_count<<<nb, kRayBlock, march_lds_pad(), st>>>(P, rays_o, rays_d, N, max_steps, nears, fars, noises, counts, block_sums,
-                                          mask, cap_words_of(sample_cap));
+  k_march_count<false><<<nb, kRayBlock, march_lds_pad(), st>>>(P, rays_o, rays_d, N, max_steps, nears, fars, noises, counts,
+                                                         block_sums, mask, cap_words_of(sample_cap), FrameArgs{});
   k_scan_block_sums<<<1, 1024, 0, st>>>(block_sums, (int)nb, N, counter);
   k_finalize_offsets<<<nb, kRayBlock, 0, st>>>(counts, block_sums, N, rays);
   return check_launch("march_rays_train_count");
@@ -1842,10 +1921,54 @@
   const MarchParams P = make_params(bitfield, bound, dt_gamma, max_steps, cascade, H);
   INR_REQUIRE(sample_cap == 0 || workspace, "sample_cap > 0 needs the workspace of the count pass");
   const uint32_t* mask = sample_cap > 0 ? reinterpret_cast<const uint32_t*>(reinterpret_cast<const int32_t*>(workspace) + ws_ints(N)) : nullptr;
-  k_march_write_patch<<<blocks_for(N, kRayBlock), kRayBlock, march_lds_pad(), as_stream(s)>>>(P, rays_o, rays_d, N, M, nears, fars,
-                                                                                noises, rays, xyzs, dirs, deltas, mask,
-                                                                                cap_words_of(sample_cap), ray_ids, normalise);
+  k_march_write_patch<false><<<blocks_for(N, kRayBlock), kRayBlock, march_lds_pad(), as_stream(s)>>>(
+      P, rays_o, rays_d, N, M, nears, fars, noises, rays, xyzs, dirs, deltas, mask, cap_words_of(sample_cap), ray_ids, normalise, 0,
+      nullptr, 0.0f);
   return check_launch("march_rays_patch_write");
+}
+
+int inr_frame_march_count(const float* rays_o, const float* rays_d, const uint8_t* bitfield, float bound, float dt_gamma,
+                          int32_t max_steps, int64_t N, int32_t cascade, int32_t H, const float* aabb, float min_near,
+                          float* nears, float* fars, const float* noises, const int32_t* order, int32_t rays_marched,
+                          int32_t* rays, int32_t* counter, void* workspace, int32_t sample_cap, inr_stream_t s) {
+  INR_REQUIRE(rays_o && rays_d && bitfield && nears && fars && rays && counter && workspace, "null pointer");
+  INR_REQUIRE(N > 0 && N < (1ll << 31), "N out of range");
+  INR_REQUIRE(rays_marched == 0 || (rays_marched == 1 && order), "rays_marched must be 0, or 1 together with an order");
+  INR_REQUIRE(max_steps > 0 && cascade >= 1 && H >= 8 && H <= 1024, "bad grid parameters");
+  INR_REQUIRE(sample_cap >= 0 && ((uintptr_t)workspace & 7) == 0, "workspace must be 8-byte aligned");
+  INR_REQUIRE(((uintptr_t)counter & 7) == 0, "counter must be 8-byte aligned");
+  const MarchParams P = make_params(bitfield, bound, dt_gamma, max_steps, cascade, H);
+  const unsigned nb = blocks_for(N, kRayBlock);
+  int32_t* counts = reinterpret_cast<int32_t*>(workspace);
+  int32_t* block_sums = counts + N;
+  uint32_t* mask = reinterpret_cast<uint32_t*>(counts + ws_ints(N));
+  hipStream_t st = as_stream(s);
+  k_march_count<true><<<nb, kRayBlock, march_lds_pad(), st>>>(P, rays_o, rays_d, N, max_steps, aabb ? nullptr : nears,
+                                                        aabb ? nullptr : fars, noises, counts, block_sums, mask,
+                                                        cap_words_of(sample_cap),
+                                                        FrameArgs{order, aabb, min_near, nears, fars, rays_marched});
+  k_scan_finalize<<<nb, kRayBlock, 0, st>>>(counts, block_sums, N, order, rays, counter);
+  return check_launch("frame_march_count");
+}
+
+int inr_frame_march_write(const float* rays_o, const float* rays_d, const uint8_t* bitfield, float bound, float dt_gamma,
+                          int32_t max_steps, int64_t N, int32_t cascade, int32_t H, int64_t M, const float* aabb,
+                          float min_near, const float* nears, const float* fars, const float* noises, const int32_t* rays,
+                          float* xyzs, float* dirs, float* deltas, const void* workspace, int32_t sample_cap,
+                          int32_t* ray_ids, int32_t normalise, int32_t rays_marched, inr_stream_t s) {
+  INR_REQUIRE(rays_o && rays_d && bitfield && rays && (aabb || (nears && fars)), "null pointer");
+  INR_REQUIRE(N > 0 && N < (1ll << 31) && M >= 0, "bad sizes");
+  INR_REQUIRE(rays_marched == 0 || rays_marched == 1, "rays_marched must be 0 or 1");
+  INR_REQUIRE(max_steps > 0 && cascade >= 1 && H >= 8 && H <= 1024, "bad grid parameters");
+  INR_REQUIRE(sample_cap >= 0 && (sample_cap == 0 || workspace), "sample_cap > 0 needs the workspace of the count pass");
+  if (M == 0) return INR_OK;
+  INR_REQUIRE(xyzs && deltas && (dirs || ray_ids), "null output");
+  const MarchParams P = make_params(bitfield, bound, dt_gamma, max_steps, cascade, H);
+  const uint32_t* mask = sample_cap > 0 ? reinterpret_cast<const uint32_t*>(reinterpret_cast<const int32_t*>(workspace) + ws_ints(N)) : nullptr;
+  k_march_write_patch<true><<<blocks_for(N, kRayBlock), kRayBlock, march_lds_pad(), as_stream(s)>>>(
+      P, rays_o, rays_d, N, M, nears, fars, noises, rays, xyzs, dirs, deltas, mask, cap_words_of(sample_cap), ray_ids, normalise,
+      rays_marched, aabb, min_near);
+  return check_launch("frame_march_write");
 }
 
 int inr_composite_rays_patch_forward(const float* sigmas, const float* rgbs, const float* deltas, const int32_t* rays,
diff --git a/instance_nerf_amd/nerf/renderer.py b/instance_nerf_amd/nerf/renderer.py
--- a/instance_nerf_amd/nerf/renderer.py
+++ b/instance_nerf_amd/nerf/renderer.py
@@ -160,7 +160,8 @@
 
     def run_cuda(self, rays_o, rays_d, dt_gamma=0, bg_color=None, perturb=False, force_all_rays=False,
                  max_steps=1024, T_thresh=1e-4, infer_mode="auto", noises=None, field_gate=None, ce_labels=None,
-                 ce_ignore_index=-1, mse_target=None, marched=None, ce_prune=False, **kwargs):
+                 ce_ignore_index=-1, mse_target=None, marched=None, ce_prune=False, order=None, rays_in_order=False,
+                 **kwargs):
         prefix = rays_o.shape[:-1]
         rays_o = rays_o.contiguous().view(-1, 3).float()
         rays_d = rays_d.contiguous().view(-1, 3).float()
@@ -171,9 +172,16 @@
                                         and marched.get("grid_state", self.iter_density) == self.iter_density):
             self.drop_ahead(marched)
             marched = None
+        if not self.training and infer_mode == "auto":
+            infer_mode = "fused_terminate" if self._recent_skippable() > self.terminate_above else "fused"
+        frame = not self.training and infer_mode in ("fused", "fused_terminate")
+        if order is not None and not frame:
+            raise ValueError("order= applies to the one-pass inference modes only (NeRFRenderer.render handles the rest)")
         if marched is not None:
             marched["consume"]()
             nears, fars = marched["nears"], marched["fars"]
+        elif frame:
+            nears = fars = None
         elif self.training and ce_prune and ce_labels is not None:
             nears, fars = raymarching.near_far_from_aabb(rays_o, rays_d, aabb, self.min_near, skip_labels=ce_labels,
                                                          ignore_index=ce_ignore_index)
@@ -184,19 +192,17 @@
         results = {}
         skipped_frac = None
         with_instance = getattr(self, "num_instances", 0) > 0
-        if not self.training and infer_mode == "auto":
-            infer_mode = "fused_terminate" if self._recent_skippable() > self.terminate_above else "fused"
 
         fused_inst = with_instance and getattr(self, "_fusable_inst", False) and hasattr(self, "instance_render")
         if (not self.training and infer_mode == "fused_terminate" and getattr(self, "_fusable", False)
                 and (fused_inst or not with_instance)):
-            counter = torch.zeros(2, dtype=torch.int32, device=device)
-            xyzs, _, deltas, rays = raymarching.march_rays_patch(
-                rays_o, rays_d, self.bound, self.density_bitfield, self.cascade, self.grid_size, nears, fars,
-                dt_gamma, max_steps, noises=noises if perturb else None, counter=counter, table=True)
+            xyzs, _, deltas, rays, nears, fars, counter, _ = raymarching.march_rays_frame(
+                rays_o, rays_d, self.bound, self.density_bitfield, self.cascade, self.grid_size, aabb, self.min_near,
+                dt_gamma, max_steps, noises=noises if perturb else None, order=order, table=True, rays_marched=rays_in_order)
             if field_gate is not None:
                 field_gate.acquire()
-            weights_sum, depth, image, wbuf, evaluated = self.nerf_render(xyzs, deltas, rays, rays_d, T_thresh,
+            dirs_marched = rays_d if (order is None or rays_in_order) else torch.index_select(rays_d, 0, order)
+            weights_sum, depth, image, wbuf, evaluated = self.nerf_render(xyzs, deltas, rays, dirs_marched, T_thresh,
                                                                           want_weights=with_instance, normalised=True)
             if field_gate is not None:
                 field_gate.release()
@@ -210,18 +216,16 @@
             results["num_evaluated"] = evaluated
             skipped_frac = (evaluated, int(xyzs.shape[0]), True)
         elif not self.training and infer_mode in ("fused", "fused_terminate"):
-            counter = torch.zeros(2, dtype=torch.int32, device=device)
             table = (fused_inst or not with_instance) and getattr(self, "_fusable", False) and hasattr(self, "forward_table")
             early = {}
 
             def while_waiting():
-                early["skippable"] = torch.zeros(1, dtype=torch.int64, device=device)
                 if table and hasattr(self, "sh_table"):
                     early["shq"] = self.sh_table(rays_d)
-            xyzs, dirs, deltas, rays = raymarching.march_rays_patch(
-                rays_o, rays_d, self.bound, self.density_bitfield, self.cascade, self.grid_size, nears, fars,
-                dt_gamma, max_steps, noises=noises if perturb else None, counter=counter, table=table,
-                while_waiting=while_waiting)
+            xyzs, dirs, deltas, rays, nears, fars, counter, skippable = raymarching.march_rays_frame(
+                rays_o, rays_d, self.bound, self.density_bitfield, self.cascade, self.grid_size, aabb, self.min_near,
+                dt_gamma, max_steps, noises=noises if perturb else None, order=order, table=table,
+                while_waiting=while_waiting, rays_marched=rays_in_order)
             if field_gate is not None:
                 field_gate.acquire()
             sigmas, rgbs = self.forward_table(xyzs, dirs, rays_d, shq=early.get("shq")) if table else self(xyzs, dirs)
@@ -229,7 +233,6 @@
                 field_gate.release()
             if self.density_scale != 1:
                 sigmas = self.density_scale * sigmas
-            skippable = early["skippable"]
             if fused_inst:
                 weights_sum, depth, image, wbuf = raymarching.composite_rays_patch(sigmas, rgbs, deltas, rays, T_thresh,
                                                                                   return_weights=True, skippable=skippable)
@@ -557,6 +560,25 @@
     def render(self, rays_o, rays_d, staged=False, max_ray_batch=4096, **kwargs):
         _run = self.run_cuda if self.cuda_ray else self.run
         B, N = rays_o.shape[:2]
+        order = kwargs.pop("order", None)
+        rays_in_order = bool(kwargs.pop("rays_in_order", False))
+        if order is not None:
+            native = (self.cuda_ray and not self.training and B == 1 and rays_o.is_cuda
+                      and kwargs.get("infer_mode", "auto") in ("auto", "fused", "fused_terminate")
+                      and not (staged and N > max(int(max_ray_batch), int(self.min_staged_batch))))
+            if native:
+                kwargs.update(order=order, rays_in_order=rays_in_order)
+            else:
+                idx = order.long()
+                if not rays_in_order:
+                    rays_o, rays_d = rays_o[:, idx].contiguous(), rays_d[:, idx].contiguous()
+                out = self.render(rays_o, rays_d, staged=staged, max_ray_batch=max_ray_batch, **kwargs)
+                for k, v in list(out.items()):
+                    if torch.is_tensor(v) and v.dim() >= 2 and v.shape[1] == N:
+                        back = torch.empty_like(v)
+                        back[:, idx] = v
+                        out[k] = back
+                return out
         if self.cuda_ray:
             max_ray_batch = max(int(max_ray_batch), int(self.min_staged_batch))
         if staged and N > max_ray_batch:
diff --git a/instance_nerf_amd/nerf/utils.py b/instance_nerf_amd/nerf/utils.py
--- a/instance_nerf_amd/nerf/utils.py
+++ b/instance_nerf_amd/nerf/utils.py
@@ -32,6 +32,16 @@
     return _PATCH_INDS[key]
 
 
+def patch_order_i32(H, W, patch, device, super_tile=None):
+    st = SUPER_TILE if super_tile is None else super_tile
+    key = (H, W, patch, st, str(device), "i32")
+    if key not in _PATCH_INDS:
+        from .. import raymarching
+        inds = patch_order(H, W, patch, device, super_tile)
+        _PATCH_INDS[key] = raymarching.check_order(inds, H * W).to(torch.int32).contiguous()
+    return _PATCH_INDS[key]
+
+
 @torch.no_grad()
 def get_rays(poses, intrinsics, H, W, N=-1, error_map=None, inds=None, patch=0):
     device = poses.device
@@ -47,13 +57,18 @@
         parts = [get_rays(poses[b:b + 1], intrinsics, H, W, inds=per_batch[b]) for b in range(B)]
         return {"rays_o": torch.cat([p["rays_o"] for p in parts]), "rays_d": torch.cat([p["rays_d"] for p in parts]),
                 "inds": per_batch, "inds_coarse": inds_coarse}
+    identity = False
     if inds is None:
         if N > 0:
             inds = torch.randint(0, H * W, size=[N], device=device)
         elif patch:
             inds = patch_order(H, W, patch, device)
         else:
-            inds = torch.arange(H * W, device=device)
+            identity = True
+            key = ("arange", H * W, str(device))
+            if key not in _PATCH_INDS:
+                _PATCH_INDS[key] = torch.arange(H * W, device=device)
+            inds = _PATCH_INDS[key]
     inds = inds.contiguous().long()
     n = inds.shape[0]
     if poses.is_cuda:
@@ -62,7 +77,7 @@
         rays_o = torch.empty(B, n, 3, dtype=torch.float32, device=device)
         rays_d = torch.empty(B, n, 3, dtype=torch.float32, device=device)
         _lib.check(lib.inr_get_rays(_lib.ptr(poses, torch.float32, "poses"), B, float(fx), float(fy), float(cx), float(cy),
-                                    int(W), _lib.ptr(inds, torch.int64, "inds", allow_none=n == 0), n,
+                                    int(W), None if identity else _lib.ptr(inds, torch.int64, "inds", allow_none=n == 0), n,
                                     _lib.ptr(rays_o, allow_none=B * n == 0), _lib.ptr(rays_d, allow_none=B * n == 0),
                                     _lib.stream_ptr()), "get_rays")
         return {"rays_o": rays_o, "rays_d": rays_d, "inds": inds[None].expand(B, -1)}
@@ -784,13 +799,8 @@
                 and H % 4 == 0 and W % 4 == 0):
             return self.model.render(rays_o, rays_d, **kwargs)
         inds = patch_order(H, W, 4, rays_o.device)
-        out = self.model.render(rays_o[:, inds].contiguous(), rays_d[:, inds].contiguous(), **kwargs)
-        for k, v in list(out.items()):
-            if torch.is_tensor(v) and v.dim() >= 2 and v.shape[1] == H * W:
-                back = torch.empty_like(v)
-                back[:, inds] = v
-                out[k] = back
-        return out
+        return self.model.render(rays_o[:, inds].contiguous(), rays_d[:, inds].contiguous(),
+                                 order=patch_order_i32(H, W, 4, rays_o.device), rays_in_order=True, **kwargs)
 
     @torch.no_grad()
     def eval_step(self, data):
diff --git a/instance_nerf_amd/raymarching.py b/instance_nerf_amd/raymarching.py
--- a/instance_nerf_amd/raymarching.py
+++ b/instance_nerf_amd/raymarching.py
@@ -217,6 +217,58 @@
     return xyzs, (ray_ids if table else dirs), deltas, rays
 
 
+def check_order(order, n_rays):
+    if not torch.is_tensor(order) or order.dim() != 1 or order.dtype not in (torch.int32, torch.int64):
+        raise ValueError("order must be a 1-D int32 / int64 tensor")
+    if order.shape[0] != int(n_rays):
+        raise ValueError(f"order has {order.shape[0]} entries for {int(n_rays)} rays")
+    if n_rays == 0:
+        return order
+    o = order.long()
+    lo, hi = int(o.min()), int(o.max())
+    if lo < 0 or hi >= n_rays:
+        raise ValueError(f"order has entries outside [0, {int(n_rays)}): min {lo}, max {hi}")
+    if not bool((torch.sort(o).values == torch.arange(n_rays, device=o.device)).all()):
+        raise ValueError("order names a ray twice (it must be a permutation)")
+    return order
+
+
+def march_rays_frame(rays_o, rays_d, bound, density_bitfield, C, H, aabb, min_near=0.2, dt_gamma=0, max_steps=1024,
+                     noises=None, order=None, table=False, while_waiting=None, rays_marched=False):
+    lib = _lib.load()
+    rays_o, rays_d = _f(rays_o).view(-1, 3), _f(rays_d).view(-1, 3)
+    dev = rays_o.device
+    N = rays_o.shape[0]
+    noises = _f(noises) if noises is not None else None
+    if order is not None and (order.dtype != I32 or order.shape != (N,)):
+        raise RuntimeError(f"order must be int32 [{N}], got {order.dtype} {tuple(order.shape)}")
+    if rays_marched and order is None:
+        raise RuntimeError("rays_marched needs an order (where the results of the n-th ray belong)")
+    nears = torch.empty(N, dtype=F32, device=dev)
+    fars = torch.empty(N, dtype=F32, device=dev)
+    scratch = torch.empty(2, dtype=torch.int64, device=dev)
+    counter, skippable = scratch.view(I32)[:2], scratch[1:]
+    rays = torch.empty(N, 3, dtype=I32, device=dev)
+    cap = SAMPLE_CAP
+    ws = torch.empty(lib.inr_march_workspace_bytes(N, cap) // 8 + 1, dtype=torch.int64, device=dev)
+    args = (ptr(rays_o, F32, "rays_o"), ptr(rays_d, F32, "rays_d"), ptr(density_bitfield, U8, "density_bitfield"),
+            float(bound), float(dt_gamma), int(max_steps), N, int(C), int(H))
+    check(lib.inr_frame_march_count(*args, ptr(_f(aabb), F32, "aabb"), float(min_near), ptr(nears), ptr(fars),
+                                    ptr(noises, F32, "noises", allow_none=True), ptr(order, I32, "order", allow_none=True),
+                                    1 if rays_marched else 0, ptr(rays), ptr(scratch), ptr(ws), cap, stream_ptr()), "frame_march_count")
+    M = _read_count(counter, while_waiting)
+    xyzs = torch.empty(M, 3, dtype=F32, device=dev)
+    dirs = None if table else torch.empty(M, 3, dtype=F32, device=dev)
+    ray_ids = torch.empty(M, dtype=I32, device=dev) if table else None
+    deltas = torch.empty(M, 2, dtype=F32, device=dev)
+    check(lib.inr_frame_march_write(*args, M, ptr(_f(aabb), F32, "aabb"), float(min_near), ptr(nears), ptr(fars), ptr(noises, F32, "noises", allow_none=True),
+                                    ptr(rays), ptr(xyzs, allow_none=M == 0), ptr(dirs, allow_none=True),
+                                    ptr(deltas, allow_none=M == 0), ptr(ws), cap,
+                                    ptr(ray_ids, allow_none=True), 1 if table else 0, 1 if rays_marched else 0,
+                                    stream_ptr()), "frame_march_write")
+    return xyzs, (ray_ids if table else dirs), deltas, rays, nears, fars, counter, skippable
+
+
 def composite_rays_patch(sigmas, rgbs, deltas, rays, T_thresh=1e-4, extra=None, return_weights=False, skippable=None):
     lib = _lib.load()
     sigmas, rgbs, deltas = _f(sigmas), _f(rgbs), _f(deltas)
```

New measurement: 6512 Msamples/s. No clear change (-0.1%).
